# JdeRobot/slam-SDVL

Hardware: AMD Instinct MI355X
Metric: tracked frames/sec (640x480, 5-lvl pyr, ~200 feats) (higher is better)
Workload: dtype u8/f32/f64

## Files before the change

### include/sdvl_hip.h

```cpp
#ifndef SDVL_HIP_H_
#define SDVL_HIP_H_

#include <stdint.h>

#ifdef __cplusplus
extern "C" {
#endif

typedef struct sdvl_ctx sdvl_ctx;
typedef struct sdvl_frame sdvl_frame;

enum sdvl_status {
  SDVL_OK = 0,
  SDVL_ERR_INVALID = -1,
  SDVL_ERR_HIP = -2,
  SDVL_ERR_CAPACITY = -3,
  SDVL_ERR_NO_DEVICE = -4
};

#define SDVL_MAX_LEVELS 8
#define SDVL_MAX_CORNERS 6144
#define SDVL_MAX_ALIGN_FEATURES 2048
#define SDVL_CELL_KP_CAP 176
#define SDVL_MAX_CELL_SIZE 64
// ... 366 lines not shown
  int32_t n_points;
  int32_t n_deleted;
  int32_t lk_iters;
  int32_t n_corners;
  int32_t status;
} sdvl_track_result;

typedef struct sdvl_track_feature_out {
  double px[2];
  int32_t level;
  int32_t point;
} sdvl_track_feature_out;

typedef struct sdvl_track_point_stat {
  int32_t score, n_failed, last_frame;
  int32_t status;
} sdvl_track_point_stat;

int sdvl_track_create(sdvl_ctx *ctx, int n_trackers, int max_points, int max_features, int grid_cells, int max_matches,
                      int max_ransac_its, sdvl_track_set **out);
int sdvl_track_destroy(sdvl_ctx *ctx, sdvl_track_set *set);
int sdvl_frame_register(sdvl_ctx *ctx, const sdvl_frame *frame, const double *pose7);
int sdvl_frames_register(sdvl_ctx *ctx, int n, const sdvl_frame *const *frames, const double *poses7);
int sdvl_track_upload(sdvl_ctx *ctx, sdvl_track_set *set, int n, const int32_t *trackers, const int32_t *feat_buf, const int32_t *n_points,
                      const sdvl_track_point *points, const int32_t *n_features, const sdvl_track_feature *features);
int sdvl_track_append(sdvl_ctx *ctx, sdvl_track_set *set, int n, const int32_t *trackers, const int32_t *feat_buf, const int32_t *n_points,
                      const sdvl_track_point *points, const int32_t *n_features, const sdvl_track_feature *features);
int sdvl_track_align(sdvl_ctx *ctx, sdvl_track_set *set, int n_jobs, const sdvl_track_job *jobs, const uint16_t *cell_rank,
                     const int32_t *rand_raw, const sdvl_camera *cam, const sdvl_track_params *p);
int sdvl_track_search(sdvl_ctx *ctx, sdvl_track_set *set);
int sdvl_track_collect(sdvl_ctx *ctx, sdvl_track_set *set, int n_jobs, sdvl_track_result *results);
const sdvl_track_feature_out *sdvl_track_features(const sdvl_track_set *set, int job);
const sdvl_track_point_stat *sdvl_track_stats(const sdvl_track_set *set, int job);

typedef struct sdvl_klt_job {
  const sdvl_frame *prev, *next;
  int32_t pt_begin, pt_end;
} sdvl_klt_job;

typedef struct sdvl_klt_params {
  int32_t win_size;
  int32_t max_level;
  int32_t max_its;
  int32_t pad_;
  double eps;
  double min_eig_threshold;
} sdvl_klt_params;

int sdvl_klt_track(sdvl_ctx *ctx, int n_jobs, const sdvl_klt_job *jobs, int n_pts, const float *prev_xy, float *next_xy, uint8_t *status,
                   float *err, const sdvl_klt_params *params);

typedef struct sdvl_homography_job {
  int32_t m_begin, m_end;
  int32_t draw_begin, draw_end;
} sdvl_homography_job;

typedef struct sdvl_homography_result {
  double H[9];
  int32_t best_draw;
  int32_t n_its;
  int32_t n_inliers;
  int32_t pad_;
} sdvl_homography_result;

int sdvl_homography_ransac(sdvl_ctx *ctx, int n_jobs, const sdvl_homography_job *jobs, int n_m, const double *src_xy, const double *dst_xy,
                           int n_draws, const int32_t *draws4, double threshold, int max_its, double confidence,
// ... 84 lines not shown
```

### slam-sdvl_amd/__init__.py

```python
import ctypes as C
import os

import numpy as np

try:
    import torch
except ImportError:
    torch = None

_HERE = os.path.dirname(os.path.abspath(__file__))
CSRC = os.path.join(_HERE, "csrc")
LIB_PATH = os.path.join(CSRC, "libsdvl_hip.so")
HOST_LIB_PATH = os.path.join(_HERE, "host", "libsdvl_host.so")

SDVL_GRAY8, SDVL_RGB8, SDVL_BGR8, SDVL_RGBA8, SDVL_BGRA8 = 0, 1, 2, 3, 4
SDVL_BAYER_RGGB8, SDVL_BAYER_GRBG8, SDVL_BAYER_GBRG8, SDVL_BAYER_BGGR8 = 16, 17, 18, 19
SDVL_YUYV8, SDVL_UYVY8 = 20, 21
SDVL_GRAY10_16, SDVL_GRAY12_16, SDVL_GRAY16 = 22, 23, 24


def _raw_bytes(im):
    im = np.asarray(im)
    if im.dtype == np.uint16:
        im = np.ascontiguousarray(im.astype("<u2", copy=False)).view(np.uint8).reshape(im.shape + (2,))
# ... 91 lines not shown
                ("R", C.c_double * 9), ("t", C.c_double * 3), ("plane", C.c_double * 4),
                ("seed", C.c_uint32), ("frame_id", C.c_uint32), ("texture", C.c_uint32), ("reserved_", C.c_uint32),
                ("dist", C.c_double * 5)]


SYNTH_MAX_SURFACES = 8
SYNTH_NO_SURFACE = 255
SYNTH_SCENE_MAX_VIEWS = 4096


class SynthSurface(C.Structure):
    _fields_ = [("plane", C.c_double * 4), ("origin", C.c_double * 3), ("e1", C.c_double * 3), ("e2", C.c_double * 3),
                ("half_u", C.c_double), ("half_v", C.c_double), ("seed_add", C.c_uint32), ("pad_", C.c_uint32)]


class SynthScene(C.Structure):
    _fields_ = [("fx", C.c_double), ("fy", C.c_double), ("u0", C.c_double), ("v0", C.c_double),
                ("R", C.c_double * 9), ("t", C.c_double * 3),
                ("seed", C.c_uint32), ("frame_id", C.c_uint32), ("texture", C.c_uint32), ("n_surfaces", C.c_uint32),
                ("dist", C.c_double * 5), ("surfaces", SynthSurface * SYNTH_MAX_SURFACES)]


ABI_SYMBOLS = [
    "sdvl_ctx_create", "sdvl_ctx_destroy", "sdvl_last_error", "sdvl_ctx_synchronize", "sdvl_ctx_stream",
    "sdvl_ctx_bind_thread", "sdvl_ctx_device", "sdvl_pointer_device", "sdvl_ctx_scratch_device",
    "sdvl_ctx_timing_enable", "sdvl_ctx_timing_only", "sdvl_ctx_timing_get", "sdvl_ctx_timing_reset",
    "sdvl_frame_create", "sdvl_frame_create_many", "sdvl_frame_destroy", "sdvl_frame_upload", "sdvl_frames_upload", "sdvl_ctx_prefetch_images", "sdvl_ctx_prefetch_fence", "sdvl_frame_set_image_device", "sdvl_frame_borrow_image_device",
    "sdvl_pyramid_build", "sdvl_frame_download_level", "sdvl_fast_num_cells", "sdvl_cell_kp_cap", "sdvl_fast_cells",
    "sdvl_detect_corners", "sdvl_frames_corner_counts", "sdvl_frame_download_corners", "sdvl_retain_best",
    "sdvl_frame_set_corners", "sdvl_frames_set_corners", "sdvl_frame_num_corners", "sdvl_shi_tomasi", "sdvl_orb_describe",
    "sdvl_frame_download_descriptors", "sdvl_filter_inputs", "sdvl_filter_inputs_begin", "sdvl_filter_inputs_end", "sdvl_filter_corners_begin", "sdvl_filter_corners_end", "sdvl_orb_describe_points", "sdvl_hamming_argmin", "sdvl_image_align", "sdvl_image_align_begin", "sdvl_image_align_end", "sdvl_align_store_create", "sdvl_align_store_destroy", "sdvl_align_store_write", "sdvl_image_align_begin_stored", "sdvl_search_points", "sdvl_search_begin", "sdvl_search_slot", "sdvl_search_run", "sdvl_align_patches", "sdvl_pose_from_matches", "sdvl_search_points_filter", "sdvl_search_run_filter", "sdvl_depth_filter", "sdvl_search_run_chain", "sdvl_search_chain_end", "sdvl_frame_footprint", "sdvl_undistort", "sdvl_frames_upload_undistorted", "sdvl_convert_gray", "sdvl_frames_upload_color", "sdvl_ctx_set_wait_hook", "sdvl_ctx_wait_done", "sdvl_ctx_wait_block", "sdvl_ctx_health", "sdvl_ctx_counters",
    "sdvl_track_create", "sdvl_track_destroy", "sdvl_frame_register", "sdvl_frames_register", "sdvl_track_upload", "sdvl_track_append", "sdvl_track_align", "sdvl_track_search",
    "sdvl_track_collect", "sdvl_track_features", "sdvl_track_stats",
    "sdvl_synth_render", "sdvl_synth_render_scene", "sdvl_synth_scene_size", "sdvl_synth_scene_preset", "sdvl_synth_scene_preset_names",
    "sdvl_device_malloc", "sdvl_device_free", "sdvl_device_download",
    "sdvl_frames_own_images", "sdvl_feed_create", "sdvl_feed_destroy", "sdvl_feed_last_error", "sdvl_feed_slot_arrived", "sdvl_feed_images", "sdvl_ctx_feed_acquire", "sdvl_ctx_feed_release", "sdvl_frame_footprint_cap", "sdvl_ctx_set_corner_capacity", "sdvl_frame_corner_capacity", "sdvl_detect_scratch_bytes",
    "sdvl_klt_track", "sdvl_homography_ransac", "sdvl_bundle_adjust",
    "sdvl_ctx_set_wait_spin", "sdvl_ctx_fork_mark", "sdvl_ctx_fork_begin", "sdvl_ctx_fork_end", "sdvl_host_alloc_pinned", "sdvl_host_free_pinned", "sdvl_host_register", "sdvl_host_unregister",
]

_lib = None


def load_library():
    global _lib
    if _lib is None:
        if not os.path.exists(LIB_PATH):
            raise SdvlError("libsdvl_hip.so is not built (%s): run `python -c 'import __graft_entry__ as g; g.build()'`"
                            % LIB_PATH)
        lib = C.CDLL(LIB_PATH)
        lib.sdvl_last_error.restype = C.c_char_p
        lib.sdvl_last_error.argtypes = [C.c_void_p]
        lib.sdvl_ctx_stream.restype = C.c_void_p
        lib.sdvl_ctx_stream.argtypes = [C.c_void_p]
        lib.sdvl_bundle_adjust.argtypes = [C.c_void_p, C.c_int, C.c_void_p, C.c_int, C.c_void_p, C.c_void_p, C.c_int, C.c_void_p, C.c_int,
                                           C.c_void_p, C.c_void_p, C.c_void_p, C.c_void_p, C.c_void_p, C.c_void_p]
        lib.sdvl_synth_scene_preset.argtypes = [C.c_char_p, C.c_void_p]
        lib.sdvl_synth_scene_preset_names.restype = C.c_char_p
        lib.sdvl_synth_render_scene.argtypes = [C.c_void_p, C.c_int, C.c_void_p, C.c_int, C.c_int, C.c_void_p, C.c_int64, C.c_void_p, C.c_void_p]
        _lib = lib
    return _lib


def synth_scene_presets():
    return load_library().sdvl_synth_scene_preset_names().decode().split()

# ... 157 lines not shown


class TrackFeature(C.Structure):
    _fields_ = [("px", C.c_double * 2), ("bearing", C.c_double * 3), ("level", C.c_int32), ("point", C.c_int32)]


TRACK_DUPLICATE = 0x40000000


class TrackParams(C.Structure):
    _fields_ = [("align", AlignParams), ("search", SearchParams), ("pose", PoseParams), ("cell_size", C.c_int32), ("patch_size", C.c_int32),
                ("max_failed", C.c_int32), ("pad_", C.c_int32)]


class TrackJob(C.Structure):
    _fields_ = [("tracker", C.c_int32), ("feat_buf", C.c_int32), ("last", C.c_void_p), ("cur", C.c_void_p), ("T", C.c_double * 7),
                ("last_pose", C.c_double * 7), ("frame_id", C.c_int32), ("max_matches", C.c_int32)]


class TrackResult(C.Structure):
    _fields_ = [("pose", C.c_double * 7), ("align_error", C.c_double), ("scene_depth", C.c_double)] + [(n, C.c_int32) for n in (
        "align_meas", "align_iters", "n_features", "n_requests", "matches", "attempts", "n_draws", "n_inliers", "n_outliers", "refined",
        "n_points", "n_deleted", "lk_iters", "n_corners", "status")]


class TrackFeatureOut(C.Structure):
    _fields_ = [("px", C.c_double * 2), ("level", C.c_int32), ("point", C.c_int32)]


class TrackPointStat(C.Structure):
    _fields_ = [("score", C.c_int32), ("n_failed", C.c_int32), ("last_frame", C.c_int32), ("status", C.c_int32)]


class TrackSet:

    def __init__(self, ctx, n_trackers, max_points, max_features, grid_cells, max_matches, max_ransac_its):
        self.ctx = ctx
        self.n, self.cells, self.max_ransac_its = int(n_trackers), int(grid_cells), int(max_ransac_its)
        h = C.c_void_p()
        ctx._check(ctx.lib.sdvl_track_create(ctx.h, self.n, int(max_points), int(max_features), self.cells, int(max_matches),
                                             self.max_ransac_its, C.byref(h)))
        self.h = h
        self.n_points = {}
        ctx.lib.sdvl_track_features.restype = C.POINTER(TrackFeatureOut)
        ctx.lib.sdvl_track_features.argtypes = [C.c_void_p, C.c_int]
        ctx.lib.sdvl_track_stats.restype = C.POINTER(TrackPointStat)
        ctx.lib.sdvl_track_stats.argtypes = [C.c_void_p, C.c_int]

    def _rows(self, fn, trackers, feat_buf, points, features):
        n = len(trackers)
        assert len(feat_buf) == len(points) == len(features) == n
        tr, fb = np.asarray(trackers, np.int32), np.asarray(feat_buf, np.int32)
        npt, nft = np.asarray([len(p) for p in points], np.int32), np.asarray([len(f) for f in features], np.int32)
        pa = (TrackPoint * max(int(npt.sum()), 1))(*[r for p in points for r in p])
        fa = (TrackFeature * max(int(nft.sum()), 1))(*[r for f in features for r in f])
        self.ctx._check(fn(self.ctx.h, self.h, n, _ptr(tr, i32p), _ptr(fb, i32p), _ptr(npt, i32p), pa, _ptr(nft, i32p), fa))
        return tr.tolist(), npt.tolist()

    def upload(self, trackers, feat_buf, points, features):
        for t, k in zip(*self._rows(self.ctx.lib.sdvl_track_upload, trackers, feat_buf, points, features)):
            self.n_points[t] = k

    def append(self, trackers, feat_buf, points, features):
        for t, k in zip(*self._rows(self.ctx.lib.sdvl_track_append, trackers, feat_buf, points, features)):
            self.n_points[t] = self.n_points.get(t, 0) + k

    def step(self, jobs, cell_rank, rand_raw, cam, params, between=None):
        n = len(jobs)
        lib = self.ctx.lib
        rank = np.ascontiguousarray(cell_rank, np.uint16).reshape(n, self.cells)
        raw = np.ascontiguousarray(rand_raw, np.int32).reshape(n, self.max_ransac_its)
        n_points = [self.n_points.get(jobs[j].tracker, 0) for j in range(n)]
        self.ctx._check(lib.sdvl_track_align(self.ctx.h, self.h, n, jobs, _ptr(rank, C.POINTER(C.c_uint16)), _ptr(raw, i32p), C.byref(cam),
                                             C.byref(params)))
        if between is not None:
            between()
        self.ctx._check(lib.sdvl_track_search(self.ctx.h, self.h))
        res = (TrackResult * n)()
        self.ctx._check(lib.sdvl_track_collect(self.ctx.h, self.h, n, res))
        feat_t = np.dtype([("px", "<f8", 2), ("level", "<i4"), ("point", "<i4")])
        stat_t = np.dtype([("score", "<i4"), ("n_failed", "<i4"), ("last_frame", "<i4"), ("status", "<i4")])
        feats, stats = [], []
        for j in range(n):
            fp, sp = lib.sdvl_track_features(self.h, j), lib.sdvl_track_stats(self.h, j)
            feats.append(np.ctypeslib.as_array(C.cast(fp, u8p), (res[j].matches * C.sizeof(TrackFeatureOut),)).view(feat_t).copy()
                         if res[j].matches else np.zeros(0, feat_t))
            stats.append(np.ctypeslib.as_array(C.cast(sp, u8p), (n_points[j] * C.sizeof(TrackPointStat),)).view(stat_t).copy()
                         if n_points[j] else np.zeros(0, stat_t))
        return res, feats, stats

    def close(self):
        if self.h:
            self.ctx._check(self.ctx.lib.sdvl_track_destroy(self.ctx.h, self.h))
            self.h = None


BUNDLE_MAX_FREE = 16
BUNDLE_OK, BUNDLE_EMPTY, BUNDLE_NO_EDGES, BUNDLE_NONFINITE = 0, 1, 2, 3
# ... 321 lines not shown
    def pose_from_matches(self, jobs, fx, max_ransac_points=5, max_ransac_its=100, max_optim_pose_its=10, inlier_error_threshold=2.0):
        n = len(jobs)
        pj = (PoseJob * n)()
        obs_all, rand_all, nits_all = [], [], []
        for k, (obs, pose, draws) in enumerate(jobs):
            obs = np.ascontiguousarray(obs, np.float64).reshape(-1, 6)
            size = len(obs)
            pj[k].obs_begin = len(obs_all); pj[k].obs_end = len(obs_all) + size
            pj[k].rand_begin = len(rand_all); pj[k].nits_begin = len(nits_all)
            for c in range(7):
                pj[k].pose[c] = float(pose[c])
            for o in obs:
                obs_all.append(PoseObs(o[0], o[1], o[2], o[3], o[4], 1.0 / (1 << int(o[5]))))
            assert len(draws) >= max_ransac_its
            rand_all += [int(d) % size if size else 0 for d in draws[:max_ransac_its]]
            nits_all += ransac_budget_table(size, max_ransac_points, max_ransac_its)
        po = (PoseObs * max(len(obs_all), 1))(*obs_all)
        ra = np.asarray(rand_all, np.int32); ni = np.asarray(nits_all, np.int32)
        prm = PoseParams(max_ransac_points, max_ransac_its, max_optim_pose_its, 0, inlier_error_threshold / fx, fx)
        res = (PoseResult * n)()
        lists = np.zeros(max(len(obs_all), 1), np.int32)
        self.lib.sdvl_pose_from_matches.argtypes = [C.c_void_p, C.c_int, C.c_void_p, C.c_int, C.c_void_p, C.c_int, C.c_void_p, C.c_int,
                                                    C.c_void_p, C.c_void_p, C.c_void_p, C.c_void_p]
        self._check(self.lib.sdvl_pose_from_matches(self.h, n, pj, len(obs_all), po, len(ra), _ptr(ra, i32p), len(ni), _ptr(ni, i32p),
                                                    C.byref(prm), res, _ptr(lists, i32p)))
        out = []
        for k in range(n):
            b = pj[k].obs_begin
            out.append(dict(pose=np.array(list(res[k].pose)), n_draws=res[k].n_draws, refined=res[k].refined,
                            inliers=lists[b:b + res[k].n_inliers].copy(),
                            outliers=lists[b + res[k].n_inliers:b + res[k].n_inliers + res[k].n_outliers].copy()))
        return out

    def track_set(self, n_trackers, max_points, max_features, grid_cells, max_matches, max_ransac_its):
        return TrackSet(self, n_trackers, max_points, max_features, grid_cells, max_matches, max_ransac_its)

    def register(self, frames, poses):
        n = len(frames)
        arr = (C.c_void_p * max(n, 1))(*[f.h for f in frames])
        p7 = np.ascontiguousarray(poses, np.float64).reshape(n, 7)
        self._check(self.lib.sdvl_frames_register(self.h, n, arr, _ptr(p7, f64p)))

    def klt_track(self, jobs, win_size=30, max_level=4, max_its=30, eps=0.001, min_eig_threshold=1e-4):
        kj = (KltJob * max(len(jobs), 1))()
        prev_all, next_all = [], []
        at = 0
        for k, (fp, fn, pxy, nxy) in enumerate(jobs):
            pxy = np.asarray(pxy, np.float32).reshape(-1, 2)
            nxy = np.asarray(nxy, np.float32).reshape(-1, 2)
            assert len(pxy) == len(nxy)
            kj[k].prev, kj[k].next = fp.h.value, fn.h.value
            kj[k].pt_begin, kj[k].pt_end = at, at + len(pxy)
            at += len(pxy)
            prev_all.append(pxy)
            next_all.append(nxy)
        prev = np.ascontiguousarray(np.concatenate(prev_all) if jobs else np.zeros((0, 2)), np.float32)
        nxt = np.ascontiguousarray(np.concatenate(next_all) if jobs else np.zeros((0, 2)), np.float32).copy()
        status = np.zeros(max(at, 1), np.uint8)
        err = np.zeros(max(at, 1), np.float32)
        prm = KltParams(win_size, max_level, max_its, 0, eps, min_eig_threshold)
        self.lib.sdvl_klt_track.argtypes = [C.c_void_p, C.c_int, C.c_void_p, C.c_int, C.c_void_p, C.c_void_p, C.c_void_p, C.c_void_p, C.c_void_p]
        self._check(self.lib.sdvl_klt_track(self.h, len(jobs), kj, at, prev.ctypes.data, nxt.ctypes.data, status.ctypes.data, err.ctypes.data,
                                            C.byref(prm)))
        return [dict(xy=nxt[kj[k].pt_begin:kj[k].pt_end].copy(), status=status[kj[k].pt_begin:kj[k].pt_end].astype(bool),
                     err=err[kj[k].pt_begin:kj[k].pt_end].copy()) for k in range(len(jobs))]

# ... 188 lines not shown
```

### slam-sdvl_amd/csrc/sdvl_orb.hip

```cpp
#include <algorithm>
#include <vector>

#include "sdvl_internal.h"
#include "sdvl_orb_device.h"

namespace {

struct OrbJob {
  const uint8_t *level[SDVL_MAX_LEVELS];
  int lw[SDVL_MAX_LEVELS], lh[SDVL_MAX_LEVELS];
  const int32_t *corners;
  uint8_t *desc;
  uint8_t *out;
  float *out_angle;
  double *out_score;
  const int32_t *n_ptr;
  int n;
  int levels;
};

__device__ __forceinline__ bool xcd_frame_block(int n_frames, int chunks, int *frame, int *chunk) {
  const int b = static_cast<int>(blockIdx.x), q = b >> 3;
  *frame = (q / chunks) * 8 + (b & 7);
  *chunk = q % chunks;
  return *frame < n_frames;
}
inline dim3 xcd_frame_grid(int n_frames, int chunks) { return dim3(static_cast<unsigned>((n_frames + 7) / 8 * 8 * chunks)); }

__global__ __launch_bounds__(256) void orb_describe_kernel(const OrbJob *__restrict__ jobs, int n_jobs, int chunks) {
  int fj, bx;
  if (!xcd_frame_block(n_jobs, chunks, &fj, &bx)) return;
  const OrbJob &job = jobs[fj];
  const int lane = threadIdx.x & 63;
  const int n = job.n_ptr ? min(job.n_ptr[0], SDVL_MAX_CORNERS) : job.n;
  const int wpb = static_cast<int>(blockDim.x >> 6);
  for (int ci = bx * wpb + (threadIdx.x >> 6); ci < n; ci += chunks * wpb) {
  const int cx = job.corners[4 * ci], cy = job.corners[4 * ci + 1], cl = job.corners[4 * ci + 2];
  if (cl < 0 || cl >= job.levels) continue;
  const int W = job.lw[cl], H = job.lh[cl];
  uint8_t *dst = job.desc + static_cast<size_t>(ci) * 32;
  if (!(cx >= 19 && cx < W - 19 && cy >= 19 && cy < H - 19)) {
    if (lane < 32) {
      dst[lane] = 0;
      if (job.out) job.out[static_cast<size_t>(ci) * 32 + lane] = 0;
    }
    if (lane == 0 && job.out_angle) job.out_angle[ci] = -1.f;
    continue;
  }
  float angle_deg;
  const uint32_t nib = orb_wave_nibble(job.level[cl], static_cast<uint32_t>(cy * W + cx), W, lane, &angle_deg);
  const uint32_t hi = __shfl_down(nib, 1, 64);
  if ((lane & 1) == 0) {
    const uint8_t byte = static_cast<uint8_t>(nib | (hi << 4));
    dst[lane >> 1] = byte;
    if (job.out) job.out[static_cast<size_t>(ci) * 32 + (lane >> 1)] = byte;
  }
  if (lane == 0 && job.out_angle) job.out_angle[ci] = angle_deg;
  }
}

constexpr int kShiPerWave = 4;
__global__ __launch_bounds__(256) void shi_tomasi_kernel(const OrbJob *__restrict__ jobs, int n_jobs, int chunks) {
  int fj, bx;
  if (!xcd_frame_block(n_jobs, chunks, &fj, &bx)) return;
  const OrbJob &job = jobs[fj];
  const int lane = threadIdx.x & 63, grp = lane >> 4, q = lane & 15;
  const int n = job.n_ptr ? min(job.n_ptr[0], SDVL_MAX_CORNERS) : job.n;
  const int wpb = static_cast<int>(blockDim.x >> 6);
  for (int c0 = (bx * wpb + (threadIdx.x >> 6)) * kShiPerWave; c0 < n; c0 += chunks * wpb * kShiPerWave) {
    const int ci = c0 + grp;
    int sxx = 0, syy = 0, sxy = 0;
    bool inside = false;
    if (ci < n) {
      const int px = job.corners[4 * ci], py = job.corners[4 * ci + 1], cl = job.corners[4 * ci + 2];
      if (cl >= 0 && cl < job.levels) {
        const int W = job.lw[cl], H = job.lh[cl];
        const int x_min = px - 4, x_max = px + 4, y_min = py - 4, y_max = py + 4;
        inside = !(x_min < 1 || x_max >= W - 1 || y_min < 1 || y_max >= H - 1);
        if (inside) {
          const uint8_t *p = job.level[cl] + static_cast<size_t>(y_min + (q >> 1)) * W + (x_min + 4 * (q & 1));
          uint32_t lf, rt, up, dn;
          __builtin_memcpy(&lf, p - 1, 4);
          __builtin_memcpy(&rt, p + 1, 4);
          __builtin_memcpy(&up, p - W, 4);
          __builtin_memcpy(&dn, p + W, 4);
#pragma unroll
          for (int k = 0; k < 4; k++) {
            const int dx = static_cast<int>((rt >> (8 * k)) & 0xFFu) - static_cast<int>((lf >> (8 * k)) & 0xFFu);
            const int dy = static_cast<int>((dn >> (8 * k)) & 0xFFu) - static_cast<int>((up >> (8 * k)) & 0xFFu);
            sxx += dx * dx;
            syy += dy * dy;
            sxy += dx * dy;
          }
        }
      }
    }
#define SDVL_ROW_SUM(v)                                                   \
    v += __builtin_amdgcn_update_dpp(0, v, 0x111, 0xf, 0xf, false);       \
    v += __builtin_amdgcn_update_dpp(0, v, 0x112, 0xf, 0xf, false);       \
    v += __builtin_amdgcn_update_dpp(0, v, 0x114, 0xf, 0xe, false);       \
    v += __builtin_amdgcn_update_dpp(0, v, 0x118, 0xf, 0xc, false);
    SDVL_ROW_SUM(sxx)
    SDVL_ROW_SUM(syy)
    SDVL_ROW_SUM(sxy)
#undef SDVL_ROW_SUM
    if (q == 15 && ci < n) {
      const int cl = job.corners[4 * ci + 2];
      if (cl >= 0 && cl < job.levels) {
        double score = 0.0;
        if (inside) {
          float dXX = static_cast<float>(sxx), dYY = static_cast<float>(syy), dXY = static_cast<float>(sxy);
          dXX = static_cast<float>(dXX / (2.0 * 64));
          dYY = static_cast<float>(dYY / (2.0 * 64));
          dXY = static_cast<float>(dXY / (2.0 * 64));
          const float disc = (dXX + dYY) * (dXX + dYY) - 4 * (dXX * dYY - dXY * dXY);
          score = 0.5 * (dXX + dYY - sqrt(static_cast<double>(disc)));
        }
        job.out_score[ci] = score;
      }
    }
  }
}
inline int shi_chunks(int max_n) { return (max_n + kShiPerWave - 1) / kShiPerWave; }


struct FilterJob {
  const uint8_t *level[SDVL_MAX_LEVELS];
  int lw[SDVL_MAX_LEVELS], lh[SDVL_MAX_LEVELS];
  const int32_t *corners;
  const int32_t *n_ptr;
  const double *scores;
  const uint32_t *locked;
  sdvl_filtered_corner *out;
  int32_t *out_count;
  int levels, ccap;
};

constexpr int kFilterMaxCorners = SDVL_MAX_CORNERS;

__global__ __launch_bounds__(256) void filter_select_kernel(const FilterJob *__restrict__ jobs, int cell_size, int grid_w, int n_cells, int margin,
                                                            int min_score, int max_out) {
  __shared__ uint16_t s_cell[kFilterMaxCorners];
  __shared__ int s_sel[4096];
  __shared__ int s_wave[4];
  const FilterJob &job = jobs[blockIdx.x];
  const int tid = threadIdx.x, lane = tid & 63, wave = tid >> 6;
  const int n = min(min(job.n_ptr[0], job.ccap), kFilterMaxCorners);
  for (int i = tid; i < n; i += 256) {
    const int px = job.corners[4 * i], py = job.corners[4 * i + 1], level = job.corners[4 * i + 2];
    uint16_t c = 0xFFFFu;
    if (level >= 0 && level < job.levels && !(px < margin || py < margin || px >= job.lw[level] - margin || py >= job.lh[level] - margin)) {
      const int scale = 1 << level;
      const int pos = ((py * scale) / cell_size) * grid_w + (px * scale) / cell_size;
      if (pos >= 0 && pos < n_cells && !((job.locked[pos >> 5] >> (pos & 31)) & 1u)) c = static_cast<uint16_t>(pos);
// ... 14 lines not shown
    s_sel[c] = best > min_score ? best_idx : -1;
  }
  __syncthreads();
  int running = 0;
  for (int c0 = 0; c0 < n_cells; c0 += 256) {
    const int c = c0 + tid;
    const bool ok = c < n_cells && s_sel[c] >= 0;
    const unsigned long long m = __ballot(ok);
    const int below = __builtin_amdgcn_mbcnt_hi(static_cast<uint32_t>(m >> 32), __builtin_amdgcn_mbcnt_lo(static_cast<uint32_t>(m), 0));
    __syncthreads();
    if (lane == 0) s_wave[wave] = __popcll(m);
    __syncthreads();
    int pos = running + below;
    for (int w = 0; w < wave; w++) pos += s_wave[w];
    if (ok && pos < max_out) {
      const int i = s_sel[c];
      sdvl_filtered_corner r;
      r.index = i;
      r.x = job.corners[4 * i]; r.y = job.corners[4 * i + 1]; r.level = job.corners[4 * i + 2];
      r.score = static_cast<int>(job.scores[i]);
      r.pad_ = 0;
      sdvl_filtered_corner *dst = job.out + pos;
      dst->index = r.index; dst->x = r.x; dst->y = r.y; dst->level = r.level; dst->score = r.score; dst->pad_ = 0;
    }
    running += s_wave[0] + s_wave[1] + s_wave[2] + s_wave[3];
  }
  if (tid == 0) job.out_count[0] = running;
}

constexpr int kBinCells = 2048, kBinSlots = 10;
constexpr int kBinCellsSmall = 512, kBinCornersSmall = 2048;
constexpr int kBinCellsLarge = SDVL_MAX_LEVEL_CELLS, kBinSlotsLarge = 4;

template <int kCells, int kCorners, int kSlots = kBinSlots>
__global__ __launch_bounds__(256) void filter_select_binned_kernel(const FilterJob *__restrict__ jobs, int cell_size, int grid_w, int n_cells,
                                                                   int margin, int min_score, int max_out) {
  __shared__ uint16_t s_cell[kCorners];
  __shared__ uint16_t s_list[kCells * kSlots];
  __shared__ int s_cnt[kCells];
  __shared__ int s_wave[4];
  const FilterJob &job = jobs[blockIdx.x];
  const int tid = threadIdx.x, lane = tid & 63, wave = tid >> 6;
  const int n = min(min(job.n_ptr[0], job.ccap), kCorners);
  for (int c = tid; c < n_cells; c += 256) s_cnt[c] = 0;
  __syncthreads();
  for (int i = tid; i < n; i += 256) {
    const int px = job.corners[4 * i], py = job.corners[4 * i + 1], level = job.corners[4 * i + 2];
    uint16_t c = 0xFFFFu;
    if (level >= 0 && level < job.levels && !(px < margin || py < margin || px >= job.lw[level] - margin || py >= job.lh[level] - margin)) {
      const int scale = 1 << level;
      const int pos = ((py * scale) / cell_size) * grid_w + (px * scale) / cell_size;
      if (pos >= 0 && pos < n_cells && !((job.locked[pos >> 5] >> (pos & 31)) & 1u)) {
        c = static_cast<uint16_t>(pos);
        const int slot = atomicAdd(&s_cnt[pos], 1);
        if (slot < kSlots) s_list[pos * kSlots + slot] = static_cast<uint16_t>(i);
      }
    }
    s_cell[i] = c;
  }
  __syncthreads();
  for (int c = tid; c < n_cells; c += 256) {
    const int cnt = s_cnt[c];
    int best_idx = 0, best = min_score;
    if (cnt <= kSlots) {
      int idx[kSlots];
#pragma unroll
      for (int q = 0; q < kSlots; q++) idx[q] = q < cnt ? s_list[c * kSlots + q] : 0x7FFFFFFF;
#pragma unroll
      for (int a = 0; a < kSlots; a++)
#pragma unroll
        for (int b = 0; b + 1 < kSlots - a; b++) {
          const int lo = min(idx[b], idx[b + 1]), hi = max(idx[b], idx[b + 1]);
          idx[b] = lo;
          idx[b + 1] = hi;
        }
#pragma unroll
      for (int q = 0; q < kSlots; q++) {
        if (q >= cnt) break;
        const double score = job.scores[idx[q]];
        if (score > best) {
          best_idx = idx[q];
          best = static_cast<int>(score);
        }
      }
    } else {
      for (int i = 0; i < n; i++) {
        if (s_cell[i] != c) continue;
        const double score = job.scores[i];
        if (score > best) {
          best_idx = i;
          best = static_cast<int>(score);
        }
      }
    }
    s_cnt[c] = best > min_score ? best_idx : -1;
  }
  __syncthreads();
  int running = 0;
  for (int c0 = 0; c0 < n_cells; c0 += 256) {
    const int c = c0 + tid;
    const bool ok = c < n_cells && s_cnt[c] >= 0;
    const unsigned long long m = __ballot(ok);
    const int below = __builtin_amdgcn_mbcnt_hi(static_cast<uint32_t>(m >> 32), __builtin_amdgcn_mbcnt_lo(static_cast<uint32_t>(m), 0));
    __syncthreads();
    if (lane == 0) s_wave[wave] = __popcll(m);
    __syncthreads();
    int pos = running + below;
    for (int w = 0; w < wave; w++) pos += s_wave[w];
    if (ok && pos < max_out) {
      const int i = s_cnt[c];
      sdvl_filtered_corner *dst = job.out + pos;
      dst->index = i;
      dst->x = job.corners[4 * i]; dst->y = job.corners[4 * i + 1]; dst->level = job.corners[4 * i + 2];
      dst->score = static_cast<int>(job.scores[i]);
      dst->pad_ = 0;
    }
    running += s_wave[0] + s_wave[1] + s_wave[2] + s_wave[3];
  }
  if (tid == 0) job.out_count[0] = running;
}

__global__ __launch_bounds__(256) void filter_describe_kernel(const FilterJob *__restrict__ jobs, int max_out, int n_jobs, int chunks) {
  int fj, bx;
  if (!xcd_frame_block(n_jobs, chunks, &fj, &bx)) return;
  const FilterJob &job = jobs[fj];
  const int lane = threadIdx.x & 63;
  const int total = min(job.out_count[0], max_out);
  const int wpb = static_cast<int>(blockDim.x >> 6);
  for (int k = bx * wpb + (threadIdx.x >> 6); k < total; k += chunks * wpb) {
    sdvl_filtered_corner *dst = job.out + k;
    const int cx = dst->x, cy = dst->y, cl = dst->level;
    const int W = job.lw[cl], H = job.lh[cl];
    uint8_t byte = 0;
    if (cx >= 19 && cx < W - 19 && cy >= 19 && cy < H - 19) {
      float angle_deg;
      const uint32_t nib = orb_wave_nibble(job.level[cl], static_cast<uint32_t>(cy * W + cx), W, lane, &angle_deg);
      const uint32_t hi = __shfl_down(nib, 1, 64);
      byte = static_cast<uint8_t>(nib | (hi << 4));
    }
    if ((lane & 1) == 0) dst->desc[lane >> 1] = byte;
  }
}

__global__ __launch_bounds__(256) void filter_gather_kernel(const OrbJob *__restrict__ jobs, uint4 *__restrict__ dst, int row_units, int ccap,
                                                            int with_desc) {
  const OrbJob &job = jobs[blockIdx.y];
  const int u = blockIdx.x * 256 + threadIdx.x;
  if (u >= row_units) return;
  uint4 v;
  if (u <= ccap) {
    v = reinterpret_cast<const uint4 *>(job.n_ptr)[u];
  } else if (with_desc) {
    v = reinterpret_cast<const uint4 *>(job.desc)[u - (ccap + 1)];
  } else {
    return;
  }
  dst[static_cast<size_t>(blockIdx.y) * row_units + u] = v;
}

int fill_jobs(sdvl_ctx *ctx, int n, sdvl_frame *const *frames, int cap, uint8_t *d_out_desc, double *d_out_score,
              OrbJob **d_jobs, int *max_n) {
  const size_t bytes = sizeof(OrbJob) * n;
  void *hs = nullptr, *dsx = nullptr;
  int rc = sdvl_stage_alloc(ctx, bytes, &hs, &dsx);
  if (rc) return rc;
  OrbJob *hj = static_cast<OrbJob *>(hs);
  *max_n = 0;
  for (int i = 0; i < n; i++) {
    int rcf = sdvl_frame_fix_header(ctx, frames[i]);
    if (rcf) return rcf;
    const FrameView &v = frames[i]->v;
    memset(&hj[i], 0, sizeof(OrbJob));
    for (int l = 0; l < v.levels; l++) { hj[i].level[l] = v.level[l]; hj[i].lw[l] = v.lw[l]; hj[i].lh[l] = v.lh[l]; }
    hj[i].corners = v.corners;
// ... 18 lines not shown
  const uint8_t *queries;
  const int32_t *offsets;
  const uint8_t *cands;
  int32_t *best;
  int n, threshold;
};

__global__ __launch_bounds__(64) void hamming_argmin_kernel(const HammingJob *jobp) {
  const HammingJob &job = *jobp;
  const int q = blockIdx.x, lane = threadIdx.x;
  if (q >= job.n) return;
  const uint4 *qp = reinterpret_cast<const uint4 *>(job.queries + 32 * static_cast<size_t>(q));
  const uint4 q0 = qp[0], q1 = qp[1];
  const int begin = job.offsets[q], end = job.offsets[q + 1];
  unsigned long long key = (static_cast<unsigned long long>(job.threshold + 1) << 32) | 0xffffffffull;
  for (int c = begin + lane; c < end; c += 64) {
    const uint4 *cp = reinterpret_cast<const uint4 *>(job.cands + 32 * static_cast<size_t>(c));
    const uint4 a = cp[0], b = cp[1];
    const int d = __popc(a.x ^ q0.x) + __popc(a.y ^ q0.y) + __popc(a.z ^ q0.z) + __popc(a.w ^ q0.w) + __popc(b.x ^ q1.x) +
                  __popc(b.y ^ q1.y) + __popc(b.z ^ q1.z) + __popc(b.w ^ q1.w);
    const unsigned long long k = (static_cast<unsigned long long>(d) << 32) | static_cast<unsigned>(c - begin);
    key = k < key ? k : key;
  }
  for (int off = 32; off > 0; off >>= 1) {
    const unsigned long long o = __shfl_xor(key, off, 64);
    key = o < key ? o : key;
  }
  if (lane == 0) {
    const int d = static_cast<int>(key >> 32);
    const bool found = d < job.threshold;
    job.best[2 * q] = found ? static_cast<int>(key & 0xffffffffull) : -1;
    job.best[2 * q + 1] = d;
  }
}

extern "C" {

int sdvl_orb_describe(sdvl_ctx *ctx, int n, sdvl_frame *const *frames, int cap, uint8_t *out_desc) {
  if (!ctx || n < 0 || (n > 0 && !frames)) return SDVL_ERR_INVALID;
  if (n == 0) return SDVL_OK;
  for (int i = 0; i < n; i++) {
    SDVL_REQUIRE(ctx, frames[i] != nullptr, "null frame");
    if (out_desc) {
      int cnt = 0;
      int rc0 = sdvl_frame_count_host(ctx, frames[i], &cnt);
      if (rc0) return rc0;
    }
    if (out_desc && frames[i]->v.n_corners > cap) {
      ctx->err = "descriptor output capacity smaller than the corner count";
      return SDVL_ERR_CAPACITY;
    }
  }
  uint8_t *d_desc = nullptr;
  const size_t out_bytes = out_desc ? static_cast<size_t>(n) * cap * 32 : 0;
  if (out_desc) {
    int rc = sdvl_ensure(ctx, &ctx->d_out, &ctx->d_out_bytes, out_bytes, false);
    if (!rc) rc = sdvl_ensure(ctx, &ctx->h_out, &ctx->h_out_bytes, out_bytes, true);
    if (rc) return rc;
    d_desc = static_cast<uint8_t *>(ctx->d_out);
  }
  OrbJob *d_jobs = nullptr;
  int max_n = 0;
  int rc = fill_jobs(ctx, n, frames, cap, d_desc, nullptr, &d_jobs, &max_n);
  if (rc) return rc;
  if (max_n > 0) SDVL_LAUNCH(ctx, "orb_describe", orb_describe_kernel, xcd_frame_grid(n, max_n), dim3(64), d_jobs, n, max_n);
    SDVL_HIP_CHECK(ctx, hipGetLastError());
// ... 339 lines not shown
```

### slam-sdvl_amd/csrc/sdvl_search_types.h

```cpp
#ifndef SDVL_SEARCH_TYPES_H_
#define SDVL_SEARCH_TYPES_H_

#include "sdvl_internal.h"
#include "sdvl_math.h"

constexpr int kWavesPerBlock = 4;
constexpr int kLdsCorners = 4096;

struct SearchBlock {
  int first, count;
};

struct SearchFrame {
  const uint8_t *level[SDVL_MAX_LEVELS];
  int lw[SDVL_MAX_LEVELS], lh[SDVL_MAX_LEVELS];
  const int32_t *corners;
  const uint8_t *desc;
  const int32_t *n_ptr;
  int levels;
  int bin_gw;
  const int32_t *bin_start;
  const uint2 *bin_entries;
  int bin_cells, pad_;
  int pad2_[2];
// ... 123 lines not shown
};
static_assert(sizeof(TrackPoint) == sizeof(sdvl_track_point), "upload converts in place");
static_assert(sizeof(sdvl_track_point) == 144, "layout");
struct TrackFeat {
  double px[2];
  double bearing[3];
  int32_t level;
  int32_t point;
};
static_assert(sizeof(TrackFeat) == sizeof(sdvl_track_feature) && sizeof(TrackFeat) == 48, "layout");

struct TrackJobDev {
  SearchFrame cur;
  int tracker, feat_buf;
  int cur_id, last_id;
  int frame_id, max_matches;
  int n_feat, n_points;
  double last_pose[7];
  double pad_;
  const uint8_t *last_level[SDVL_MAX_LEVELS];
  double T0[7];
  double pad2_;
};

extern "C" TrackPoint *sdvl_track_points_device(sdvl_track_set *set, int *max_points, int *n_trackers);

int sdvl_search_launch_device(sdvl_ctx *ctx, int n_slots, const SearchReqDev *d_reqs, const SearchFramePose *d_table,
                              const SearchBlock *d_blocks, int n_blocks, const sdvl_camera *cam, const sdvl_search_params *p,
                              SearchPrep *d_prep, sdvl_search_res *d_res, sdvl_search_res *h_res, bool prepared = false, bool binned = true);
int sdvl_select_matches_launch(sdvl_ctx *ctx, int n_frames, const PoseChainIn &in, PoseJobDev *d_jobs, sdvl_pose_obs *d_obs);
int sdvl_image_align_track_enqueue(sdvl_ctx *ctx, int n_jobs, const TrackJobDev *d_jobs, const TrackPoint *d_points, const TrackFeat *d_feats0,
                                   const TrackFeat *d_feats1, int np, int nfeat_cap, int max_nf, int levels, const sdvl_camera *cam,
                                   const sdvl_align_params *p, sdvl_align_result *d_results, int batch_size);
extern "C" int sdvl_ensure_nits_table(sdvl_ctx *ctx, int npoints_cfg, int max_its, int max_size);

#endif
```

### slam-sdvl_amd/csrc/sdvl_track.hip

```cpp
#include <atomic>
#include <chrono>
#include <vector>

#include "sdvl_internal.h"
#include "sdvl_math.h"
#include "sdvl_search_types.h"
#include "sdvl_search_prepare.h"

namespace {

using namespace sdvl;


struct UploadRec {
  int tracker, feat_buf;
  int n_points, n_feat;
  long long point_off, feat_off;
  int point_dst, feat_dst;
  long long pad_;
};

struct RegisterRec {
  SearchFramePose e;
  int id, pad_;
};

__global__ __launch_bounds__(64) void track_clear_bins_kernel(TrackJobDev *__restrict__ jobs, const uint8_t *__restrict__ no_bins, int n) {
  const int j = blockIdx.x * 64 + threadIdx.x;
  if (j < n && no_bins[j]) {
    jobs[j].cur.bin_start = nullptr;
    jobs[j].cur.bin_entries = nullptr;
    jobs[j].cur.bin_gw = 0;
    jobs[j].cur.bin_cells = 0;
  }
}

__global__ __launch_bounds__(64) void registry_write_kernel(const RegisterRec *__restrict__ recs, int n, SearchFramePose *__restrict__ registry) {
  const int i = blockIdx.x * 64 + threadIdx.x;
  if (i < n) registry[recs[i].id] = recs[i].e;
}

__global__ __launch_bounds__(256) void track_upload_kernel(const UploadRec *__restrict__ recs, const TrackPoint *__restrict__ src_points,
                                                           const TrackFeat *__restrict__ src_feats, TrackPoint *__restrict__ points,
                                                           TrackFeat *__restrict__ feats0, TrackFeat *__restrict__ feats1, int np, int nf) {
  const UploadRec r = recs[blockIdx.x];
  const uint4 *sp = reinterpret_cast<const uint4 *>(src_points + r.point_off);
  uint4 *dp = reinterpret_cast<uint4 *>(points + static_cast<size_t>(r.tracker) * np + r.point_dst);
  const int pw = r.n_points * static_cast<int>(sizeof(TrackPoint) / 16);
  for (int i = threadIdx.x; i < pw; i += 256) dp[i] = sp[i];
  const uint4 *sf = reinterpret_cast<const uint4 *>(src_feats + r.feat_off);
  uint4 *df = reinterpret_cast<uint4 *>((r.feat_buf ? feats1 : feats0) + static_cast<size_t>(r.tracker) * nf + r.feat_dst);
  const int fw = r.n_feat * static_cast<int>(sizeof(TrackFeat) / 16);
  for (int i = threadIdx.x; i < fw; i += 256) df[i] = sf[i];
}

constexpr int kProjThreads = 512;

struct ProjLds {
  size_t px, cell, bytes;
  __host__ __device__ constexpr explicit ProjLds(size_t stride) : px(8 * stride), cell(px + 16 * stride), bytes(cell + 2 * stride + 64) {}
};
constexpr size_t kProjLdsDefault = 60 * 1024, kProjLdsMax = ProjLds(4096).bytes;
static_assert(kProjLdsMax == 106560, "track_project at stride 4096");

__global__ __launch_bounds__(kProjThreads) void track_project_kernel(const TrackJobDev *__restrict__ jobs, TrackPoint *__restrict__ points,
                                                                     const TrackFeat *__restrict__ feats0, const TrackFeat *__restrict__ feats1,
                                                                     int np, int nf, int stride, int mm, int max_its,
                                                                     const sdvl_align_result *__restrict__ ares,
                                                                     const uint16_t *__restrict__ cell_rank, int cells, Cam cam, int cell_size,
                                                                     int patch, SearchFramePose *__restrict__ registry,
                                                                     SearchReqDev *__restrict__ reqs, double *__restrict__ req_point,
                                                                     int32_t *__restrict__ cand_first, int32_t *__restrict__ cand_feat,
                                                                     SearchBlock *__restrict__ blocks, ChainFrameDev *__restrict__ chain,
                                                                     sdvl_search_params sprm, SearchPrep *__restrict__ prep) {
  extern __shared__ __attribute__((aligned(16))) uint8_t s_dyn[];
  const ProjLds lds(stride);
  unsigned long long *s_key = reinterpret_cast<unsigned long long *>(s_dyn);
  double *s_px = reinterpret_cast<double *>(s_dyn + lds.px);
  uint16_t *s_cell = reinterpret_cast<uint16_t *>(s_dyn + lds.cell);
  __shared__ double s_pose[7];
  __shared__ int s_ncand;
  const int j = blockIdx.x, tid = threadIdx.x;
  const TrackJobDev &jb = jobs[j];
  const TrackFeat *F = (jb.feat_buf ? feats1 : feats0) + static_cast<size_t>(jb.tracker) * nf;
  TrackPoint *P = points + static_cast<size_t>(jb.tracker) * np;
  const int n_feat = jb.n_feat;
// ... 88 lines not shown
  for (int b = tid; b < nblk; b += static_cast<int>(blockDim.x)) {
    int cnt = n_cand - b * kWavesPerBlock;
    cnt = cnt < 0 ? 0 : (cnt > kWavesPerBlock ? kWavesPerBlock : cnt);
    blocks[j * nblk + b] = SearchBlock{base + b * kWavesPerBlock, cnt};
  }
  if (tid == 0) {
    ChainFrameDev c;
    c.cand_begin = base;
    c.cand_end = base + n_cand;
    c.max_matches = jb.max_matches;
    c.rand_begin = j * max_its;
    c.obs_begin = j * mm;
    c.pad_ = 0;
#pragma unroll
    for (int q = 0; q < 7; q++) c.pose[q] = s_pose[q];
    c.pad2_ = 0.0;
    chain[j] = c;
  }
}

struct CommitLds {
  size_t found, depth, bytes;
  __host__ __device__ CommitLds(size_t stride, size_t mm) : found(2 * (stride + 1)), depth((found + stride + 64 + 7) / 8 * 8), bytes(depth + 8 * mm) {}
};

__global__ __launch_bounds__(256) void track_commit_kernel(const TrackJobDev *__restrict__ jobs, TrackPoint *__restrict__ points,
                                                           const TrackFeat *__restrict__ feats0_c, const TrackFeat *__restrict__ feats1_c,
                                                           TrackFeat *__restrict__ feats0, TrackFeat *__restrict__ feats1, int np, int nf, int stride,
                                                           int mm, const ChainFrameDev *__restrict__ chain, const int32_t *__restrict__ cand_first,
                                                           const int32_t *__restrict__ cand_feat, const sdvl_search_res *__restrict__ res,
                                                           const sdvl_pose_result *__restrict__ pres, const int32_t *__restrict__ lists,
                                                           const sdvl_align_result *__restrict__ ares, Cam cam, int max_failed,
                                                           SearchFramePose *__restrict__ registry, sdvl_track_result *__restrict__ h_results,
                                                           sdvl_track_feature_out *__restrict__ h_feats, sdvl_track_point_stat *__restrict__ h_stats) {
  extern __shared__ __attribute__((aligned(16))) uint8_t s_dyn[];
  const CommitLds lds(stride, mm);
  uint16_t *s_before = reinterpret_cast<uint16_t *>(s_dyn);
  uint8_t *s_found = s_dyn + lds.found;
  double *s_depth = reinterpret_cast<double *>(s_dyn + lds.depth);
  __shared__ int s_wave[4];
  __shared__ int s_attempts, s_deleted, s_lk, s_npoints;
  __shared__ double s_median;
  const int j = blockIdx.x, tid = threadIdx.x, lane = tid & 63, wave = tid >> 6;
  const TrackJobDev &jb = jobs[j];
  const ChainFrameDev &fr = chain[j];
  const int base = fr.cand_begin, n = fr.cand_end - fr.cand_begin;
  const TrackFeat *F = (jb.feat_buf ? feats1_c : feats0_c) + static_cast<size_t>(jb.tracker) * nf;
  TrackFeat *N = (jb.feat_buf ? feats0 : feats1) + static_cast<size_t>(jb.tracker) * nf;
  TrackPoint *P = points + static_cast<size_t>(jb.tracker) * np;
  if (tid == 0) { s_attempts = 0; s_deleted = 0; s_lk = 0; s_npoints = 0; }
  int lk = 0;
  for (int k = tid; k < n; k += 256) {
    const sdvl_search_res &r = res[base + k];
    s_found[k] = r.found != 0 ? 1 : 0;
    lk += r.lk_its;
  }
  __syncthreads();
  if (lk) atomicAdd(&s_lk, lk);
  int running = 0;
  for (int c0 = 0; c0 < n; c0 += 256) {
    const int k = c0 + tid;
    bool sel = false;
    if (k < n && s_found[k]) {
      sel = true;
      for (int q = cand_first[base + k] - base; q < k; q++)
        if (s_found[q]) { sel = false; break; }
    }
    const unsigned long long m = __ballot(sel);
    const int below = __builtin_amdgcn_mbcnt_hi(static_cast<uint32_t>(m >> 32), __builtin_amdgcn_mbcnt_lo(static_cast<uint32_t>(m), 0));
    __syncthreads();
    if (lane == 0) s_wave[wave] = __popcll(m);
    __syncthreads();
    int b = running;
    for (int w = 0; w < wave; w++) b += s_wave[w];
// ... 81 lines not shown
  for (int q = tid; q < jb.n_points; q += 256) {
    TrackPoint &p = P[q];
    if (p.status & kTrash) p.status = (p.status & ~kTrash) | kDeleted;
    sdvl_track_point_stat s;
    s.score = p.score; s.n_failed = p.n_failed; s.last_frame = p.last_frame; s.status = p.status;
    h_stats[static_cast<size_t>(j) * np + q] = s;
  }
  __syncthreads();
  if (tid == 0) {
    sdvl_track_result out;
#pragma unroll
    for (int q = 0; q < 7; q++) out.pose[q] = pr.pose[q];
    out.align_error = ares[j].error;
    out.scene_depth = s_median;
    out.align_meas = ares[j].n_meas;
    out.align_iters = ares[j].iters_run;
    out.n_features = jb.n_feat;
    out.n_requests = n;
    out.matches = matches;
    out.attempts = s_attempts;
    out.n_draws = pr.n_draws;
    out.n_inliers = pr.n_inliers;
    out.n_outliers = pr.n_outliers;
    out.refined = pr.refined;
    out.n_points = s_npoints;
    out.n_deleted = s_deleted;
    out.lk_iters = s_lk;
    out.n_corners = jb.cur.n_ptr[0];
    out.status = 0;
    h_results[j] = out;
#pragma unroll
    for (int q = 0; q < 7; q++) registry[jb.cur_id].pose[q] = pr.pose[q];
  }
}

}

struct sdvl_track_set {
  sdvl_ctx *ctx;
  int n, np, nf, cells, mm, max_its;
  TrackPoint *d_points = nullptr;
  TrackFeat *d_feats[2] = {nullptr, nullptr};
  uint8_t *d_scratch = nullptr;
  sdvl_part<TrackJobDev> djobs;
  sdvl_part<uint16_t> cell_rank;
  sdvl_part<sdvl_align_result> ares;
  sdvl_part<SearchReqDev> reqs;
  sdvl_part<SearchPrep> prep;
  sdvl_part<sdvl_search_res> res;
  sdvl_part<double> reqpt;
  sdvl_part<int32_t> rand, cfirst, cfeat, lists, nobs;
  sdvl_part<SearchBlock> blocks;
  sdvl_part<ChainFrameDev> chain;
  sdvl_part<PoseJobDev> pjobs;
  sdvl_part<sdvl_pose_obs> obs;
  sdvl_part<uint8_t> hyp;
  sdvl_part<sdvl_pose_result> pres;
  uint8_t *h_pinned = nullptr;
  sdvl_track_result *h_results;
  sdvl_track_feature_out *h_feats;
  sdvl_track_point_stat *h_stats;
  std::vector<int> n_points;
  std::vector<int> n_feat[2];
  std::vector<sdvl_track_job> jobs;
  int stride = 0;
  int phase = 0;
  uint32_t ticket = 0;
  sdvl_camera cam;
  sdvl_track_params prm;
};

extern "C" {

int sdvl_track_create(sdvl_ctx *ctx, int n, int max_points, int max_features, int grid_cells, int max_matches, int max_ransac_its,
                      sdvl_track_set **out) {
  if (!ctx || !out) return SDVL_ERR_INVALID;
  *out = nullptr;
  SDVL_REQUIRE(ctx, n >= 1 && n <= 65536, "tracker count out of range");
  SDVL_REQUIRE(ctx, max_points >= 1 && max_points < SDVL_TRACK_DUPLICATE && max_features >= 4 && max_features <= 4096, "table capacities out of range (features <= 4096)");
  SDVL_REQUIRE(ctx, grid_cells >= 1 && grid_cells <= 65535, "grid too large");
  SDVL_REQUIRE(ctx, max_matches >= 1 && max_matches <= 1024 && max_matches <= max_features, "max_matches outside the device pose stage's range (1024)");
  SDVL_REQUIRE(ctx, max_ransac_its >= 1 && max_ransac_its <= 4096, "bad max_ransac_its");
  SDVL_HIP_CHECK(ctx, sdvl_bind_device(ctx));
  sdvl_track_set *s = new sdvl_track_set();
  s->ctx = ctx;
  s->n = n;
  s->np = max_points;
  s->nf = (max_features + 3) / 4 * 4;
  s->cells = grid_cells;
  s->mm = max_matches;
  s->max_its = max_ransac_its;
  const size_t N = static_cast<size_t>(n), NF = N * s->nf;
  hipError_t e = hipMalloc(reinterpret_cast<void **>(&s->d_points), sizeof(TrackPoint) * N * s->np);
  if (e == hipSuccess) e = hipMalloc(reinterpret_cast<void **>(&s->d_feats[0]), sizeof(TrackFeat) * NF);
  if (e == hipSuccess) e = hipMalloc(reinterpret_cast<void **>(&s->d_feats[1]), sizeof(TrackFeat) * NF);
  sdvl_layout L;
  s->djobs = L.take<TrackJobDev>(N);
  s->cell_rank = L.take<uint16_t>(N * s->cells);
  s->rand = L.take<int32_t>(N * s->max_its);
  s->ares = L.take<sdvl_align_result>(N);
  s->reqs = L.take<SearchReqDev>(NF);
  s->prep = L.take<SearchPrep>(NF);
  s->res = L.take<sdvl_search_res>(NF);
  s->reqpt = L.take<double>(NF * 3);
  s->cfirst = L.take<int32_t>(NF);
  s->cfeat = L.take<int32_t>(NF);
  s->blocks = L.take<SearchBlock>(NF / kWavesPerBlock);
  s->chain = L.take<ChainFrameDev>(N);
  const bool separate = sdvl_pose_separate_launches(n);
  s->pjobs = L.take<PoseJobDev>(separate ? N : 0);
  s->obs = L.take<sdvl_pose_obs>(N * s->mm);
  s->hyp = L.take<uint8_t>(separate ? sdvl_pose_hyp_bytes() * N * s->max_its : 0);
  s->pres = L.take<sdvl_pose_result>(N);
  s->lists = L.take<int32_t>(N * s->mm);
  s->nobs = L.take<int32_t>(N);
  if (e == hipSuccess) e = hipMalloc(reinterpret_cast<void **>(&s->d_scratch), L.bytes());
  if (e == hipSuccess) {
    sdvl_layout H;
    const sdvl_part<sdvl_track_result> results = H.take<sdvl_track_result>(N);
    const sdvl_part<sdvl_track_feature_out> feats = H.take<sdvl_track_feature_out>(NF);
    const sdvl_part<sdvl_track_point_stat> stats = H.take<sdvl_track_point_stat>(N * s->np);
    e = hipHostMalloc(reinterpret_cast<void **>(&s->h_pinned), H.bytes(), hipHostMallocDefault);
    if (e == hipSuccess) {
      memset(s->h_pinned, 0, H.bytes());
      s->h_results = results.in(s->h_pinned);
      s->h_feats = feats.in(s->h_pinned);
      s->h_stats = stats.in(s->h_pinned);
    }
  }
  if (e != hipSuccess) {
    ctx->err = std::string("sdvl_track_create: ") + hipGetErrorString(e);
    sdvl_track_destroy(ctx, s);
    return SDVL_ERR_HIP;
  }
  s->n_points.assign(n, 0);
  s->n_feat[0].assign(n, 0);
  s->n_feat[1].assign(n, 0);
  *out = s;
  return SDVL_OK;
}

TrackPoint *sdvl_track_points_device(sdvl_track_set *set, int *max_points, int *n_trackers) {
  if (max_points) *max_points = set->np;
  if (n_trackers) *n_trackers = set->n;
  return set->d_points;
}

int sdvl_track_destroy(sdvl_ctx *ctx, sdvl_track_set *s) {
  if (!ctx || !s) return SDVL_ERR_INVALID;
  (void)sdvl_bind_device(ctx);
  (void)sdvl_stream_wait(ctx);
  if (s->d_points) (void)hipFree(s->d_points);
  if (s->d_feats[0]) (void)hipFree(s->d_feats[0]);
  if (s->d_feats[1]) (void)hipFree(s->d_feats[1]);
  if (s->d_scratch) (void)hipFree(s->d_scratch);
  if (s->h_pinned) (void)hipHostFree(s->h_pinned);
  delete s;
  return SDVL_OK;
}

int sdvl_frame_register(sdvl_ctx *ctx, const sdvl_frame *f, const double *pose7) { return sdvl_frames_register(ctx, 1, &f, pose7); }

int sdvl_frames_register(sdvl_ctx *ctx, int n, const sdvl_frame *const *frames, const double *poses7) {
  if (!ctx || n < 0 || (n > 0 && (!frames || !poses7))) return SDVL_ERR_INVALID;
  if (n == 0) return SDVL_OK;
  for (int i = 0; i < n; i++)
    SDVL_REQUIRE(ctx, frames[i] && frames[i]->home == ctx && frames[i]->reg_id >= 0 && frames[i]->reg_id < ctx->registry_cap,
                 "frame was not created on this context");
  void *hs = nullptr, *dsx = nullptr;
  int rc = sdvl_stage_alloc(ctx, sizeof(RegisterRec) * static_cast<size_t>(n), &hs, &dsx);
  if (rc) return rc;
  RegisterRec *r = static_cast<RegisterRec *>(hs);
  for (int i = 0; i < n; i++) {
    fill_view(&r[i].e.f, frames[i]);
    memcpy(r[i].e.pose, poses7 + 7 * i, sizeof(double) * 7);
    r[i].e.pad_ = 0.0;
    r[i].id = frames[i]->reg_id;
    r[i].pad_ = 0;
  }
  SDVL_HIP_CHECK(ctx, sdvl_push(ctx, dsx, hs, sizeof(RegisterRec) * static_cast<size_t>(n)));
  SDVL_LAUNCH(ctx, "registry_write", registry_write_kernel, dim3((n + 63) / 64), dim3(64), static_cast<const RegisterRec *>(dsx), n,
              static_cast<SearchFramePose *>(ctx->d_registry));
  SDVL_HIP_CHECK(ctx, hipGetLastError());
  return SDVL_OK;
}

static int track_upload_rows(sdvl_ctx *ctx, sdvl_track_set *s, int n, const int32_t *trackers, const int32_t *feat_buf, const int32_t *n_points,
                             const sdvl_track_point *points, const int32_t *n_features, const sdvl_track_feature *features, bool append) {
// ... 92 lines not shown
  rc = sdvl_ensure_nits_table(ctx, p->pose.max_ransac_points, p->pose.max_ransac_its, s->mm);
  if (rc) return rc;
  s->stride = (max_nf + kWavesPerBlock - 1) / kWavesPerBlock * kWavesPerBlock;
  if (s->stride < kWavesPerBlock) s->stride = kWavesPerBlock;
  s->cam = *cam;
  s->prm = *p;
  s->jobs.assign(jobs, jobs + n_jobs);
  const size_t rand_bytes = sizeof(int32_t) * static_cast<size_t>(n_jobs) * s->max_its;
  const size_t head_bytes = s->rand.off + rand_bytes;
  void *hs = nullptr, *dsx = nullptr;
  rc = sdvl_stage_alloc(ctx, head_bytes, &hs, &dsx);
  if (rc) return rc;
  TrackJobDev *hj = s->djobs.in(hs);
  for (int j = 0; j < n_jobs; j++) {
    const sdvl_track_job &a = jobs[j];
    TrackJobDev &d = hj[j];
    fill_view(&d.cur, a.cur,  true);
    d.tracker = a.tracker;
    d.feat_buf = a.feat_buf;
    d.cur_id = a.cur->reg_id;
    d.last_id = a.last->reg_id;
    d.frame_id = a.frame_id;
    d.max_matches = a.max_matches;
    d.n_feat = s->n_feat[a.feat_buf][a.tracker];
    d.n_points = s->n_points[a.tracker];
    memcpy(d.last_pose, a.last_pose, sizeof(double) * 7);
    d.pad_ = 0.0;
    SDVL_REQUIRE(ctx, a.last->width == a.cur->width && a.last->height == a.cur->height && a.last->v.levels == a.cur->v.levels,
                 "frame pair with different geometry");
    for (int l = 0; l < SDVL_MAX_LEVELS; l++) d.last_level[l] = l < a.last->v.levels ? a.last->v.level[l] : nullptr;
    memcpy(d.T0, a.T, sizeof(double) * 7);
    d.pad2_ = 0.0;
  }
  memcpy(s->cell_rank.in(hs), cell_rank, sizeof(uint16_t) * static_cast<size_t>(n_jobs) * s->cells);
  memcpy(s->rand.in(hs), rand_raw, rand_bytes);
  SDVL_HIP_CHECK(ctx, sdvl_push(ctx, s->d_scratch, hs, head_bytes));
  rc = sdvl_image_align_track_enqueue(ctx, n_jobs, s->djobs.cin(s->d_scratch), static_cast<const TrackPoint *>(s->d_points),
                                      static_cast<const TrackFeat *>(s->d_feats[0]), static_cast<const TrackFeat *>(s->d_feats[1]), s->np, s->nf, max_nf,
                                      jobs[0].cur->v.levels, cam, &p->align, s->ares.in(s->d_scratch), s->n);
  if (rc) return rc;
  s->phase = 1;
  return SDVL_OK;
}

int sdvl_track_search(sdvl_ctx *ctx, sdvl_track_set *s) {
  if (!ctx || !s || s->ctx != ctx) return SDVL_ERR_INVALID;
  SDVL_REQUIRE(ctx, s->phase == 1, "sdvl_track_search without sdvl_track_align");
  const int n_jobs = static_cast<int>(s->jobs.size());
  for (const sdvl_track_job &a : s->jobs) {
    SDVL_REQUIRE(ctx, !a.cur->hdr_stale, "current frame has a new image but no corners (detect or set corners first)");
    SDVL_REQUIRE(ctx, s->prm.search.max_fast_levels <= a.cur->v.levels, "max_fast_levels exceeds the pyramid depth");
  }
  const Cam c = cam_of(s->cam);
  const int stride = s->stride;
  uint8_t *const D = s->d_scratch;
  SearchFramePose *registry = static_cast<SearchFramePose *>(ctx->d_registry);
  {
    static const bool never = getenv("SDVL_TRACK_NO_BINS") != nullptr;
    bool any = false;
    for (const sdvl_track_job &a : s->jobs) any = any || (a.cur->bin_cells > 0 && (never || !a.cur->bins_valid));
    for (const sdvl_track_job &a : s->jobs) ctx->counters[(a.cur->bin_cells > 0 && !never && a.cur->bins_valid) ? 0 : 1]++;
    if (any) {
      void *hs = nullptr, *dsx = nullptr;
      const int rc_m = sdvl_stage_alloc(ctx, static_cast<size_t>(n_jobs), &hs, &dsx);
      if (rc_m) return rc_m;
      uint8_t *hm = static_cast<uint8_t *>(hs);
      for (int j = 0; j < n_jobs; j++) hm[j] = (s->jobs[j].cur->bin_cells > 0 && (never || !s->jobs[j].cur->bins_valid)) ? 1 : 0;
      SDVL_HIP_CHECK(ctx, sdvl_push(ctx, dsx, hs, static_cast<size_t>(n_jobs)));
      hipLaunchKernelGGL(track_clear_bins_kernel, dim3((n_jobs + 63) / 64), dim3(64), 0, ctx->stream, s->djobs.in(D), static_cast<const uint8_t *>(dsx), n_jobs);
      SDVL_HIP_CHECK(ctx, hipGetLastError());
    }
  }
  const size_t proj_lds = ProjLds(stride).bytes;
  if (proj_lds > kProjLdsDefault) {
    static std::atomic<unsigned long long> attr_devices{0};
    const int rc_a = sdvl_allow_dynamic_lds(ctx, reinterpret_cast<const void *>(track_project_kernel), kProjLdsMax, &attr_devices);
    if (rc_a) return rc_a;
  }
  {
    const int proj_threads = stride <= 256 ? (s->n > 32 ? 128 : 256) : kProjThreads;
    SDVL_LAUNCH_LDS(ctx, "track_project", track_project_kernel, dim3(n_jobs), dim3(proj_threads), proj_lds, s->djobs.cin(D), s->d_points,
                    static_cast<const TrackFeat *>(s->d_feats[0]), static_cast<const TrackFeat *>(s->d_feats[1]), s->np, s->nf, stride, s->mm,
                    s->max_its, s->ares.cin(D), s->cell_rank.cin(D), s->cells, c, s->prm.cell_size, s->prm.patch_size, registry, s->reqs.in(D),
                    s->reqpt.in(D), s->cfirst.in(D), s->cfeat.in(D), s->blocks.in(D), s->chain.in(D), s->prm.search, s->prep.in(D));
    SDVL_HIP_CHECK(ctx, hipGetLastError());
  }
  int rc = sdvl_search_launch_device(ctx, n_jobs * stride, s->reqs.in(D), registry, s->blocks.in(D), n_jobs * (stride / kWavesPerBlock), &s->cam,
                                     &s->prm.search, s->prep.in(D), s->res.in(D), nullptr,  true);
  if (rc) return rc;
  const PoseChainIn chain = {s->chain.cin(D), nullptr, s->cfirst.cin(D), s->res.cin(D), s->reqpt.cin(D), c, s->nobs.in(D), nullptr};
  const bool separate = sdvl_pose_separate_launches(s->n);
  sdvl_pose_params pp = s->prm.pose;
  pp.pad_ = 1;
  rc = sdvl_pose_enqueue_device(ctx, n_jobs, &chain, separate ? s->pjobs.in(D) : nullptr, s->obs.in(D), s->rand.in(D), static_cast<const int32_t *>(ctx->d_nits),
                                &pp, separate ? s->hyp.in(D) : nullptr, s->pres.in(D), s->lists.in(D), s->mm, s->n);
  if (rc) return rc;
  SDVL_LAUNCH_LDS(ctx, "track_commit", track_commit_kernel, dim3(n_jobs), dim3(256), CommitLds(stride, s->mm).bytes, s->djobs.cin(D), s->d_points,
                  static_cast<const TrackFeat *>(s->d_feats[0]), static_cast<const TrackFeat *>(s->d_feats[1]), s->d_feats[0], s->d_feats[1], s->np,
                  s->nf, stride, s->mm, s->chain.cin(D), s->cfirst.cin(D), s->cfeat.cin(D), s->res.cin(D), s->pres.cin(D), s->lists.cin(D),
                  s->ares.cin(D), c, s->prm.max_failed, registry, s->h_results, s->h_feats, s->h_stats);
  SDVL_HIP_CHECK(ctx, hipGetLastError());
  SDVL_HIP_CHECK(ctx, sdvl_mark_record(ctx, SDVL_MARK_CHAIN, &s->ticket));
  s->phase = 2;
  return SDVL_OK;
}

int sdvl_track_collect(sdvl_ctx *ctx, sdvl_track_set *s, int n_jobs, sdvl_track_result *results) {
  if (!ctx || !s || s->ctx != ctx || !results) return SDVL_ERR_INVALID;
  SDVL_REQUIRE(ctx, s->phase == 2 && n_jobs == static_cast<int>(s->jobs.size()), "sdvl_track_collect without a matching sdvl_track_search");
  SDVL_HIP_CHECK(ctx, sdvl_mark_wait(ctx, SDVL_MARK_CHAIN, s->ticket));
  s->phase = 0;
  memcpy(results, s->h_results, sizeof(sdvl_track_result) * n_jobs);
  for (int j = 0; j < n_jobs; j++) {
    const sdvl_track_job &a = s->jobs[j];
    s->n_feat[1 - a.feat_buf][a.tracker] = results[j].matches;
    if (results[j].n_corners >= 0) a.cur->v.n_corners = results[j].n_corners;
  }
  ctx->wait_gen++;
  return SDVL_OK;
}

const sdvl_track_feature_out *sdvl_track_features(const sdvl_track_set *s, int job) {
  return (s && job >= 0 && job < s->n) ? s->h_feats + static_cast<size_t>(job) * s->nf : nullptr;
}

const sdvl_track_point_stat *sdvl_track_stats(const sdvl_track_set *s, int job) {
  return (s && job >= 0 && job < s->n) ? s->h_stats + static_cast<size_t>(job) * s->np : nullptr;
}

}
```

### slam-sdvl_amd/host/capi.cc

```cpp
#include <algorithm>
#include <cstddef>
#include <cstring>
#include <set>
#include <string>

#include "farm.h"
#include "homography_init.h"

using namespace sdvl;

namespace {
thread_local std::string g_err;
bool g_use_mapper = false;

template <typename F>
int Guarded(F body) {
  try {
    body();
    return 0;
  } catch (const std::exception &e) {
    g_err = e.what();
    return -1;
  }
}
// ... 130 lines not shown
  for (int k = 0; k < 6; k++) out6[k] = 0.0;
  for (auto &kf : b->map(i).GetKeyframes())
    for (auto &ft : kf->GetFeatures()) {
      Point *p = ft ? ft->GetPointRaw() : nullptr;
      if (!p || !seen.insert(p).second) continue;
      out6[0] += 1.0;
      out6[1] += p->Score();
      out6[2] += p->GetFailed();
      out6[3] += p->ToDelete() ? 1.0 : 0.0;
      out6[4] += p->GetInverseDepth();
      out6[5] += p->GetStd();
    }
  return 0;
}

int sdvlh_batch_map_points(void *bp, int i, int cap, double *out4) {
  TrackerGroup *b = AsGroup(bp);
  if (!b || i < 0 || i >= b->size()) return -1;
  MapperMap *m = dynamic_cast<MapperMap *>(&b->map(i));
  if (!m) return -1;
  int n = -1;
  const int rc = Guarded([&] {
    Device::SetCurrent(b->device());
    b->batch().SyncHostState();
    const std::vector<MapperMap::MapPoint> pts = m->GetMapPoints();
    n = static_cast<int>(pts.size());
    for (int k = 0; k < n && k < cap && out4; k++) {
      out4[4 * k] = pts[k].x; out4[4 * k + 1] = pts[k].y; out4[4 * k + 2] = pts[k].z; out4[4 * k + 3] = pts[k].fixed ? 1.0 : 0.0;
    }
  });
  return rc ? -2 : n;
}

void sdvlh_set_device_pose(int on) { SDVLBatch::SetDevicePose(on != 0); }
int sdvlh_device_pose() { return SDVLBatch::DevicePose() ? 1 : 0; }

long sdvlh_batch_stage_times(void *bp, double *out, int cap, int reset) {
  StageTimes &st = AsGroup(bp)->batch().stage_times;
  for (int i = 0; i < cap && i < ST_COUNT; i++) out[i] = st.t[i];
  const long n = st.steps;
  if (reset) st = StageTimes();
  return n;
}

int sdvlh_batch_step_host(void *bp, const uint8_t *const *imgs, int stride, sdvlh_frame_stats *out) {
  return Guarded([&] { AsGroup(bp)->Step(TrackerGroup::Frames::kHost, reinterpret_cast<const void *const *>(imgs), stride, out); });
}
int sdvlh_batch_step_device(void *bp, const void *const *dev_imgs, int stride, sdvlh_frame_stats *out) {
  return Guarded([&] { AsGroup(bp)->Step(TrackerGroup::Frames::kResident, dev_imgs, stride, out); });
}
int sdvlh_batch_step_device_transient(void *bp, const void *const *dev_imgs, int stride, sdvlh_frame_stats *out) {
  return Guarded([&] { AsGroup(bp)->Step(TrackerGroup::Frames::kTransient, dev_imgs, stride, out); });
}
int sdvlh_batch_set_next_device(void *bp, const void *const *dev_imgs, int stride) {
  return Guarded([&] { AsGroup(bp)->SetNextImages(dev_imgs, stride); });
}

void *sdvlh_farm_create(int gpu, int G, int Bg, int w, int h, const double *cam4, const double *plane4, const double *first_poses7,
                        int host_threads_per_group) {
  try {
    return new TrackerFarm(gpu, G, Bg, w, h, cam4, plane4, first_poses7, host_threads_per_group, g_use_mapper);
  } catch (const std::exception &e) {
    g_err = e.what();
    return nullptr;
  }
}
// ... 60 lines not shown
```

### slam-sdvl_amd/host/frontend.cc

```cpp
#include "host_internal.h"

#include <algorithm>
#include <atomic>
#include <cmath>
#include <condition_variable>
#include <cstdlib>
#include <cstring>
#include <iostream>
#include <mutex>
#include <new>
#include <stdexcept>
#include <chrono>
#include <thread>

#include <sys/mman.h>

namespace sdvl {

using std::shared_ptr;
using std::vector;

static thread_local Device *g_current_device = nullptr;

static thread_local StageTimes *g_stage_times = nullptr;
// ... 565 lines not shown

vector<vector<uchar>> &Frame::GetDescriptors() {
  if (!descriptors_on_host_ && Config::UseORB() && !GetCorners().empty()) {
    Device *dev = Device::Current();
    vector<uint8_t> buf(corners_.size() * 32);
    dev->Check(sdvl_frame_download_descriptors(dev->ctx(), dev_, static_cast<int>(corners_.size()), buf.data()), "sdvl_frame_download_descriptors");
    descriptors_.resize(corners_.size());
    for (size_t i = 0; i < corners_.size(); i++) descriptors_[i].assign(buf.begin() + 32 * i, buf.begin() + 32 * (i + 1));
    descriptors_on_host_ = true;
  }
  return descriptors_;
}

void Frame::FilterCorners() { FilterCornersBatch({shared_from_this()}); }

void Frame::FilterCornersBatch(const vector<shared_ptr<Frame>> &frames) {
  FilterCornersBegin(frames);
  FilterCornersEnd(frames);
}

void Frame::FilterCornersBegin(const vector<shared_ptr<Frame>> &frames) {
  const int n = static_cast<int>(frames.size());
  if (n == 0) return;
  Device *dev = Device::Current();
  const int cell = Config::CellSize();
  const int gw = static_cast<int>(std::ceil(static_cast<double>(frames[0]->width_) / cell));
  const int gh = static_cast<int>(std::ceil(static_cast<double>(frames[0]->height_) / cell));
  const int words = (gw * gh + 31) / 32;
  vector<sdvl_frame *> devs(n);
  vector<uint32_t> locked(static_cast<size_t>(n) * words, 0u);
  for (int i = 0; i < n; i++) {
    Frame &f = *frames[i];
    devs[i] = f.dev_;
    f.ForEachFeaturePosition([&](double px, double py) {
      const int index = static_cast<int>(py / cell) * gw + static_cast<int>(px / cell);
      if (index >= 0 && index < gw * gh) locked[static_cast<size_t>(i) * words + (index >> 5)] |= 1u << (index & 31);
    });
  }
  dev->Check(sdvl_filter_corners_begin(dev->ctx(), n, devs.data(), locked.data(), words, cell, DetectMargin(), Config::MinFeatureScore(),
                                       Config::UseORB() ? 1 : 0), "sdvl_filter_corners_begin");
}

void Frame::FilterCornersEnd(const vector<shared_ptr<Frame>> &frames, const std::function<void(int, const std::function<void(int)> &)> *pfor) {
  const int n = static_cast<int>(frames.size());
  if (n == 0) return;
  Device *dev = Device::Current();
  const int cell = Config::CellSize();
  const int gw = static_cast<int>(std::ceil(static_cast<double>(frames[0]->width_) / cell));
  const int gh = static_cast<int>(std::ceil(static_cast<double>(frames[0]->height_) / cell));
  const int cap = gw * gh;
  vector<int32_t> counts(n);
  vector<sdvl_filtered_corner> &recs = dev->scratch_filtered;
  if (recs.size() < static_cast<size_t>(n) * cap) recs.resize(static_cast<size_t>(n) * cap);
  dev->Check(sdvl_filter_corners_end(dev->ctx(), n, cap, counts.data(), recs.data()), "sdvl_filter_corners_end");
  (void)pfor;
  for (int i = 0; i < n; i++) {
    Frame &f = *frames[i];
    f.filt_.assign(recs.begin() + static_cast<size_t>(i) * cap, recs.begin() + static_cast<size_t>(i) * cap + counts[i]);
    f.filtered_corners_.resize(counts[i]);
    for (int k = 0; k < counts[i]; k++) f.filtered_corners_[k] = f.filt_[k].index;
  }
}

int Frame::GetNumPoints() const {
  int count = 0;
  if (flat_)
    for (const sdvl_track_feature_out &f : flat_->feats) count += f.point >= 0 ? 1 : 0;
  for (auto it = features_.begin(); it != features_.end(); it++) {
    if (!(*it)) continue;
    if (!(*it)->GetPointRaw()) continue;
    count++;
  }
  return count;
}

bool Frame::Project(const Vector3d &p3D, Vector2d *p2D) {
  const Vector3d rel_p = GetRelativePos(p3D);
  if (rel_p(2) < 0.0) return false;
  camera_->Project(rel_p, p2D);
  return true;
}

void Frame::SetFlatFeatures(const sdvl_track_feature_out *feats, int n, const shared_ptr<PointTable> &points) {
  features_.clear();
  DropFlat();
  if (!arena_) arena_ = NewArena();
  sdvl_track_feature_out *dst = nullptr;
  if (n > 0) {
    dst = static_cast<sdvl_track_feature_out *>(arena_->Allocate(sizeof(sdvl_track_feature_out) * static_cast<size_t>(n), alignof(sdvl_track_feature_out)));
    std::memcpy(dst, feats, sizeof(sdvl_track_feature_out) * static_cast<size_t>(n));
  }
  flat_store_.feats.data = dst;
  flat_store_.feats.n = n;
// ... 711 lines not shown
```

### slam-sdvl_amd/host/frontend.h

```cpp
#ifndef SDVL_FRONTEND_H_
#define SDVL_FRONTEND_H_

#include "frontend_deps.h"

namespace sdvl {

class ChunkPool {
 public:
  static constexpr size_t kChunk = 32 * 1024;
  ~ChunkPool();
  char *Get();
  void Put(char *c);

 private:
  void Map(size_t bytes);
  std::mutex m_;
  std::vector<char *> free_;
  std::vector<std::pair<void *, size_t>> regions_;
};

class Device {
 public:
  explicit Device(int gpu = 0);
  ~Device();
// ... 153 lines not shown
template <typename T>
struct ArenaAllocator {
  typedef T value_type;
  FrameArena *arena;
  explicit ArenaAllocator(FrameArena *a) : arena(a) {}
  template <typename U>
  ArenaAllocator(const ArenaAllocator<U> &o) : arena(o.arena) {}
  T *allocate(size_t n) { return static_cast<T *>(arena->Allocate(n * sizeof(T), alignof(T))); }
  void deallocate(T *, size_t) { arena->Release(); }
  template <typename U>
  bool operator==(const ArenaAllocator<U> &o) const { return arena == o.arena; }
  template <typename U>
  bool operator!=(const ArenaAllocator<U> &o) const { return arena != o.arena; }
};


class Frame : public std::enable_shared_from_this<Frame> {
 public:
  Frame(Camera *camera, ORBDetector *detector, const Image &img, bool corners);
  ~Frame();
  static void CreateBatch(Camera *camera, ORBDetector *detector, const std::vector<Image> &imgs, bool corners, int nfeatures,
                          std::vector<std::shared_ptr<Frame>> *out, const std::function<void(int, std::function<void(int)>)> *pfor = nullptr);

  bool IsKeyframe() { return is_keyframe_; }
  void SetKeyframe() { is_keyframe_ = true; }
  bool ImageTransient() const { return image_transient_; }
  void SetImageTransient(bool on) { image_transient_ = on; }
  static void OwnImages(const std::vector<std::shared_ptr<Frame>> &frames);
  void FilterCorners();
  static void FilterCornersBatch(const std::vector<std::shared_ptr<Frame>> &frames);
  static void FilterCornersBegin(const std::vector<std::shared_ptr<Frame>> &frames);
  static void FilterCornersEnd(const std::vector<std::shared_ptr<Frame>> &frames,
                               const std::function<void(int, const std::function<void(int)> &)> *pfor = nullptr);
  static void DetectBatch(const std::vector<std::shared_ptr<Frame>> &frames, int nfeatures);
  SE3 &GetPose() { return pose_; }
  const SE3 &GetPose() const { return pose_; }
  void SetPose(const SE3 &se3) { pose_ = se3; }
  std::vector<Image> &GetPyramid();
  typedef std::vector<std::shared_ptr<Point>> PointTable;
  std::vector<std::shared_ptr<Feature>> &GetFeatures() {
    if (flat_) MaterializeFeatures();
    return features_;
  }
  void SetFlatFeatures(const sdvl_track_feature_out *feats, int n, const std::shared_ptr<PointTable> &points);
  bool HasFlatFeatures() const { return flat_ != nullptr; }
  bool IsRegistered() const { return registered_; }
  void SetRegistered() { registered_ = true; }
  void ClearRegistered() { registered_ = false; }
  int GetLastBA() const { return last_ba_; }
  void SetLastBA(int id) { last_ba_ = id; }
  std::vector<Vector3i> &GetCorners();
  int GetNumCorners();
  std::vector<int> &GetFilteredCorners() { return filtered_corners_; }
  std::vector<Vector2d> &GetOutliers() { return outliers_; }
  std::vector<std::vector<uchar>> &GetDescriptors();
  int NumFiltered() const { return static_cast<int>(filt_.size()); }
  Vector3i FilteredCorner(int k) const { return Vector3i(filt_[k].x, filt_[k].y, filt_[k].level); }
  const uchar *FilteredDescriptor(int k) const { return filt_[k].desc; }
  const uchar *HostDescriptor(int index) const {
    for (const sdvl_filtered_corner &c : filt_)
      if (c.index == index) return c.desc;
    return nullptr;
  }
  Camera *GetCamera() const { return camera_; }
  int GetWidth() const { return width_; }
  int GetHeight() const { return height_; }
// ... 246 lines not shown
```

### slam-sdvl_amd/host/frontend_deps.h

```cpp
#ifndef SDVL_FRONTEND_DEPS_H_
#define SDVL_FRONTEND_DEPS_H_

#include <array>
#include <atomic>
#include <cstring>
#include <functional>
#include <deque>
#include <list>
#include <memory>
#include <mutex>
#include <string>
#include <thread>
#include <utility>
#include <vector>

#include "../../include/sdvl_hip.h"
#include "config.h"
#include "se3.h"
#include "types.h"

namespace sdvl {

class Frame;
class Feature;
// ... 78 lines not shown
  int GetLastBA() const { return last_ba_; }
  void SetLastBA(int id) { last_ba_ = id; }
  static void ConsumeId();
  static double ComputeTau(const SE3 &pose, const Vector3d &v, double depth, double px_error_angle);
  static double PDFNormal(double mean, double sd, double x);

 private:
  PointStatus status_;
  bool delete_;
  bool fixed_;
  int last_frame_, n_successful_, n_failed_;
  int id_;
  Vector3d p3d_;
  double rho_;
  std::shared_ptr<Feature> feature_;
  double sigma2_, a_, b_, z_range_;
  double cos_alpha_ = 1.0, last_distance_ = 1.0;
  int track_row_ = -1;
  int seen_stamp_ = -1;
  int last_ba_ = -1;
  bool dev_trashed_ = false;
  std::list<std::shared_ptr<Feature>> features_;
};

class Map {
 public:
  virtual ~Map() {}
  std::mutex &GetMutex() { return mutex_map_; }
  virtual void UpdateMap() {}
  virtual void Start() {}
  virtual void Stop() {}
  void DeletePoint(const std::shared_ptr<Point> &p) { points_trash_.push_back(p); version_++; }
  bool NeedKeyframe(const std::shared_ptr<Frame> &frame, int matches);
  virtual void AddKeyframe(const std::shared_ptr<Frame> &frame, bool search = true);
  virtual void AddFrame(const std::shared_ptr<Frame> &) {}
  virtual void LimitKeyframes(const std::shared_ptr<Frame> &) {}
  virtual void SetRelocalizing(bool) {}
  virtual void EmptyTrash();
  bool TakeTablesDirty() { const bool d = tables_dirty_; tables_dirty_ = false; return d; }
  std::vector<std::shared_ptr<Frame>> &GetKeyframes() { return keyframes_; }
  unsigned long long Version() const { return version_; }
  void Touch() { version_++; }
  virtual void InitCandidates(const std::shared_ptr<Frame> &) {}

 protected:
  std::vector<std::shared_ptr<Frame>> keyframes_;
  std::vector<std::shared_ptr<Point>> points_trash_;
  bool tables_dirty_ = false;
  unsigned long long version_ = 0;
  std::shared_ptr<Frame> last_kf_;
  int last_matches_ = 0;
  std::mutex mutex_map_;
};

}

#endif
```

### slam-sdvl_amd/host/sdvl_host.h

```cpp
#ifndef SDVL_HOST_H_
#define SDVL_HOST_H_

#include "frontend.h"
#include "bundle.h"

namespace sdvl {

class PlaneMap : public Map {
 public:
  PlaneMap(const Vector3d &n, double d) : n_(n), d_(d) {}
  void InitCandidates(const std::shared_ptr<Frame> &kf) override;
  void SeedFromFiltered(const std::shared_ptr<Frame> &kf);
  void SetPlane(const Vector3d &n, double d) { n_ = n; d_ = d; }
  void LimitKeyframes(const std::shared_ptr<Frame> &frame) override;
  void EmptyTrash() override;

 private:
  Vector3d n_;
  double d_;
  std::vector<std::shared_ptr<Frame>> culled_;
};

class MapperMap : public PlaneMap {
 public:
// ... 71 lines not shown
  std::thread thread_;
  std::atomic<bool> running_{false};
  std::atomic<long> updates_{0};
  Device *tracker_device_ = nullptr;
};

typedef std::pair<std::shared_ptr<Point>, Vector2d> PointInfo;
typedef std::list<PointInfo> GridCell;

class SDVLBatch;
class HomographyInit;

class SDVL {
 public:
  enum State { STATE_FIRST_FRAME, STATE_SECOND_FRAME, STATE_RUNNING };
  enum TrackingQuality { TRACKING_GOOD, TRACKING_INSUFFICIENT, TRACKING_BAD };
  explicit SDVL(Camera *camera);
  SDVL(Camera *camera, Map *map, const SE3 &first_pose = SE3());
  ~SDVL();
  void SetBootstrapPlane(const Vector3d &n, double d);
  void SetTwoFrameInit(bool on);
  bool TwoFrameInit() const { return two_frame_init_; }
  void SetBundleAdjustment(bool on);
  void GetCameraTrail(std::vector<std::pair<SE3, bool>> *positions);
  void GetPoints(std::vector<Vector3d> *positions);
  void GetLastFeatures(std::vector<Vector3i> *positions);
  void Start() { map_->Start(); }
  void Stop() { map_->Stop(); }
  void Mapping();
  bool HandleFrame(const Image &img);
  void SetNextImage(const Image &next);
  SE3 GetPose() const;
  TrackingQuality GetTrackingQuality() const { return tracking_quality_; }
  bool HasMap() { return state_ == STATE_RUNNING; }
  const FrameStats &LastStats() const { return stats_; }
  Map *GetMap() { return map_; }
  const StageTimes *HandleFrameStageTimes() const;

 private:
  friend class SDVLBatch;
  void CalcTrackingQuality(int matches, int attempts);
  void SetMotionModel();
  void GetMotionModel();
  void ResetMotionModel();
  void SaveFirstFrame(FrameStats &st);
  bool InitFirstFrame(FrameStats &st);
  void SecondFrameDone(bool initialised, FrameStats &st);
  bool two_frame_init_ = false, init_failed_ = false;
  std::unique_ptr<HomographyInit> h_init_;
  int TrackingDecision();
  void StartRelocalizing();
  void Relocalized(const std::shared_ptr<Frame> &kf, FrameStats &st);
  void LinkFeatures();
  void SaveKeyframe(FrameStats &st);
  std::unique_ptr<Device> own_device_;
  std::unique_ptr<Map> own_map_;
  Camera *camera_;
  Map *map_;
  ORBDetector orb_detector_;
  RandStream rng_;
  State state_ = STATE_FIRST_FRAME;
  std::shared_ptr<Frame> current_frame_, last_frame_, last_kf_, pending_kf_;
  TrackingQuality tracking_quality_ = TRACKING_GOOD;
  Vector6d vel_;
  FeatureAlign feature_align_;
  int lost_frames_ = 0, matches_ = 0, attempts_ = 0;
  int frame_counter_ = 0;
  SE3 first_pose_;
  FrameStats stats_;
  bool relocalize_pending_ = false;
  std::unique_ptr<SDVLBatch> self_batch_;
  std::vector<Image> next_image_;
  void SyncSelfBatch();
  struct TrackState {
    bool valid = false;
    int feat_buf = 0;
    int slot = 0;
    const void *owner = nullptr;
    std::shared_ptr<Frame::PointTable> points;
    std::vector<sdvl_track_point_stat> stats;
    bool stats_dirty = false;
    std::vector<sdvl_track_point> up_points;
    std::vector<sdvl_track_feature> up_feats;
    std::vector<Frame *> up_register;
    bool append_pending = false;
    size_t first_seed = 0;
  } track_;
  struct RelocCache {
    const void *owner = nullptr;
    unsigned long long version = ~0ull;
    unsigned long long epoch = 0;
    std::vector<std::shared_ptr<Frame>> kfs;
    std::vector<int32_t> begin;
    std::vector<double> T;
  } reloc_;
};

class SDVLBatch {
 public:
  SDVLBatch(Device *dev, const std::vector<SDVL *> &trackers, int host_threads);
  ~SDVLBatch();
  void HandleFrames(const std::vector<Image> &imgs, FrameStats *stats);
  void SetNextImages(const std::vector<Image> &next);
  static void SetDevicePose(bool on);
  static bool DevicePose();
  static void SetTrackTables(bool on);
  static bool TrackTables();
  void SyncHostState();

 private:
  void ParallelFor(int n, const std::function<void(int)> &fn);
 public:
  StageTimes stage_times;
 private:
  friend class SDVL;
  Device *dev_;
  std::vector<SDVL *> trk_;
  int threads_;
  std::function<void(int, std::function<void(int)>)> pfor_;
  std::function<void(int, const std::function<void(int)> &)> pfor_ref_;
  std::vector<sdvl_search_req> scratch_reqs_;
  FeatureAlign::PoseBatch scratch_pose_;
  std::vector<double> scratch_points_;
  std::vector<int32_t> chain_cand_req_, chain_cand_first_, chain_rand_;
  struct Step;
  struct HostStep;
  enum FrameStart { kFirstFrame, kLost, kRunning };
  FrameStart BeginFrame(int i, const std::shared_ptr<Frame> &frame, FrameStats &st);
  void InitializeTrackers(Step &s);
  void DetectOnSideStream(const std::vector<std::shared_ptr<Frame>> &frames, bool fork);
  void FetchCornerCounts(const std::vector<std::shared_ptr<Frame>> &frames, FrameStats *stats);
  void CollectKeyframes(Step &s, bool fetch_counts);
  void GatherRows(const std::vector<int> &up, bool own_buf);
  void SyncStats(SDVL &t);
  void EpilogueAndMapper(Step &s);
  void FinishKeyframes(Step &s);
  void RunMappers();
  bool HandleFramesTracked(const std::vector<Image> &imgs, FrameStats *stats);
  bool TrackedStepApplies();
  bool EnsureTrackSet();
  void TakeLookAhead(Step &s);
  void QueueLookAhead(const Step &s);
  void RelocalizeIntoStep(Step &s);
  sdvl_track_params AssembleTrackJobs(const Step &s);
  void SubmitTracked(Step &s);
  void ReplayTracked(Step &s);
  void SaveTrackedFrames(Step &s);
  void InvalidateStaleTables();
  int TrackOnHost(SDVL &t, FrameStats *st);
  bool BuildTable(SDVL &t);
  bool UploadTables(const std::vector<int> &need, std::vector<char> *built);
  bool AppendSeeds(SDVL &t, const std::shared_ptr<Frame> &kf);
  std::vector<Image> next_imgs_;
  std::vector<std::shared_ptr<Frame>> ahead_frames_;
  std::vector<const void *> ahead_src_;
  sdvl_track_set *track_ = nullptr;
  int track_cells_ = 0, track_cap_ = 0;
  std::vector<sdvl_track_job> tr_jobs_;
  std::vector<uint16_t> tr_rank_;
  std::vector<int32_t> tr_rand_;
  std::vector<sdvl_track_result> tr_res_;
  std::vector<sdvl_track_point> tr_up_points_;
  std::vector<sdvl_track_feature> tr_up_feats_;
  std::vector<int32_t> tr_up_trk_, tr_up_buf_, tr_up_np_, tr_up_nf_;
  void RelocalizeLost(const std::vector<int> &lost, FrameStats *stats, std::vector<char> *found);
  void PackRelocCache(SDVL &t, std::vector<sdvl_align_feature> *packed);
  void RefreshRelocStore(const std::vector<int> &lost);
  void RelocAlignKeyframes(const std::vector<int> &lost, std::vector<int> *first, std::vector<sdvl_align_result> *res);
  void RelocAlign(const std::vector<sdvl_align_job> &jobs, const sdvl_align_params &ap, std::vector<sdvl_align_result> *res);
  sdvl_align_store *reloc_store_ = nullptr;
  int reloc_cap_ = 0, reloc_used_ = 0;
  unsigned long long reloc_epoch_ = 0;
  void HandleFramesGeneric(const std::vector<Image> &imgs, FrameStats *stats);
  bool RelocalizeOnHost(SDVL &t, FrameStats &st);
  void AlignImages(HostStep &s);
  void PackRequests(HostStep &s);
  void PackChain(HostStep &s);
  void CollectRequests(HostStep &s);
  void LaunchSearch(HostStep &s);
  void ReplaySelect(HostStep &s);
  void LaunchPose(HostStep &s);
  void CommitAndSave(HostStep &s);
};

}

#endif
```

### slam-sdvl_amd/host/standalone.cc

```cpp
#include "sdvl_host.h"
#include "homography_init.h"
#include "host_internal.h"

#include <algorithm>
#include <atomic>
#include <cmath>
#include <condition_variable>
#include <cstdlib>
#include <cstring>
#include <iostream>
#include <mutex>
#include <new>
#include <stdexcept>
#include <chrono>
#include <thread>

#include <sys/mman.h>

namespace sdvl {

using std::shared_ptr;
using std::vector;

Camera::Camera() {
// ... 113 lines not shown
  }
}

Vector3d Point::GetPosition() const {
  if (fixed_) return p3d_;
  Frame *fr = feature_->GetFrameRaw();
  const SE3 se3 = fr->GetWorldPose();
  const Vector3d &v = feature_->GetVector();
  const double s = 1.0 / rho_;
  return se3 * Vector3d(s * v(0), s * v(1), s * v(2));
}

void Point::SetPosition(const Vector3d &pos) {
  if (fixed_) {
    p3d_ = pos;
    return;
  }
  shared_ptr<Frame> frame = feature_->GetFrame();
  Vector2d p2d;
  frame->Project(pos, &p2d);
  Vector3d v3d = frame->GetCamera()->Unproject(p2d);
  feature_->SetVector(v3d);
  rho_ = 1.0 / frame->DistanceTo(pos);
}

bool Point::Promote() { n_successful_++; n_failed_ = 0; return true; }
bool Point::Unpromote() {
  n_failed_++;
  b_++;
  return n_failed_ > Config::MaxFailed();
}

bool Map::NeedKeyframe(const shared_ptr<Frame> &frame, int) {
  const int npoints = frame->GetNumPoints();
  const bool enough_its = (frame->GetID() - last_kf_->GetID()) >= Config::MinKeyframeIts();
  const bool lost_many = npoints < last_matches_ * Config::LostRatio();
  const bool lost_some = npoints < last_matches_ * 0.9;
  last_matches_ = std::max(last_matches_, npoints);
  if ((enough_its && lost_some) || lost_many) {
    last_matches_ = npoints;
    return true;
  }
  return false;
}

void Map::AddKeyframe(const shared_ptr<Frame> &frame, bool) {
  version_++;
  keyframes_.push_back(frame);
  last_kf_ = frame;
}

void Map::EmptyTrash() {
  if (!points_trash_.empty()) version_++;
  for (auto &p : points_trash_) {
    if (!p->ToDelete() && p->TrackRow() >= 0 && !p->DeviceTrashed()) tables_dirty_ = true;
    std::list<shared_ptr<Feature>> &features = p->GetFeatures();
    for (auto it = features.begin(); it != features.end(); it++) (*it)->SetPoint(nullptr);
    features.clear();
    p->SetDelete();
  }
  points_trash_.clear();
}

void PlaneMap::LimitKeyframes(const shared_ptr<Frame> &frame) {
  if (static_cast<int>(keyframes_.size()) < Config::MaxKeyframes()) return;
  const Vector3d pos = frame->GetWorldPosition();
  shared_ptr<Frame> kf;
  double maxdist = 0.0;
  for (auto it = keyframes_.begin(); it != keyframes_.end(); it++) {
    const Vector3d q = (*it)->GetWorldPosition();
    const double dist = vnorm({q(0) - pos(0), q(1) - pos(1), q(2) - pos(2)});
    if (dist > maxdist) {
      maxdist = dist;
// ... 116 lines not shown
        const double zmin = 1.0 / (p->GetInverseDepth() + 2.0 * p->GetStd());
        const double zmax = 1.0 / (std::max(p->GetInverseDepth() - 2.0 * p->GetStd(), 0.00000001));
        const Vector3d &v = p->GetInitFeature()->GetVector();
        const SE3 pose = p->GetInitFeature()->GetFrame()->GetWorldPose();
        positions->push_back(pose * Vector3d(v(0) * zmin, v(1) * zmin, v(2) * zmin));
        positions->push_back(pose * Vector3d(v(0) * zmax, v(1) * zmax, v(2) * zmax));
      }
    }
  }
}

void SDVL::GetLastFeatures(vector<Vector3i> *positions) {
  std::unique_lock<std::mutex> lock(map_->GetMutex());
  SyncSelfBatch();
  positions->clear();
  if (!last_frame_) return;
  vector<shared_ptr<Feature>> &features = last_frame_->GetFeatures();
  for (auto feature = features.begin(); feature != features.end(); feature++) {
    shared_ptr<Point> point = (*feature)->GetPoint();
    if (!point || point->ToDelete()) continue;
    const Vector2d &pos = (*feature)->GetPosition();
    positions->push_back(Vector3i(static_cast<int>(pos(0)), static_cast<int>(pos(1)), static_cast<int>(point->GetStatus())));
  }
  vector<Vector2d> &outliers = last_frame_->GetOutliers();
  for (auto it = outliers.begin(); it != outliers.end(); it++)
    positions->push_back(Vector3i(static_cast<int>((*it)(0)), static_cast<int>((*it)(1)), static_cast<int>(Point::P_OUTLIER)));
}

SE3 SDVL::GetPose() const {
  if (last_frame_) return last_frame_->GetWorldPose();
  return SE3();
}

void SDVL::CalcTrackingQuality(int matches, int attempts) {
  const double ratio = (attempts == 0) ? 0.0 : static_cast<double>(matches) / static_cast<double>(attempts);
  if (ratio > 0.2) {
    tracking_quality_ = TRACKING_GOOD;
    lost_frames_ = 0;
    return;
  }
  if (matches < Config::MinMatches()) {
    tracking_quality_ = TRACKING_BAD;
    lost_frames_++;
    return;
  }
  lost_frames_ = 0;
  tracking_quality_ = TRACKING_INSUFFICIENT;
}

void SDVL::SetMotionModel() { current_frame_->SetPose(SE3::Exp(vel_) * last_frame_->GetPose()); }

void SDVL::GetMotionModel() {
  const SE3 mov = current_frame_->GetPose() * last_frame_->GetPose().Inverse();
  const Vector6d vel = SE3::Log(mov);
  for (int c = 0; c < 6; c++) vel_[c] = 0.9 * (0.5 * vel[c] + 0.5 * vel_[c]);
}

void SDVL::ResetMotionModel() {
  for (int k = 0; k < 6; k++) vel_[k] = 0.0;
}

void SDVL::SaveFirstFrame(FrameStats &st) {
  current_frame_->SetPose(first_pose_);
  current_frame_->SetKeyframe();
  map_->AddKeyframe(current_frame_, false);
  pending_kf_ = current_frame_;
  last_frame_ = current_frame_;
  last_kf_ = current_frame_;
  state_ = STATE_RUNNING;
  track_.valid = false;
  st.state = 0;
  st.keyframe = 1;
}

void SDVL::SetBundleAdjustment(bool on) {
  MapperMap *m = dynamic_cast<MapperMap *>(map_);
  if (!m) throw std::runtime_error("SDVL::SetBundleAdjustment needs the reference's mapper (MapperMap)");
  m->SetBundleAdjustment(on);
}

void SDVL::SetTwoFrameInit(bool on) {
  if (on && !dynamic_cast<MapperMap *>(map_)) throw std::runtime_error("SDVL::SetTwoFrameInit needs the reference's mapper (MapperMap)");
  two_frame_init_ = on;
  if (on && !h_init_) h_init_.reset(new HomographyInit(map_, Config::MinAvgShift()));
}

bool SDVL::InitFirstFrame(FrameStats &st) {
  st.state = 0;
  current_frame_->CreateCorners(Config::MaxFastLevels(), 2 * Config::NumFeatures());
  current_frame_->SetPose(SE3());
  last_frame_ = current_frame_;
  last_kf_ = current_frame_;
  track_.valid = false;
  if (!h_init_->InitFirstFrame(current_frame_)) return false;
  current_frame_->SetKeyframe();
  map_->AddKeyframe(current_frame_, false);
  state_ = STATE_SECOND_FRAME;
  st.keyframe = 1;
  return true;
}

void SDVL::SecondFrameDone(bool initialised, FrameStats &st) {
  st.state = 1;
  track_.valid = false;
  if (!initialised) {
// ... 35 lines not shown
  map_->SetRelocalizing(false);
  last_kf_ = kf;
  last_frame_ = kf;
  track_.valid = false;
  st.relocalized = 1;
}

void SDVL::LinkFeatures() {
  vector<shared_ptr<Feature>> &features = current_frame_->GetFeatures();
  for (auto it = features.begin(); it != features.end(); it++)
    if (Point *p = (*it)->GetPointRaw()) p->AddFeature(*it);
}

void SDVL::SaveKeyframe(FrameStats &st) {
  current_frame_->SetKeyframe();
  map_->AddKeyframe(current_frame_);
  last_kf_ = current_frame_;
  map_->LimitKeyframes(current_frame_);
  if (!dynamic_cast<MapperMap *>(map_)) pending_kf_ = current_frame_;
  st.keyframe = 1;
}

void SDVL::SetNextImage(const Image &next) {
  next_image_.assign(1, next);
}

bool SDVL::HandleFrame(const Image &img) {
  std::unique_lock<std::mutex> lock(map_->GetMutex());
  FrameStats st;
  Device *dev = Device::Current();
  if (!self_batch_ || self_batch_->dev_ != dev) {
    if (self_batch_) self_batch_->SyncHostState();
    self_batch_.reset(new SDVLBatch(dev, {this}, 1));
    track_.valid = false;
  }
  if (!next_image_.empty()) {
    self_batch_->SetNextImages(next_image_);
    next_image_.clear();
  }
  try {
    self_batch_->HandleFrames({img}, &st);
  } catch (...) {
    self_batch_.reset();
    track_.valid = false;
    throw;
  }
  return !init_failed_;
}

void SDVL::Mapping() {
  std::unique_lock<std::mutex> lock(map_->GetMutex());
  if (pending_kf_) {
    PlaneMap *pm = dynamic_cast<PlaneMap *>(map_);
    if (pm) {
      pending_kf_->FilterCorners();
      pm->SeedFromFiltered(pending_kf_);
    } else {
      map_->InitCandidates(pending_kf_);
    }
    pending_kf_ = nullptr;
  }
  if (MapperMap *m = dynamic_cast<MapperMap *>(map_)) m->UpdateMap();
}

namespace {
class Pool {
// ... 302 lines not shown
      if (!ref->IsRegistered()) {
        double pose[7];
        ref->GetPose().ToArray(pose);
        reg_frames.push_back(ref->device());
        reg_poses.insert(reg_poses.end(), pose, pose + 7);
        ref->SetRegistered();
      }
    up.push_back(need[q]);
  }
  GatherRows(up, false);
  if (!reg_frames.empty())
    dev_->Check(sdvl_frames_register(dev_->ctx(), static_cast<int>(reg_frames.size()), reg_frames.data(), reg_poses.data()), "sdvl_frames_register");
  if (!up.empty())
    dev_->Check(sdvl_track_upload(dev_->ctx(), track_, static_cast<int>(up.size()), tr_up_trk_.data(), tr_up_buf_.data(), tr_up_np_.data(), tr_up_points_.data(),
                                  tr_up_nf_.data(), tr_up_feats_.data()), "sdvl_track_upload");
  for (int i : up) {
    trk_[i]->track_.feat_buf = 0;
    trk_[i]->track_.valid = true;
  }
  if (built) *built = ok;
  return true;
}

struct SDVLBatch::Step {
  Step(const vector<Image> &i, FrameStats *st, int B) : imgs(i), stats(st), decision(B, 0) {}
  const vector<Image> &imgs;
  FrameStats *stats;
  vector<shared_ptr<Frame>> frames;
  vector<int> run, lost, host_run;
  vector<int> init;
  vector<char> decision;
  vector<shared_ptr<Frame>> kfs;
  vector<int> kf_owner;
  bool filter_begun = false;
  bool detected = false;
  std::unique_ptr<StageClock> clk;
  void Stage(int id) { clk.reset(new StageClock(id)); }
  int R() const { return static_cast<int>(run.size()); }
};

static void Concatenate(const vector<vector<sdvl_search_req>> &per, vector<sdvl_search_req> *all, vector<size_t> *begin) {
  begin->resize(per.size() + 1);
  size_t total = 0;
  for (size_t k = 0; k < per.size(); k++) {
    (*begin)[k] = total;
    total += per[k].size();
    if (all) all->insert(all->end(), per[k].begin(), per[k].end());
  }
  (*begin)[per.size()] = total;
}

SDVLBatch::FrameStart SDVLBatch::BeginFrame(int i, const shared_ptr<Frame> &frame, FrameStats &st) {
  SDVL &t = *trk_[i];
  st = FrameStats();
  t.current_frame_ = frame;
  t.current_frame_->SetID(t.frame_counter_++);
  if (t.state_ != SDVL::STATE_RUNNING) {
    if (!t.two_frame_init_) t.SaveFirstFrame(st);
    return kFirstFrame;
  }
  st.state = 2;
  return t.lost_frames_ >= 3 ? kLost : kRunning;
}

void SDVLBatch::InitializeTrackers(Step &s) {
  vector<int> second;
// ... 55 lines not shown
                                       res.data(), inl.data()),
                "sdvl_homography_ransac");
    for (size_t f = 0; f < fit.size(); f++) {
      SDVL &t = *trk_[second[fit[f]]];
      done[fit[f]] = t.h_init_->FinishSecondFrame(res[f], inl.data() + hjobs[f].m_begin, &t.rng_) ? 1 : 0;
    }
  }
  for (size_t k = 0; k < second.size(); k++) trk_[second[k]]->SecondFrameDone(done[k] != 0, s.stats[second[k]]);
}

void SDVLBatch::DetectOnSideStream(const vector<shared_ptr<Frame>> &frames, bool fork) {
  if (fork) dev_->Check(sdvl_ctx_fork_begin(dev_->ctx()), "sdvl_ctx_fork_begin");
  try {
    Frame::DetectBatch(frames, Config::NumFeatures());
  } catch (...) {
    if (fork) (void)sdvl_ctx_fork_end(dev_->ctx());
    throw;
  }
  if (fork) dev_->Check(sdvl_ctx_fork_end(dev_->ctx()), "sdvl_ctx_fork_end");
}

void SDVLBatch::FetchCornerCounts(const vector<shared_ptr<Frame>> &frames, FrameStats *stats) {
  const int B = static_cast<int>(frames.size());
  vector<sdvl_frame *> devs(B);
  vector<int32_t> counts(B);
  for (int i = 0; i < B; i++) devs[i] = frames[i]->device();
  dev_->Check(sdvl_frames_corner_counts(dev_->ctx(), B, devs.data(), counts.data()), "sdvl_frames_corner_counts");
  for (int i = 0; i < B; i++) stats[i].n_corners = counts[i];
}

void SDVLBatch::CollectKeyframes(Step &s, bool fetch_counts) {
  s.kfs.clear();
  s.kf_owner.clear();
  for (size_t i = 0; i < trk_.size(); i++) {
    const bool fresh = s.decision[i] == 2 && !dynamic_cast<MapperMap *>(trk_[i]->map_);
    if (trk_[i]->pending_kf_) { s.kfs.push_back(trk_[i]->pending_kf_); s.kf_owner.push_back(static_cast<int>(i)); }
    else if (fresh) { s.kfs.push_back(trk_[i]->current_frame_); s.kf_owner.push_back(static_cast<int>(i)); }
  }
  if (s.kfs.empty()) return;
  std::unique_ptr<StageClock> nested(s.clk->id != ST_MAPPING ? new StageClock(ST_MAPPING) : nullptr);
  if (fetch_counts) FetchCornerCounts(s.frames, s.stats);
  Frame::FilterCornersBegin(s.kfs);
  s.filter_begun = true;
}

static std::atomic<unsigned long long> g_reloc_epoch{1};

void SDVLBatch::RelocAlign(const vector<sdvl_align_job> &jobs, const sdvl_align_params &ap, vector<sdvl_align_result> *res) {
  res->resize(jobs.size());
  const sdvl_camera cam = trk_[0]->camera_->abi();
  const size_t kChunk = 4096;
  for (size_t b = 0; b < jobs.size(); b += kChunk) {
    const int n = static_cast<int>(std::min(jobs.size(), b + kChunk) - b);
    dev_->Check(sdvl_image_align_begin_stored(dev_->ctx(), n, jobs.data() + b, reloc_store_, &cam, &ap), "sdvl_image_align_begin_stored");
    dev_->Check(sdvl_image_align_end(dev_->ctx(), n, res->data() + b), "sdvl_image_align_end");
  }
}

void SDVLBatch::PackRelocCache(SDVL &t, vector<sdvl_align_feature> *packed) {
  SDVL::RelocCache &rc = t.reloc_;
  rc.kfs.clear();
  rc.begin.assign(1, 0);
  rc.T.clear();
  vector<shared_ptr<Frame>> &kfs = t.map_->GetKeyframes();
  for (auto it = kfs.rbegin(); it != kfs.rend(); it++) {
    rc.kfs.push_back(*it);
    ImageAlign::PackFeatures(**it, packed);
    rc.begin.push_back(static_cast<int32_t>(packed->size()));
    double T7[7];
    ((*it)->GetPose() * (*it)->GetPose().Inverse()).ToArray(T7);
    rc.T.insert(rc.T.end(), T7, T7 + 7);
  }
}

void SDVLBatch::RefreshRelocStore(const vector<int> &lost) {
  const int L = static_cast<int>(lost.size());
// ... 249 lines not shown
  ParallelFor(R, [&](int k) {
    SDVL &t = *trk_[s.run[k]];
    sdvl_track_job &jb = tr_jobs_[k];
    jb.tracker = s.run[k];
    jb.feat_buf = t.track_.feat_buf;
    jb.last = t.last_frame_->device();
    jb.cur = t.current_frame_->device();
    const SE3 T = t.current_frame_->GetPose() * t.last_frame_->GetPose().Inverse();
    T.ToArray(jb.T);
    t.last_frame_->GetPose().ToArray(jb.last_pose);
    jb.frame_id = t.current_frame_->GetID();
    jb.max_matches = t.feature_align_.MaxMatches();
    t.feature_align_.ShuffleCellRanks(tr_rank_.data() + static_cast<size_t>(k) * cells);
    t.feature_align_.PeekRand(max_its, tr_rand_.data() + static_cast<size_t>(k) * max_its);
  });
  sdvl_track_params prm;
  prm.align = AlignParams(false);
  prm.search = SearchParams();
  prm.pose = FeatureAlign::PoseParams(*trk_[0]->camera_);
  prm.cell_size = Config::CellSize();
  prm.patch_size = Config::PatchSize();
  prm.max_failed = Config::MaxFailed();
  prm.pad_ = 0;
  return prm;
}

void SDVLBatch::SubmitTracked(Step &s) {
  const int R = s.R();
  s.Stage(ST_IMAGE_ALIGN);
  const sdvl_track_params prm = AssembleTrackJobs(s);
  const sdvl_camera cam = trk_[0]->camera_->abi();
  const bool fork = !s.detected && trk_.size() <= 4;
  if (fork) dev_->Check(sdvl_ctx_fork_mark(dev_->ctx()), "sdvl_ctx_fork_mark");
  dev_->Check(sdvl_track_align(dev_->ctx(), track_, R, tr_jobs_.data(), tr_rank_.data(), tr_rand_.data(), &cam, &prm), "sdvl_track_align");
  if (!s.detected) {
    DetectOnSideStream(s.frames, fork);
    s.detected = true;
  }
  s.Stage(ST_SEARCH);
  dev_->Check(sdvl_track_search(dev_->ctx(), track_), "sdvl_track_search");
  QueueLookAhead(s);
  tr_res_.resize(R);
  dev_->Check(sdvl_track_collect(dev_->ctx(), track_, R, tr_res_.data()), "sdvl_track_collect");
}

void SDVLBatch::ReplayTracked(Step &s) {
  const int R = s.R();
  s.Stage(ST_FINISH);
  for (int k = 0; k < R; k++)
    if (tr_res_[k].status != 0) throw std::runtime_error("sdvl_track: a table capacity was exceeded on the device");
  ParallelFor(R, [&](int k) {
    const int i = s.run[k];
    SDVL &t = *trk_[i];
    FrameStats &st = s.stats[i];
    const sdvl_track_result &r = tr_res_[k];
    SDVL::TrackState &ts = t.track_;
    st.align_meas = r.align_meas;
    st.align_iters = r.align_iters;
    st.align_features = r.n_features;
    st.search_requests = r.n_requests;
    st.lk_iters = r.lk_iters;
    st.n_corners = r.n_corners;
    t.current_frame_->SetPose(SE3::FromArray(r.pose));
    t.current_frame_->SetRegistered();
    t.current_frame_->SetFlatFeatures(sdvl_track_features(track_, k), r.matches, ts.points);
    t.current_frame_->SetSceneDepthHint(r.scene_depth);
// ... 384 lines not shown
      Frame::DetectBatch(s.frames, Config::NumFeatures());
      s.detected = true;
    }
  s.Stage(ST_PRELUDE);
  for (int i = 0; i < B; i++) {
    const FrameStart start = BeginFrame(i, s.frames[i], stats[i]);
    stats[i].host_path = 1;
    if (start == kFirstFrame && trk_[i]->two_frame_init_) s.init.push_back(i);
    if (start == kFirstFrame || (start == kLost && !RelocalizeOnHost(*trk_[i], stats[i]))) continue;
    trk_[i]->SetMotionModel();
    s.run.push_back(i);
  }
  if (!s.init.empty()) InitializeTrackers(s);
  AlignImages(s);
  s.Stage(ST_PREPARE);
  scratch_reqs_.clear();
  s.chain_obs_begin.assign(s.run.size() + 1, 0);
  if (threads_ <= 1 && !s.run.empty()) {
    PackRequests(s);
    if (s.chain) PackChain(s);
  } else {
    CollectRequests(s);
  }
  LaunchSearch(s);
  ReplaySelect(s);
  LaunchPose(s);
  CommitAndSave(s);
  s.clk.reset();
  EpilogueAndMapper(s);
}

void SDVLBatch::FinishKeyframes(Step &s) {
  if (s.kfs.empty()) return;
  Frame::FilterCornersEnd(s.kfs, &pfor_ref_);
  vector<char> appended(s.kfs.size(), 0);
  ParallelFor(static_cast<int>(s.kfs.size()), [&](int k) {
    SDVL &t = *trk_[s.kf_owner[k]];
    PlaneMap *pm = dynamic_cast<PlaneMap *>(t.map_);
    if (pm) pm->SeedFromFiltered(s.kfs[k]);
    t.pending_kf_ = nullptr;
    if (t.track_.append_pending) {
      t.track_.append_pending = false;
      if (t.track_.valid && AppendSeeds(t, s.kfs[k])) appended[k] = 1;
      else t.track_.valid = false;
    }
  });
  vector<int> up;
  for (size_t k = 0; k < s.kfs.size(); k++)
    if (appended[k]) up.push_back(s.kf_owner[k]);
  GatherRows(up, true);
  if (!up.empty())
    dev_->Check(sdvl_track_append(dev_->ctx(), track_, static_cast<int>(up.size()), tr_up_trk_.data(), tr_up_buf_.data(), tr_up_np_.data(), tr_up_points_.data(),
                                  tr_up_nf_.data(), tr_up_feats_.data()), "sdvl_track_append");
}

void SDVLBatch::EpilogueAndMapper(Step &s) {
  s.Stage(ST_MAPPING);
  if (!s.filter_begun) {
    FetchCornerCounts(s.frames, s.stats);
    CollectKeyframes(s, false);
  }
  FinishKeyframes(s);
  s.Stage(ST_EPILOGUE);
  ParallelFor(static_cast<int>(trk_.size()), [&](int i) {
    SDVL &t = *trk_[i];
    FrameStats &st = s.stats[i];
    st.quality = static_cast<int>(t.tracking_quality_);
// ... 140 lines not shown
```

### slam-sdvl_amd/host/track_sequence.cc

```cpp
#include <algorithm>
#include <atomic>
#include <chrono>
#include <cstdio>
#include <cstdlib>
#include <cstring>
#include <fstream>
#include <iostream>
#include <memory>
#include <string>
#include <thread>
#include <vector>

#include "sdvl_host.h"
#undef SDVL_HD
#include "../csrc/sdvl_synth_scene.h"

extern "C" int sdvl_synth_render_host(const sdvl_synth_view *view, int width, int height, uint8_t *out, int stride);
extern "C" int sdvl_synth_render_scene_host(const sdvl_synth_scene *scene, int width, int height, uint8_t *out, int stride, float *depth, uint8_t *surface);

using namespace sdvl;

namespace {

bool ReadPNM(const std::string &path, int *w, int *h, std::vector<uint8_t> *px, int *format) {
// ... 4 lines not shown
  *format = magic == "P6" ? PIX_RGB8 : PIX_GRAY8;
  int vals[3], n = 0;
  while (n < 3) {
    f >> std::ws;
    if (f.peek() == '#') { std::string skip; std::getline(f, skip); continue; }
    if (!(f >> vals[n])) return false;
    n++;
  }
  if (vals[2] != 255) return false;
  f.get();
  *w = vals[0];
  *h = vals[1];
  px->resize(static_cast<size_t>(vals[0]) * vals[1] * channels);
  f.read(reinterpret_cast<char *>(px->data()), static_cast<std::streamsize>(px->size()));
  return static_cast<size_t>(f.gcount()) == px->size();
}

int RawFormatByName(const std::string &name) {
  static const char *const names[] = {"bayer_rggb", "bayer_grbg", "bayer_gbrg", "bayer_bggr", "yuyv", "uyvy", "gray10", "gray12", "gray16"};
  for (int i = 0; i < 9; i++)
    if (name == names[i]) return PIX_BAYER_RGGB8 + i;
  return 0;
}

const char kUsage[] =
    "track_sequence --synthetic N [--seed S] [--scene NAME] | --list frames.txt [--raw-format NAME]\n"
    "  --list: one binary PGM (P5, 8 bit) or PPM (P6, 8 bit RGB) path per line\n"
    "  --raw-format NAME: the P5 files are raw camera frames, converted to gray on the device:\n"
    "      bayer_rggb | bayer_grbg | bayer_gbrg | bayer_bggr   a Bayer mosaic, named by the 2x2 tile at its top-left corner\n"
    "      yuyv | uyvy                                         YUV 4:2:2; the P5 is 2 W bytes wide for a W-pixel frame\n"
    "      gray10 | gray12 | gray16                            little-endian 16-bit gray; the P5 is 2 W bytes wide\n"
    "    16-bit PGM (maxval above 255) is big-endian and is not supported\n"
    "  common: [--config file.cfg] [--size W H] [--cam fx fy u0 v0] [--dist d0 d1 d2 d3 d4] [--plane nx ny nz d] [--mapper] [--bundle]\n"
    "          [--init plane|two-frame] [--trackers N] [--batch] [--lookahead] [--prerender] [--pageable] [--set SDVL.key value]\n"
    "          [--quiet] [--json] [--profile]\n";

bool WrapListFrame(const uint8_t *data, int file_w, int W, int H, int format, int raw_format, Image *img) {
  if (format == PIX_GRAY8 && raw_format) format = raw_format;
  const int row = W * PixelFormatBytes(format);
  if (file_w != (format == PIX_RGB8 ? W : row)) return false;
  *img = Image::Wrap(data, W, H, row, format);
  return true;
}

}

int main(int argc, char **argv) {
  int W = 640, H = 480, n_synth = 0;
  unsigned seed = 20260001;
  double cam4[4] = {517.3, 516.5, 318.6, 255.3}, dist[5] = {0, 0, 0, 0, 0}, plane[4] = {0, 0, 1, 2.0};
  std::string list, cfg, scene_name;
  bool mapper = false, bundle = false, two_frame = false, size_given = false, cam_given = false, dist_given = false;
  bool prerender = false, pageable = false, quiet = false, json = false, profile = false, batch = false, lookahead = false;
  int n_trackers = 1, raw_format = 0;
  std::vector<std::pair<std::string, double>> sets;
  unsigned texture = SDVL_TEXTURE_PLANE_NOISE;
  for (int i = 1; i < argc; i++) {
    const std::string a = argv[i];
    auto need = [&](int k) { if (i + k >= argc) { std::cerr << "missing value after " << a << std::endl; std::exit(2); } };
    if (a == "--synthetic") { need(1); n_synth = std::atoi(argv[++i]); }
    else if (a == "--seed") { need(1); seed = static_cast<unsigned>(std::strtoul(argv[++i], nullptr, 10)); }
    else if (a == "--list") { need(1); list = argv[++i]; }
    else if (a == "--raw-format") { need(1); raw_format = RawFormatByName(argv[++i]); if (!raw_format) { std::cerr << "unknown --raw-format " << argv[i] << "\n" << kUsage; return 2; } }
    else if (a == "--help" || a == "-h") { std::cout << kUsage; return 0; }
    else if (a == "--config") { need(1); cfg = argv[++i]; }
    else if (a == "--size") { need(2); W = std::atoi(argv[++i]); H = std::atoi(argv[++i]); size_given = true; }
    else if (a == "--cam") { need(4); for (int k = 0; k < 4; k++) cam4[k] = std::atof(argv[++i]); cam_given = true; }
    else if (a == "--dist") { need(5); for (int k = 0; k < 5; k++) dist[k] = std::atof(argv[++i]); dist_given = true; }
    else if (a == "--plane") { need(4); for (int k = 0; k < 4; k++) plane[k] = std::atof(argv[++i]); }
    else if (a == "--mapper") mapper = true;
    else if (a == "--bundle") { bundle = true; mapper = true; }
    else if (a == "--init") { need(1); const std::string t = argv[++i]; if (t == "two-frame") { two_frame = true; mapper = true; } else if (t != "plane") { std::cerr << "unknown --init " << t << std::endl; return 2; } }
    else if (a == "--texture") { need(1); const std::string t = argv[++i]; if (t == "camera") texture = SDVL_TEXTURE_CAMERA; else if (t != "plane") { std::cerr << "unknown texture " << t << std::endl; return 2; } }
    else if (a == "--scene") { need(1); scene_name = argv[++i]; }
    else if (a == "--trackers") { need(1); n_trackers = std::max(1, std::atoi(argv[++i])); }
    else if (a == "--batch") batch = true;
    else if (a == "--lookahead") lookahead = true;
    else if (a == "--prerender") prerender = true;
    else if (a == "--pageable") pageable = true;
    else if (a == "--quiet") quiet = true;
    else if (a == "--json") json = true;
    else if (a == "--profile") profile = true;
    else if (a == "--set") { need(2); sets.emplace_back(argv[i + 1], std::atof(argv[i + 2])); i += 2; }
    else { std::cerr << "unknown argument " << a << std::endl; return 2; }
  }
  if ((n_synth > 0) == !list.empty()) { std::cerr << "give either --synthetic N or --list file" << std::endl; return 2; }
  if (raw_format && list.empty()) { std::cerr << "--raw-format says what the P5 files of a --list hold: give --list file" << std::endl; return 2; }
  sdvl_synth_scene scene_surfaces = {};
  if (!scene_name.empty()) {
    if (n_synth <= 0) { std::cerr << "--scene renders the synthetic sequence: give --synthetic N" << std::endl; return 2; }
    if (sdvl_synth_scene_preset(scene_name.c_str(), &scene_surfaces) != 0) {
      std::cerr << "unknown --scene " << scene_name << " (one of: " << sdvl_synth_scene_preset_names() << ")" << std::endl;
      return 2;
    }
  }
  const bool use_scene = !scene_name.empty();

  Config &c = Config::GetInstance();
  c.SetParameter("SDVL.cell_size", 32); c.SetParameter("SDVL.max_matches", 200); c.SetParameter("SDVL.use_orb", 1);
  c.SetParameter("SDVL.fast_threshold", 10); c.SetParameter("SDVL.num_features", 1000); c.SetParameter("SDVL.min_avg_shift", 5);
  c.SetParameter("SDVL.max_keyframes", 1000); c.SetParameter("SDVL.lost_ratio", 0.7);
  if (!cfg.empty()) {
    if (!c.ReadParameters(cfg)) { std::cerr << "cannot read " << cfg << std::endl; return 2; }
    const CameraParameters &cp = Config::GetCameraParameters();
    if (!size_given) { W = cp.width; H = cp.height; }
    if (!cam_given) { cam4[0] = cp.fx; cam4[1] = cp.fy; cam4[2] = cp.u0; cam4[3] = cp.v0; }
    if (!dist_given) { dist[0] = cp.d1; dist[1] = cp.d2; dist[2] = cp.d3; dist[3] = cp.d4; dist[4] = cp.d5; }
  }

  for (const auto &kv : sets)
// ... 63 lines not shown
      render_dev->Check(sdvl_device_malloc(rc, static_cast<int64_t>(frame_bytes * chunk), &dbuf), "sdvl_device_malloc");
      for (int k0 = 0; k0 < n_frames; k0 += chunk) {
        const int n = std::min(chunk, n_frames - k0);
        if (use_scene) {
          std::vector<sdvl_synth_scene> scenes;
          for (int k = k0; k < k0 + n; k++) scenes.push_back(scene_of(k));
          render_dev->Check(sdvl_synth_render_scene(rc, n, scenes.data(), W, H, dbuf, static_cast<int64_t>(frame_bytes), nullptr, nullptr), "sdvl_synth_render_scene");
        } else {
          std::vector<sdvl_synth_view> views;
          for (int k = k0; k < k0 + n; k++) views.push_back(view_of(k));
          render_dev->Check(sdvl_synth_render(rc, n, views.data(), W, H, dbuf, static_cast<int64_t>(frame_bytes)), "sdvl_synth_render");
        }
        render_dev->Check(sdvl_device_download(rc, dbuf, static_cast<int64_t>(frame_bytes * n), pool + frame_bytes * k0), "sdvl_device_download");
      }
      render_dev->Check(sdvl_device_free(rc, dbuf), "sdvl_device_free");
    }

    struct PerTracker { double busy = 0.0; int tracked = 0; std::vector<float> ms; std::string err; };
    std::vector<PerTracker> per(n_trackers);
    std::atomic<int> ready{0};
    std::atomic<bool> go{false};
    std::chrono::steady_clock::time_point t_go;
    auto run_tracker = [&](int id) {
      PerTracker &me = per[id];
      try {
        Device dev(0);
        Device::SetCurrent(&dev);
        Camera camera(W, H, cam4[0], cam4[1], cam4[2], cam4[3]);
        camera.SetDistortions(dist[0], dist[1], dist[2], dist[3], dist[4]);
        std::unique_ptr<Map> map;
        if (mapper) map.reset(new MapperMap(Vector3d(plane[0], plane[1], plane[2]), plane[3], &camera));
        else map.reset(new PlaneMap(Vector3d(plane[0], plane[1], plane[2]), plane[3]));
        SDVL sdvl(&camera, map.get());
        if (two_frame) sdvl.SetTwoFrameInit(true);
        if (bundle) sdvl.SetBundleAdjustment(true);
        std::vector<uint8_t> px(pool ? 0 : frame_bytes);
        me.ms.reserve(n_frames);
        Image ahead;
        bool ahead_valid = false;
        if (n_trackers > 1) {
          ready.fetch_add(1);
          while (!go.load(std::memory_order_acquire)) std::this_thread::yield();
        }
        for (int k = 0; k < n_frames; k++) {
          uint8_t *data = px.data();
          int format = PIX_GRAY8, file_w = W;
          if (pool) {
            data = pool + frame_bytes * k;
          } else if (n_synth > 0) {
            render_host(k, px.data());
          } else {
            int w = 0, h = 0;
            if (!ReadPNM(files[k], &w, &h, &px, &format) || h != H) {
              me.err = "cannot read " + files[k] + " as a binary PGM / PPM of the configured size";
              return;
            }
            data = px.data();
            file_w = w;
          }
          Image img;
          if (!WrapListFrame(data, file_w, W, H, format, raw_format, &img)) {
            me.err = "cannot read " + files[k] + " as a binary PGM / PPM of the configured size";
            return;
          }
          Image imgu;
          if (lookahead && pool && ahead_valid) {
// ... 160 lines not shown
```

### slam-sdvl_amd/tracker.py

```python
import ctypes as C
import os

import numpy as np

_HERE = os.path.dirname(os.path.abspath(__file__))
HOST_LIB_PATH = os.path.join(_HERE, "host", "libsdvl_host.so")


class FrameStats(C.Structure):
    _fields_ = [(n, C.c_int) for n in ("state", "quality", "matches", "attempts", "inliers", "outliers", "n_corners",
                                       "align_meas", "keyframe", "relocalized")] + [("pose", C.c_double * 7)] + [
        (n, C.c_int) for n in ("align_features", "align_iters", "search_requests", "lk_iters", "host_path")]


_lib = None


def load_host_library():
    global _lib
    if _lib is None:
        if not os.path.exists(HOST_LIB_PATH):
            raise RuntimeError("libsdvl_host.so is not built (%s): run __graft_entry__.build()" % HOST_LIB_PATH)
        lib = C.CDLL(HOST_LIB_PATH)
        lib.sdvlh_last_error.restype = C.c_char_p
# ... 99 lines not shown
class TrackerBatch:
    def __init__(self, dev, B, w, h, cam4, plane4=(0, 0, 1, 2.0), first_poses=None, host_threads=1):
        self.lib = dev.lib
        self.dev = dev
        self.B, self.w, self.h_img = B, w, h
        self.channels = 1
        cam4 = np.ascontiguousarray(cam4, np.float64)
        plane4 = np.ascontiguousarray(plane4, np.float64)
        if first_poses is None:
            first_poses = np.tile(np.array([1, 0, 0, 0, 0, 0, 0], np.float64), (B, 1))
        first_poses = np.ascontiguousarray(first_poses, np.float64).reshape(B, 7)
        self.h = self.lib.sdvlh_batch_create(dev.h, B, w, h, cam4.ctypes.data, plane4.ctypes.data, first_poses.ctypes.data, host_threads)
        if not self.h:
            raise RuntimeError(self.lib.sdvlh_last_error().decode())
        self._stats = (FrameStats * B)()

    def step_host(self, imgs):
        imgs = [np.ascontiguousarray(im, "<u2").view(np.uint8) if np.asarray(im).dtype == np.uint16 else np.ascontiguousarray(im, np.uint8) for im in imgs]
        ptrs = (C.c_void_p * self.B)(*[im.ctypes.data for im in imgs])
        if self.lib.sdvlh_batch_step_host(self.h, ptrs, self.w * self.channels, self._stats) != 0:
            raise RuntimeError(self.lib.sdvlh_last_error().decode())
        return self._stats

    def step_device(self, dev_ptrs):
        ptrs = (C.c_void_p * self.B)(*[int(p) for p in dev_ptrs])
        if self.lib.sdvlh_batch_step_device(self.h, ptrs, self.w * self.channels, self._stats) != 0:
            raise RuntimeError(self.lib.sdvlh_last_error().decode())
        return self._stats

    def set_next_device(self, dev_ptrs):
        ptrs = (C.c_void_p * self.B)(*[int(p) for p in dev_ptrs]) if dev_ptrs is not None else None
        if self.lib.sdvlh_batch_set_next_device(self.h, ptrs, self.w * self.channels) != 0:
            raise RuntimeError(self.lib.sdvlh_last_error().decode())

    def set_distortion(self, dist5):
        d = np.ascontiguousarray(dist5, np.float64)
        self.lib.sdvlh_batch_set_distortion.argtypes = [C.c_void_p, C.c_void_p]
        if self.lib.sdvlh_batch_set_distortion(self.h, d.ctypes.data) != 0:
            raise RuntimeError("sdvlh_batch_set_distortion")

    def set_color(self, fmt):
        code = pixel_format(fmt)
        self.lib.sdvlh_batch_set_color.argtypes = [C.c_void_p, C.c_int]
        if self.lib.sdvlh_batch_set_color(self.h, code) != 0:
            raise RuntimeError(self.lib.sdvlh_last_error().decode())
        self.channels = PIXEL_CHANNELS[code]

    def set_two_frame_init(self, on=True):
        self.lib.sdvlh_batch_set_two_frame_init.argtypes = [C.c_void_p, C.c_int]
        if self.lib.sdvlh_batch_set_two_frame_init(self.h, int(bool(on))) != 0:
            raise RuntimeError(self.lib.sdvlh_last_error().decode())

    def set_bundle_adjustment(self, on=True):
        self.lib.sdvlh_batch_set_bundle_adjustment.argtypes = [C.c_void_p, C.c_int]
        if self.lib.sdvlh_batch_set_bundle_adjustment(self.h, int(bool(on))) != 0:
            raise RuntimeError(self.lib.sdvlh_last_error().decode())

    def bundle_stats(self, i):
        from . import BundleResult
        counts = (C.c_longlong * 6)()
        last = BundleResult()
        self.lib.sdvlh_batch_bundle_stats.argtypes = [C.c_void_p, C.c_int, C.c_void_p, C.c_void_p]
        if self.lib.sdvlh_batch_bundle_stats(self.h, int(i), counts, C.byref(last)) != 0:
            raise RuntimeError("tracker %d has no mapper" % i)
        out = dict(zip(("runs", "skipped", "n_free", "n_fixed", "n_points", "n_edges"), [int(c) for c in counts]))
        out["last"] = last
# ... 148 lines not shown
```

Measured before the change: 460,400.

## Chain speculative keyframe corner filtering into the tracked GPU step

Predicts on the device whether each tracker will take a keyframe and, for predicted keyframes, runs Shi-Tomasi scoring, binned cell selection and descriptor computation inside the tracking chain. The results are pulled to host memory. On the host, a chained result is accepted only if the predicted lock mask matches the real one. Otherwise it falls back to the separate filter pass. This removes the second filter launch-and-wait round trip for keyframes, at the cost of wasted speculative GPU work and extra complexity. It is enabled by default only for batches of more than four trackers.

```diff
diff --git a/include/sdvl_hip.h b/include/sdvl_hip.h
--- a/include/sdvl_hip.h
+++ b/include/sdvl_hip.h
@@ -422,6 +422,30 @@
 int sdvl_track_collect(sdvl_ctx *ctx, sdvl_track_set *set, int n_jobs, sdvl_track_result *results);
 const sdvl_track_feature_out *sdvl_track_features(const sdvl_track_set *set, int job);
 const sdvl_track_point_stat *sdvl_track_stats(const sdvl_track_set *set, int job);
+
+typedef struct sdvl_track_kf_job {
+  int32_t eligible;
+  int32_t last_kf_id;
+  int32_t last_matches;
+  int32_t pad_;
+} sdvl_track_kf_job;
+typedef struct sdvl_track_kf_params {
+  double lost_ratio;
+  int32_t min_matches;
+  int32_t min_keyframe_its;
+  int32_t margin;
+  int32_t min_feature_score;
+} sdvl_track_kf_params;
+typedef struct sdvl_track_kf_result {
+  int32_t decision;
+  int32_t last_matches;
+  int32_t served;
+  int32_t count;
+} sdvl_track_kf_result;
+int sdvl_track_keyframe_filter(sdvl_ctx *ctx, sdvl_track_set *set, int n_jobs, const sdvl_track_kf_job *jobs, const sdvl_track_kf_params *p);
+int sdvl_track_keyframe_result(const sdvl_track_set *set, int job, sdvl_track_kf_result *out, const uint32_t **mask, int32_t *mask_words,
+                               const sdvl_filtered_corner **records);
+int sdvl_keyframe_predict(sdvl_ctx *ctx, int n, const int32_t *in6, const sdvl_track_kf_params *p, int32_t *out2);
 
 typedef struct sdvl_klt_job {
   const sdvl_frame *prev, *next;
diff --git a/slam-sdvl_amd/__init__.py b/slam-sdvl_amd/__init__.py
--- a/slam-sdvl_amd/__init__.py
+++ b/slam-sdvl_amd/__init__.py
@@ -147,6 +147,7 @@
     "sdvl_frame_download_descriptors", "sdvl_filter_inputs", "sdvl_filter_inputs_begin", "sdvl_filter_inputs_end", "sdvl_filter_corners_begin", "sdvl_filter_corners_end", "sdvl_orb_describe_points", "sdvl_hamming_argmin", "sdvl_image_align", "sdvl_image_align_begin", "sdvl_image_align_end", "sdvl_align_store_create", "sdvl_align_store_destroy", "sdvl_align_store_write", "sdvl_image_align_begin_stored", "sdvl_search_points", "sdvl_search_begin", "sdvl_search_slot", "sdvl_search_run", "sdvl_align_patches", "sdvl_pose_from_matches", "sdvl_search_points_filter", "sdvl_search_run_filter", "sdvl_depth_filter", "sdvl_search_run_chain", "sdvl_search_chain_end", "sdvl_frame_footprint", "sdvl_undistort", "sdvl_frames_upload_undistorted", "sdvl_convert_gray", "sdvl_frames_upload_color", "sdvl_ctx_set_wait_hook", "sdvl_ctx_wait_done", "sdvl_ctx_wait_block", "sdvl_ctx_health", "sdvl_ctx_counters",
     "sdvl_track_create", "sdvl_track_destroy", "sdvl_frame_register", "sdvl_frames_register", "sdvl_track_upload", "sdvl_track_append", "sdvl_track_align", "sdvl_track_search",
     "sdvl_track_collect", "sdvl_track_features", "sdvl_track_stats",
+    "sdvl_track_keyframe_filter", "sdvl_track_keyframe_result", "sdvl_keyframe_predict",
     "sdvl_synth_render", "sdvl_synth_render_scene", "sdvl_synth_scene_size", "sdvl_synth_scene_preset", "sdvl_synth_scene_preset_names",
     "sdvl_device_malloc", "sdvl_device_free", "sdvl_device_download",
     "sdvl_frames_own_images", "sdvl_feed_create", "sdvl_feed_destroy", "sdvl_feed_last_error", "sdvl_feed_slot_arrived", "sdvl_feed_images", "sdvl_ctx_feed_acquire", "sdvl_ctx_feed_release", "sdvl_frame_footprint_cap", "sdvl_ctx_set_corner_capacity", "sdvl_frame_corner_capacity", "sdvl_detect_scratch_bytes",
@@ -370,6 +371,19 @@
     _fields_ = [("score", C.c_int32), ("n_failed", C.c_int32), ("last_frame", C.c_int32), ("status", C.c_int32)]
 
 
+class TrackKfJob(C.Structure):
+    _fields_ = [("eligible", C.c_int32), ("last_kf_id", C.c_int32), ("last_matches", C.c_int32), ("pad_", C.c_int32)]
+
+
+class TrackKfParams(C.Structure):
+    _fields_ = [("lost_ratio", C.c_double), ("min_matches", C.c_int32), ("min_keyframe_its", C.c_int32), ("margin", C.c_int32),
+                ("min_feature_score", C.c_int32)]
+
+
+class TrackKfResult(C.Structure):
+    _fields_ = [("decision", C.c_int32), ("last_matches", C.c_int32), ("served", C.c_int32), ("count", C.c_int32)]
+
+
 class TrackSet:
 
     def __init__(self, ctx, n_trackers, max_points, max_features, grid_cells, max_matches, max_ransac_its):
@@ -402,6 +416,19 @@
     def append(self, trackers, feat_buf, points, features):
         for t, k in zip(*self._rows(self.ctx.lib.sdvl_track_append, trackers, feat_buf, points, features)):
             self.n_points[t] = self.n_points.get(t, 0) + k
+
+    def keyframe_filter(self, kf_jobs, kf_params):
+        n = 0 if kf_jobs is None else len(kf_jobs)
+        self.ctx._check(self.ctx.lib.sdvl_track_keyframe_filter(self.ctx.h, self.h, n, kf_jobs, C.byref(kf_params) if n else None))
+
+    def keyframe_result(self, job):
+        lib = self.ctx.lib
+        r, mask, recs, words = TrackKfResult(), C.POINTER(C.c_uint32)(), C.c_void_p(), C.c_int32()
+        lib.sdvl_track_keyframe_result.argtypes = [C.c_void_p, C.c_int, C.c_void_p, C.c_void_p, C.c_void_p, C.c_void_p]
+        self.ctx._check(lib.sdvl_track_keyframe_result(self.h, int(job), C.byref(r), C.byref(mask), C.byref(words), C.byref(recs)))
+        m = np.ctypeslib.as_array(mask, (words.value,)).copy()
+        rec = np.ctypeslib.as_array(C.cast(recs, i32p), (self.cells, 14)).copy()
+        return r, m, rec
 
     def step(self, jobs, cell_rank, rand_raw, cam, params, between=None):
         n = len(jobs)
@@ -789,6 +816,12 @@
                             outliers=lists[b + res[k].n_inliers:b + res[k].n_inliers + res[k].n_outliers].copy()))
         return out
 
+    def keyframe_predict(self, rows, kf_params):
+        rows = np.ascontiguousarray(rows, np.int32).reshape(-1, 6)
+        out = np.zeros((len(rows), 2), np.int32)
+        self._check(self.lib.sdvl_keyframe_predict(self.h, len(rows), _ptr(rows, i32p), C.byref(kf_params), _ptr(out, i32p)))
+        return out
+
     def track_set(self, n_trackers, max_points, max_features, grid_cells, max_matches, max_ransac_its):
         return TrackSet(self, n_trackers, max_points, max_features, grid_cells, max_matches, max_ransac_its)
 
diff --git a/slam-sdvl_amd/csrc/sdvl_orb.hip b/slam-sdvl_amd/csrc/sdvl_orb.hip
--- a/slam-sdvl_amd/csrc/sdvl_orb.hip
+++ b/slam-sdvl_amd/csrc/sdvl_orb.hip
@@ -3,6 +3,7 @@
 
 #include "sdvl_internal.h"
 #include "sdvl_orb_device.h"
+#include "sdvl_search_types.h"
 
 namespace {
 
@@ -60,12 +61,9 @@
 }
 
 constexpr int kShiPerWave = 4;
-__global__ __launch_bounds__(256) void shi_tomasi_kernel(const OrbJob *__restrict__ jobs, int n_jobs, int chunks) {
-  int fj, bx;
-  if (!xcd_frame_block(n_jobs, chunks, &fj, &bx)) return;
-  const OrbJob &job = jobs[fj];
+template <class View>
+__device__ __forceinline__ void shi_tomasi_corners(const View &job, int n, double *__restrict__ out_score, int bx, int chunks) {
   const int lane = threadIdx.x & 63, grp = lane >> 4, q = lane & 15;
-  const int n = job.n_ptr ? min(job.n_ptr[0], SDVL_MAX_CORNERS) : job.n;
   const int wpb = static_cast<int>(blockDim.x >> 6);
   for (int c0 = (bx * wpb + (threadIdx.x >> 6)) * kShiPerWave; c0 < n; c0 += chunks * wpb * kShiPerWave) {
     const int ci = c0 + grp;
@@ -116,10 +114,16 @@
           const float disc = (dXX + dYY) * (dXX + dYY) - 4 * (dXX * dYY - dXY * dXY);
           score = 0.5 * (dXX + dYY - sqrt(static_cast<double>(disc)));
         }
-        job.out_score[ci] = score;
+        out_score[ci] = score;
       }
     }
   }
+}
+__global__ __launch_bounds__(256) void shi_tomasi_kernel(const OrbJob *__restrict__ jobs, int n_jobs, int chunks) {
+  int fj, bx;
+  if (!xcd_frame_block(n_jobs, chunks, &fj, &bx)) return;
+  const OrbJob &job = jobs[fj];
+  shi_tomasi_corners(job, job.n_ptr ? min(job.n_ptr[0], SDVL_MAX_CORNERS) : job.n, job.out_score, bx, chunks);
 }
 inline int shi_chunks(int max_n) { return (max_n + kShiPerWave - 1) / kShiPerWave; }
 
@@ -200,16 +204,16 @@
 constexpr int kBinCellsSmall = 512, kBinCornersSmall = 2048;
 constexpr int kBinCellsLarge = SDVL_MAX_LEVEL_CELLS, kBinSlotsLarge = 4;
 
-template <int kCells, int kCorners, int kSlots = kBinSlots>
-__global__ __launch_bounds__(256) void filter_select_binned_kernel(const FilterJob *__restrict__ jobs, int cell_size, int grid_w, int n_cells,
-                                                                   int margin, int min_score, int max_out) {
+template <int kCells, int kCorners, int kSlots, class View>
+__device__ __forceinline__ void filter_select_binned_cells(const View &job, const double *__restrict__ scores, const uint32_t *__restrict__ locked,
+                                                           sdvl_filtered_corner *__restrict__ out, int32_t *__restrict__ out_count, int ccap,
+                                                           int cell_size, int grid_w, int n_cells, int margin, int min_score, int max_out) {
   __shared__ uint16_t s_cell[kCorners];
   __shared__ uint16_t s_list[kCells * kSlots];
   __shared__ int s_cnt[kCells];
   __shared__ int s_wave[4];
-  const FilterJob &job = jobs[blockIdx.x];
   const int tid = threadIdx.x, lane = tid & 63, wave = tid >> 6;
-  const int n = min(min(job.n_ptr[0], job.ccap), kCorners);
+  const int n = min(min(job.n_ptr[0], ccap), kCorners);
   for (int c = tid; c < n_cells; c += 256) s_cnt[c] = 0;
   __syncthreads();
   for (int i = tid; i < n; i += 256) {
@@ -218,7 +222,7 @@
     if (level >= 0 && level < job.levels && !(px < margin || py < margin || px >= job.lw[level] - margin || py >= job.lh[level] - margin)) {
       const int scale = 1 << level;
       const int pos = ((py * scale) / cell_size) * grid_w + (px * scale) / cell_size;
-      if (pos >= 0 && pos < n_cells && !((job.locked[pos >> 5] >> (pos & 31)) & 1u)) {
+      if (pos >= 0 && pos < n_cells && !((locked[pos >> 5] >> (pos & 31)) & 1u)) {
         c = static_cast<uint16_t>(pos);
         const int slot = atomicAdd(&s_cnt[pos], 1);
         if (slot < kSlots) s_list[pos * kSlots + slot] = static_cast<uint16_t>(i);
@@ -245,7 +249,7 @@
 #pragma unroll
       for (int q = 0; q < kSlots; q++) {
         if (q >= cnt) break;
-        const double score = job.scores[idx[q]];
+        const double score = scores[idx[q]];
         if (score > best) {
           best_idx = idx[q];
           best = static_cast<int>(score);
@@ -254,7 +258,7 @@
     } else {
       for (int i = 0; i < n; i++) {
         if (s_cell[i] != c) continue;
-        const double score = job.scores[i];
+        const double score = scores[i];
         if (score > best) {
           best_idx = i;
           best = static_cast<int>(score);
@@ -277,26 +281,31 @@
     for (int w = 0; w < wave; w++) pos += s_wave[w];
     if (ok && pos < max_out) {
       const int i = s_cnt[c];
-      sdvl_filtered_corner *dst = job.out + pos;
+      sdvl_filtered_corner *dst = out + pos;
       dst->index = i;
       dst->x = job.corners[4 * i]; dst->y = job.corners[4 * i + 1]; dst->level = job.corners[4 * i + 2];
-      dst->score = static_cast<int>(job.scores[i]);
+      dst->score = static_cast<int>(scores[i]);
       dst->pad_ = 0;
     }
     running += s_wave[0] + s_wave[1] + s_wave[2] + s_wave[3];
   }
-  if (tid == 0) job.out_count[0] = running;
-}
-
-__global__ __launch_bounds__(256) void filter_describe_kernel(const FilterJob *__restrict__ jobs, int max_out, int n_jobs, int chunks) {
-  int fj, bx;
-  if (!xcd_frame_block(n_jobs, chunks, &fj, &bx)) return;
-  const FilterJob &job = jobs[fj];
+  if (tid == 0) out_count[0] = running;
+}
+
+template <int kCells, int kCorners, int kSlots = kBinSlots>
+__global__ __launch_bounds__(256) void filter_select_binned_kernel(const FilterJob *__restrict__ jobs, int cell_size, int grid_w, int n_cells,
+                                                                   int margin, int min_score, int max_out) {
+  const FilterJob &job = jobs[blockIdx.x];
+  filter_select_binned_cells<kCells, kCorners, kSlots>(job, job.scores, job.locked, job.out, job.out_count, job.ccap, cell_size, grid_w, n_cells,
+                                                       margin, min_score, max_out);
+}
+
+template <class View>
+__device__ __forceinline__ void filter_describe_corners(const View &job, sdvl_filtered_corner *__restrict__ out, int total, int bx, int chunks) {
   const int lane = threadIdx.x & 63;
-  const int total = min(job.out_count[0], max_out);
   const int wpb = static_cast<int>(blockDim.x >> 6);
   for (int k = bx * wpb + (threadIdx.x >> 6); k < total; k += chunks * wpb) {
-    sdvl_filtered_corner *dst = job.out + k;
+    sdvl_filtered_corner *dst = out + k;
     const int cx = dst->x, cy = dst->y, cl = dst->level;
     const int W = job.lw[cl], H = job.lh[cl];
     uint8_t byte = 0;
@@ -308,6 +317,61 @@
     }
     if ((lane & 1) == 0) dst->desc[lane >> 1] = byte;
   }
+}
+__global__ __launch_bounds__(256) void filter_describe_kernel(const FilterJob *__restrict__ jobs, int max_out, int n_jobs, int chunks) {
+  int fj, bx;
+  if (!xcd_frame_block(n_jobs, chunks, &fj, &bx)) return;
+  const FilterJob &job = jobs[fj];
+  filter_describe_corners(job, job.out, min(job.out_count[0], max_out), bx, chunks);
+}
+
+__global__ __launch_bounds__(256) void shi_tomasi_track_kernel(const TrackJobDev *__restrict__ jobs, const sdvl_track_kf_result *__restrict__ pred,
+                                                               double *__restrict__ scores, int ccap, int n_jobs, int chunks) {
+  int fj, bx;
+  if (!xcd_frame_block(n_jobs, chunks, &fj, &bx)) return;
+  if (pred[fj].decision != 2) return;
+  const SearchFrame &v = jobs[fj].cur;
+  shi_tomasi_corners(v, min(v.n_ptr[0], ccap), scores + static_cast<size_t>(fj) * ccap, bx, chunks);
+}
+
+template <int kCells, int kCorners>
+__global__ __launch_bounds__(256) void filter_select_binned_track_kernel(const TrackJobDev *__restrict__ jobs, sdvl_track_kf_result *__restrict__ pred,
+                                                                         const double *__restrict__ scores, int ccap, const uint32_t *__restrict__ mask,
+                                                                         int mask_words, sdvl_filtered_corner *__restrict__ recs, int cell_size, int grid_w,
+                                                                         int n_cells, int margin, int min_score, int max_out) {
+  const int j = blockIdx.x;
+  if (pred[j].decision != 2) return;
+  const SearchFrame &v = jobs[j].cur;
+  if (v.n_ptr[0] > min(ccap, kCorners)) return;
+  filter_select_binned_cells<kCells, kCorners, kBinSlots>(v, scores + static_cast<size_t>(j) * ccap, mask + static_cast<size_t>(j) * mask_words,
+                                                          recs + static_cast<size_t>(j) * max_out, &pred[j].count, ccap, cell_size, grid_w, n_cells,
+                                                          margin, min_score, max_out);
+  if (threadIdx.x == 0) pred[j].served = 1;
+}
+
+__global__ __launch_bounds__(256) void filter_describe_track_kernel(const TrackJobDev *__restrict__ jobs, const sdvl_track_kf_result *__restrict__ pred,
+                                                                    sdvl_filtered_corner *__restrict__ recs, int max_out, int n_jobs, int chunks) {
+  int fj, bx;
+  if (!xcd_frame_block(n_jobs, chunks, &fj, &bx)) return;
+  const sdvl_track_kf_result p = pred[fj];
+  if (p.decision != 2 || !p.served) return;
+  filter_describe_corners(jobs[fj].cur, recs + static_cast<size_t>(fj) * max_out, min(p.count, max_out), bx, chunks);
+}
+
+static_assert(sizeof(sdvl_filtered_corner) % 8 == 0, "keyframe_pull copies records in 8-byte units");
+__global__ __launch_bounds__(256) void keyframe_pull_kernel(const sdvl_track_kf_result *__restrict__ pred, const uint32_t *__restrict__ mask, int mask_words,
+                                                            const sdvl_filtered_corner *__restrict__ recs, int max_out,
+                                                            sdvl_track_kf_result *__restrict__ h_pred, uint32_t *__restrict__ h_mask,
+                                                            sdvl_filtered_corner *__restrict__ h_recs) {
+  const int j = blockIdx.x, tid = threadIdx.x;
+  const sdvl_track_kf_result p = pred[j];
+  if (tid == 0) h_pred[j] = p;
+  if (p.decision != 2 || !p.served) return;
+  for (int w = tid; w < mask_words; w += 256) h_mask[static_cast<size_t>(j) * mask_words + w] = mask[static_cast<size_t>(j) * mask_words + w];
+  const uint2 *src = reinterpret_cast<const uint2 *>(recs + static_cast<size_t>(j) * max_out);
+  uint2 *dst = reinterpret_cast<uint2 *>(h_recs + static_cast<size_t>(j) * max_out);
+  const int units = min(p.count, max_out) * static_cast<int>(sizeof(sdvl_filtered_corner) / 8);
+  for (int u = tid; u < units; u += 256) dst[u] = src[u];
 }
 
 __global__ __launch_bounds__(256) void filter_gather_kernel(const OrbJob *__restrict__ jobs, uint4 *__restrict__ dst, int row_units, int ccap,
@@ -392,6 +456,29 @@
     job.best[2 * q] = found ? static_cast<int>(key & 0xffffffffull) : -1;
     job.best[2 * q + 1] = d;
   }
+}
+
+int sdvl_keyframe_filter_enqueue(sdvl_ctx *ctx, int n_jobs, const KeyframeChain &k) {
+  SDVL_REQUIRE(ctx, k.n_cells >= 1 && k.n_cells <= kBinCells && k.max_out == k.n_cells && k.mask_words * 32 >= k.n_cells && k.ccap >= 1 &&
+                        k.ccap <= kFilterMaxCorners,
+               "keyframe filter inside the tracked step: grids of up to 2048 cells");
+  const int chunks = 64;
+  SDVL_LAUNCH(ctx, "shi_tomasi_track", shi_tomasi_track_kernel, xcd_frame_grid(n_jobs, chunks), dim3(64), k.jobs, static_cast<const sdvl_track_kf_result *>(k.pred),
+              k.scores, k.ccap, n_jobs, chunks);
+  if (k.n_cells <= kBinCellsSmall)
+    SDVL_LAUNCH(ctx, "filter_select_track", (filter_select_binned_track_kernel<kBinCellsSmall, kBinCornersSmall>), dim3(n_jobs), dim3(256), k.jobs, k.pred,
+                static_cast<const double *>(k.scores), k.ccap, static_cast<const uint32_t *>(k.mask), k.mask_words, k.recs, k.cell_size, k.grid_w, k.n_cells,
+                k.margin, k.min_score, k.max_out);
+  else
+    SDVL_LAUNCH(ctx, "filter_select_track", (filter_select_binned_track_kernel<kBinCells, kFilterMaxCorners>), dim3(n_jobs), dim3(256), k.jobs, k.pred,
+                static_cast<const double *>(k.scores), k.ccap, static_cast<const uint32_t *>(k.mask), k.mask_words, k.recs, k.cell_size, k.grid_w, k.n_cells,
+                k.margin, k.min_score, k.max_out);
+  SDVL_LAUNCH(ctx, "filter_describe_track", filter_describe_track_kernel, xcd_frame_grid(n_jobs, chunks), dim3(64), k.jobs,
+              static_cast<const sdvl_track_kf_result *>(k.pred), k.recs, k.max_out, n_jobs, chunks);
+  SDVL_LAUNCH(ctx, "keyframe_pull", keyframe_pull_kernel, dim3(n_jobs), dim3(256), static_cast<const sdvl_track_kf_result *>(k.pred),
+              static_cast<const uint32_t *>(k.mask), k.mask_words, static_cast<const sdvl_filtered_corner *>(k.recs), k.max_out, k.h_pred, k.h_mask, k.h_recs);
+  SDVL_HIP_CHECK(ctx, hipGetLastError());
+  return SDVL_OK;
 }
 
 extern "C" {
diff --git a/slam-sdvl_amd/csrc/sdvl_search_types.h b/slam-sdvl_amd/csrc/sdvl_search_types.h
--- a/slam-sdvl_amd/csrc/sdvl_search_types.h
+++ b/slam-sdvl_amd/csrc/sdvl_search_types.h
@@ -179,6 +179,19 @@
 int sdvl_image_align_track_enqueue(sdvl_ctx *ctx, int n_jobs, const TrackJobDev *d_jobs, const TrackPoint *d_points, const TrackFeat *d_feats0,
                                    const TrackFeat *d_feats1, int np, int nfeat_cap, int max_nf, int levels, const sdvl_camera *cam,
                                    const sdvl_align_params *p, sdvl_align_result *d_results, int batch_size);
+struct KeyframeChain {
+  const TrackJobDev *jobs;
+  sdvl_track_kf_result *pred;
+  double *scores;
+  uint32_t *mask;
+  sdvl_filtered_corner *recs;
+  int ccap, mask_words, max_out;
+  int cell_size, grid_w, n_cells, margin, min_score;
+  sdvl_track_kf_result *h_pred;
+  uint32_t *h_mask;
+  sdvl_filtered_corner *h_recs;
+};
+int sdvl_keyframe_filter_enqueue(sdvl_ctx *ctx, int n_jobs, const KeyframeChain &k);
 extern "C" int sdvl_ensure_nits_table(sdvl_ctx *ctx, int npoints_cfg, int max_its, int max_size);
 
 #endif
diff --git a/slam-sdvl_amd/csrc/sdvl_track.hip b/slam-sdvl_amd/csrc/sdvl_track.hip
--- a/slam-sdvl_amd/csrc/sdvl_track.hip
+++ b/slam-sdvl_amd/csrc/sdvl_track.hip
@@ -52,6 +52,32 @@
   uint4 *df = reinterpret_cast<uint4 *>((r.feat_buf ? feats1 : feats0) + static_cast<size_t>(r.tracker) * nf + r.feat_dst);
   const int fw = r.n_feat * static_cast<int>(sizeof(TrackFeat) / 16);
   for (int i = threadIdx.x; i < fw; i += 256) df[i] = sf[i];
+}
+
+__device__ __forceinline__ void keyframe_predict(int matches, int attempts, int npoints, int frame_id, int last_kf_id, int last_matches,
+                                                 const sdvl_track_kf_params &kp, int *decision, int *last_matches_out) {
+  *last_matches_out = last_matches;
+  const double ratio = (attempts == 0) ? 0.0 : static_cast<double>(matches) / static_cast<double>(attempts);
+  if (!(ratio > 0.2)) {
+    *decision = matches < kp.min_matches ? 0 : 1;
+    return;
+  }
+  const bool enough_its = (frame_id - last_kf_id) >= kp.min_keyframe_its;
+  const bool lost_many = npoints < last_matches * kp.lost_ratio;
+  const bool lost_some = npoints < last_matches * 0.9;
+  const bool kf = (enough_its && lost_some) || lost_many;
+  *last_matches_out = kf ? npoints : (last_matches > npoints ? last_matches : npoints);
+  *decision = kf ? 2 : 1;
+}
+
+__global__ __launch_bounds__(64) void keyframe_predict_kernel(const int32_t *__restrict__ in6, int n, sdvl_track_kf_params kp, int32_t *__restrict__ out2) {
+  const int i = blockIdx.x * 64 + threadIdx.x;
+  if (i >= n) return;
+  const int32_t *r = in6 + 6 * i;
+  int d, lm;
+  keyframe_predict(r[0], r[1], r[2], r[3], r[4], r[5], kp, &d, &lm);
+  out2[2 * i] = d;
+  out2[2 * i + 1] = lm;
 }
 
 constexpr int kProjThreads = 512;
@@ -206,14 +232,17 @@
                                                            const sdvl_pose_result *__restrict__ pres, const int32_t *__restrict__ lists,
                                                            const sdvl_align_result *__restrict__ ares, Cam cam, int max_failed,
                                                            SearchFramePose *__restrict__ registry, sdvl_track_result *__restrict__ h_results,
-                                                           sdvl_track_feature_out *__restrict__ h_feats, sdvl_track_point_stat *__restrict__ h_stats) {
+                                                           sdvl_track_feature_out *__restrict__ h_feats, sdvl_track_point_stat *__restrict__ h_stats,
+                                                           const sdvl_track_kf_job *__restrict__ kf_in, sdvl_track_kf_params kp,
+                                                           sdvl_track_kf_result *__restrict__ kf_pred, uint32_t *__restrict__ kf_mask,
+                                                           int mask_words, int cell_size, int grid_w, int grid_cells) {
   extern __shared__ __attribute__((aligned(16))) uint8_t s_dyn[];
   const CommitLds lds(stride, mm);
   uint16_t *s_before = reinterpret_cast<uint16_t *>(s_dyn);
   uint8_t *s_found = s_dyn + lds.found;
   double *s_depth = reinterpret_cast<double *>(s_dyn + lds.depth);
   __shared__ int s_wave[4];
-  __shared__ int s_attempts, s_deleted, s_lk, s_npoints;
+  __shared__ int s_attempts, s_deleted, s_lk, s_npoints, s_decision;
   __shared__ double s_median;
   const int j = blockIdx.x, tid = threadIdx.x, lane = tid & 63, wave = tid >> 6;
   const TrackJobDev &jb = jobs[j];
@@ -361,6 +390,27 @@
 #pragma unroll
     for (int q = 0; q < 7; q++) registry[jb.cur_id].pose[q] = pr.pose[q];
   }
+  if (!kf_in) return;
+  if (tid == 0) {
+    const sdvl_track_kf_job in = kf_in[j];
+    sdvl_track_kf_result r;
+    r.decision = -1;
+    r.last_matches = in.last_matches;
+    r.served = 0;
+    r.count = 0;
+    if (in.eligible) keyframe_predict(matches, s_attempts, s_npoints, jb.frame_id, in.last_kf_id, in.last_matches, kp, &r.decision, &r.last_matches);
+    kf_pred[j] = r;
+    s_decision = r.decision;
+  }
+  __syncthreads();
+  if (s_decision != 2) return;
+  uint32_t *mask = kf_mask + static_cast<size_t>(j) * mask_words;
+  for (int w = tid; w < mask_words; w += 256) mask[w] = 0u;
+  __syncthreads();
+  for (int r = tid; r < matches; r += 256) {
+    const int index = static_cast<int>(N[r].px[1] / cell_size) * grid_w + static_cast<int>(N[r].px[0] / cell_size);
+    if (index >= 0 && index < grid_cells) atomicOr(&mask[index >> 5], 1u << (index & 31));
+  }
 }
 
 }
@@ -385,6 +435,20 @@
   sdvl_part<sdvl_pose_obs> obs;
   sdvl_part<uint8_t> hyp;
   sdvl_part<sdvl_pose_result> pres;
+  sdvl_part<sdvl_track_kf_job> kfin;
+  uint8_t *d_kf = nullptr;
+  sdvl_part<sdvl_track_kf_result> kf_pred;
+  sdvl_part<uint32_t> kf_mask;
+  sdvl_part<double> kf_scores;
+  sdvl_part<sdvl_filtered_corner> kf_recs;
+  uint8_t *h_kf = nullptr;
+  sdvl_part<sdvl_track_kf_result> hkf_pred;
+  sdvl_part<uint32_t> hkf_mask;
+  sdvl_part<sdvl_filtered_corner> hkf_recs;
+  int kf_words = 0;
+  std::vector<sdvl_track_kf_job> kf_jobs;
+  sdvl_track_kf_params kf_prm = {};
+  bool kf_step = false;
   uint8_t *h_pinned = nullptr;
   sdvl_track_result *h_results;
   sdvl_track_feature_out *h_feats;
@@ -425,6 +489,7 @@
   if (e == hipSuccess) e = hipMalloc(reinterpret_cast<void **>(&s->d_feats[1]), sizeof(TrackFeat) * NF);
   sdvl_layout L;
   s->djobs = L.take<TrackJobDev>(N);
+  s->kfin = L.take<sdvl_track_kf_job>(N);
   s->cell_rank = L.take<uint16_t>(N * s->cells);
   s->rand = L.take<int32_t>(N * s->max_its);
   s->ares = L.take<sdvl_align_result>(N);
@@ -483,6 +548,8 @@
   if (s->d_feats[0]) (void)hipFree(s->d_feats[0]);
   if (s->d_feats[1]) (void)hipFree(s->d_feats[1]);
   if (s->d_scratch) (void)hipFree(s->d_scratch);
+  if (s->d_kf) (void)hipFree(s->d_kf);
+  if (s->h_kf) (void)hipHostFree(s->h_kf);
   if (s->h_pinned) (void)hipHostFree(s->h_pinned);
   delete s;
   return SDVL_OK;
@@ -641,6 +708,10 @@
     memcpy(d.T0, a.T, sizeof(double) * 7);
     d.pad2_ = 0.0;
   }
+  s->kf_step = static_cast<int>(s->kf_jobs.size()) == n_jobs;
+  memset(s->kfin.in(hs), 0, s->kfin.bytes());
+  if (s->kf_step) memcpy(s->kfin.in(hs), s->kf_jobs.data(), sizeof(sdvl_track_kf_job) * static_cast<size_t>(n_jobs));
+  s->kf_jobs.clear();
   memcpy(s->cell_rank.in(hs), cell_rank, sizeof(uint16_t) * static_cast<size_t>(n_jobs) * s->cells);
   memcpy(s->rand.in(hs), rand_raw, rand_bytes);
   SDVL_HIP_CHECK(ctx, sdvl_push(ctx, s->d_scratch, hs, head_bytes));
@@ -707,8 +778,32 @@
   SDVL_LAUNCH_LDS(ctx, "track_commit", track_commit_kernel, dim3(n_jobs), dim3(256), CommitLds(stride, s->mm).bytes, s->djobs.cin(D), s->d_points,
                   static_cast<const TrackFeat *>(s->d_feats[0]), static_cast<const TrackFeat *>(s->d_feats[1]), s->d_feats[0], s->d_feats[1], s->np,
                   s->nf, stride, s->mm, s->chain.cin(D), s->cfirst.cin(D), s->cfeat.cin(D), s->res.cin(D), s->pres.cin(D), s->lists.cin(D),
-                  s->ares.cin(D), c, s->prm.max_failed, registry, s->h_results, s->h_feats, s->h_stats);
+                  s->ares.cin(D), c, s->prm.max_failed, registry, s->h_results, s->h_feats, s->h_stats,
+                  s->kf_step ? s->kfin.cin(D) : nullptr, s->kf_prm, s->kf_step ? s->kf_pred.in(s->d_kf) : nullptr,
+                  s->kf_step ? s->kf_mask.in(s->d_kf) : nullptr, s->kf_words, s->prm.cell_size,
+                  static_cast<int>(ceil(s->cam.width / s->prm.cell_size)), s->cells);
   SDVL_HIP_CHECK(ctx, hipGetLastError());
+  if (s->kf_step) {
+    KeyframeChain k;
+    k.jobs = s->djobs.cin(D);
+    k.pred = s->kf_pred.in(s->d_kf);
+    k.scores = s->kf_scores.in(s->d_kf);
+    k.mask = s->kf_mask.in(s->d_kf);
+    k.recs = s->kf_recs.in(s->d_kf);
+    k.ccap = SDVL_MAX_CORNERS;
+    k.mask_words = s->kf_words;
+    k.max_out = s->cells;
+    k.cell_size = s->prm.cell_size;
+    k.grid_w = (s->jobs[0].cur->width + s->prm.cell_size - 1) / s->prm.cell_size;
+    k.n_cells = s->cells;
+    k.margin = s->kf_prm.margin;
+    k.min_score = s->kf_prm.min_feature_score;
+    k.h_pred = s->hkf_pred.in(s->h_kf);
+    k.h_mask = s->hkf_mask.in(s->h_kf);
+    k.h_recs = s->hkf_recs.in(s->h_kf);
+    rc = sdvl_keyframe_filter_enqueue(ctx, n_jobs, k);
+    if (rc) return rc;
+  }
   SDVL_HIP_CHECK(ctx, sdvl_mark_record(ctx, SDVL_MARK_CHAIN, &s->ticket));
   s->phase = 2;
   return SDVL_OK;
@@ -737,4 +832,70 @@
   return (s && job >= 0 && job < s->n) ? s->h_stats + static_cast<size_t>(job) * s->np : nullptr;
 }
 
-}
+int sdvl_track_keyframe_filter(sdvl_ctx *ctx, sdvl_track_set *s, int n_jobs, const sdvl_track_kf_job *jobs, const sdvl_track_kf_params *p) {
+  if (!ctx || !s || s->ctx != ctx || n_jobs < 0) return SDVL_ERR_INVALID;
+  SDVL_REQUIRE(ctx, s->phase == 0, "sdvl_track_keyframe_filter while a step is in flight");
+  s->kf_jobs.clear();
+  if (n_jobs == 0 || !jobs) return SDVL_OK;
+  SDVL_REQUIRE(ctx, p != nullptr && n_jobs <= s->n, "keyframe inputs: null parameters or more jobs than trackers");
+  SDVL_REQUIRE(ctx, s->cells <= 2048, "keyframe filter inside the tracked step: grids of up to 2048 cells");
+  SDVL_REQUIRE(ctx, p->margin >= 0 && p->min_keyframe_its >= 0, "bad keyframe parameters");
+  if (!s->d_kf) {
+    SDVL_HIP_CHECK(ctx, sdvl_bind_device(ctx));
+    const size_t N = static_cast<size_t>(s->n);
+    s->kf_words = (s->cells + 31) / 32;
+    sdvl_layout L, H;
+    s->kf_pred = L.take<sdvl_track_kf_result>(N);
+    s->kf_mask = L.take<uint32_t>(N * s->kf_words);
+    s->kf_recs = L.take<sdvl_filtered_corner>(N * s->cells);
+    s->kf_scores = L.take<double>(N * SDVL_MAX_CORNERS);
+    s->hkf_pred = H.take<sdvl_track_kf_result>(N);
+    s->hkf_mask = H.take<uint32_t>(N * s->kf_words);
+    s->hkf_recs = H.take<sdvl_filtered_corner>(N * s->cells);
+    hipError_t e = hipMalloc(reinterpret_cast<void **>(&s->d_kf), L.bytes());
+    if (e == hipSuccess) e = hipHostMalloc(reinterpret_cast<void **>(&s->h_kf), H.bytes(), hipHostMallocDefault);
+    if (e != hipSuccess) {
+      if (s->d_kf) (void)hipFree(s->d_kf);
+      s->d_kf = nullptr;
+      ctx->err = std::string("sdvl_track_keyframe_filter: ") + hipGetErrorString(e);
+      return SDVL_ERR_HIP;
+    }
+    memset(s->h_kf, 0, H.bytes());
+  }
+  s->kf_prm = *p;
+  s->kf_jobs.assign(jobs, jobs + n_jobs);
+  return SDVL_OK;
+}
+
+int sdvl_track_keyframe_result(const sdvl_track_set *s, int job, sdvl_track_kf_result *out, const uint32_t **mask, int32_t *mask_words,
+                               const sdvl_filtered_corner **records) {
+  if (!s || !out || job < 0 || job >= s->n || !s->kf_step || !s->h_kf || s->phase != 0) return SDVL_ERR_INVALID;
+  *out = s->hkf_pred.cin(s->h_kf)[job];
+  if (mask) *mask = s->hkf_mask.cin(s->h_kf) + static_cast<size_t>(job) * s->kf_words;
+  if (mask_words) *mask_words = s->kf_words;
+  if (records) *records = s->hkf_recs.cin(s->h_kf) + static_cast<size_t>(job) * s->cells;
+  return SDVL_OK;
+}
+
+int sdvl_keyframe_predict(sdvl_ctx *ctx, int n, const int32_t *in6, const sdvl_track_kf_params *p, int32_t *out2) {
+  if (!ctx || n < 0 || (n > 0 && (!in6 || !out2)) || !p) return SDVL_ERR_INVALID;
+  if (n == 0) return SDVL_OK;
+  SDVL_HIP_CHECK(ctx, sdvl_bind_device(ctx));
+  const size_t in_bytes = sizeof(int32_t) * 6 * static_cast<size_t>(n), out_bytes = sizeof(int32_t) * 2 * static_cast<size_t>(n);
+  void *hs = nullptr, *dsx = nullptr;
+  int rc = sdvl_ensure(ctx, &ctx->d_out, &ctx->d_out_bytes, out_bytes, false);
+  if (!rc) rc = sdvl_ensure(ctx, &ctx->h_out, &ctx->h_out_bytes, out_bytes, true);
+  if (!rc) rc = sdvl_stage_alloc(ctx, in_bytes, &hs, &dsx);
+  if (rc) return rc;
+  memcpy(hs, in6, in_bytes);
+  SDVL_HIP_CHECK(ctx, sdvl_push(ctx, dsx, hs, in_bytes));
+  SDVL_LAUNCH(ctx, "keyframe_predict", keyframe_predict_kernel, dim3((n + 63) / 64), dim3(64), static_cast<const int32_t *>(dsx), n, *p,
+              static_cast<int32_t *>(ctx->d_out));
+  SDVL_HIP_CHECK(ctx, hipGetLastError());
+  SDVL_HIP_CHECK(ctx, hipMemcpyAsync(ctx->h_out, ctx->d_out, out_bytes, hipMemcpyDeviceToHost, ctx->stream));
+  SDVL_HIP_CHECK(ctx, sdvl_stream_wait(ctx));
+  memcpy(out2, ctx->h_out, out_bytes);
+  return SDVL_OK;
+}
+
+}
diff --git a/slam-sdvl_amd/host/capi.cc b/slam-sdvl_amd/host/capi.cc
--- a/slam-sdvl_amd/host/capi.cc
+++ b/slam-sdvl_amd/host/capi.cc
@@ -186,6 +186,30 @@
   return rc ? -2 : n;
 }
 
+int sdvlh_batch_set_chained_keyframe_filter(void *bp, int on) {
+  if (!bp) return -1;
+  return Guarded([&] { AsGroup(bp)->batch().SetChainedKeyframeFilter(on != 0); });
+}
+int sdvlh_batch_keyframe_filter_counts(void *bp, long long *out3) {
+  if (!bp || !out3) return -1;
+  return Guarded([&] { AsGroup(bp)->batch().KeyframeFilterCounts(out3); });
+}
+int sdvlh_batch_force_keyframe_misprediction(void *bp, int i) {
+  if (!bp || i < 0 || i >= AsGroup(bp)->size()) return -1;
+  return Guarded([&] { AsGroup(bp)->batch().ForceKeyframeMisprediction(i); });
+}
+
+int sdvlh_batch_restart_tracker(void *bp, int i) {
+  if (!bp || i < 0 || i >= AsGroup(bp)->size()) return -1;
+  return Guarded([&] { AsGroup(bp)->tracker(i).Restart(); });
+}
+
+void sdvlh_tracking_decision(int matches, int attempts, int npoints, int frame_id, int last_kf_id, int last_matches, int *out2) {
+  const SDVL::TrackingQuality q = SDVL::QualityOf(matches, attempts);
+  out2[0] = q == SDVL::TRACKING_BAD ? 0 : ((q == SDVL::TRACKING_GOOD && Map::KeyframeRule(npoints, frame_id - last_kf_id, &last_matches)) ? 2 : 1);
+  out2[1] = last_matches;
+}
+
 void sdvlh_set_device_pose(int on) { SDVLBatch::SetDevicePose(on != 0); }
 int sdvlh_device_pose() { return SDVLBatch::DevicePose() ? 1 : 0; }
 
diff --git a/slam-sdvl_amd/host/frontend.cc b/slam-sdvl_amd/host/frontend.cc
--- a/slam-sdvl_amd/host/frontend.cc
+++ b/slam-sdvl_amd/host/frontend.cc
@@ -621,13 +621,26 @@
   for (int i = 0; i < n; i++) {
     Frame &f = *frames[i];
     devs[i] = f.dev_;
-    f.ForEachFeaturePosition([&](double px, double py) {
-      const int index = static_cast<int>(py / cell) * gw + static_cast<int>(px / cell);
-      if (index >= 0 && index < gw * gh) locked[static_cast<size_t>(i) * words + (index >> 5)] |= 1u << (index & 31);
-    });
+    f.LockMask(cell, gw, gh, locked.data() + static_cast<size_t>(i) * words);
   }
   dev->Check(sdvl_filter_corners_begin(dev->ctx(), n, devs.data(), locked.data(), words, cell, DetectMargin(), Config::MinFeatureScore(),
                                        Config::UseORB() ? 1 : 0), "sdvl_filter_corners_begin");
+}
+
+void Frame::LockMask(int cell, int gw, int gh, uint32_t *mask) const {
+  std::fill(mask, mask + (gw * gh + 31) / 32, 0u);
+  ForEachFeaturePosition([&](double px, double py) {
+    const int index = static_cast<int>(py / cell) * gw + static_cast<int>(px / cell);
+    if (index >= 0 && index < gw * gh) mask[index >> 5] |= 1u << (index & 31);
+  });
+}
+
+int Frame::FilterMargin() { return DetectMargin(); }
+
+void Frame::SetFiltered(const sdvl_filtered_corner *recs, int n) {
+  filt_.assign(recs, recs + n);
+  filtered_corners_.resize(n);
+  for (int k = 0; k < n; k++) filtered_corners_[k] = filt_[k].index;
 }
 
 void Frame::FilterCornersEnd(const vector<shared_ptr<Frame>> &frames, const std::function<void(int, const std::function<void(int)> &)> *pfor) {
@@ -644,10 +657,7 @@
   dev->Check(sdvl_filter_corners_end(dev->ctx(), n, cap, counts.data(), recs.data()), "sdvl_filter_corners_end");
   (void)pfor;
   for (int i = 0; i < n; i++) {
-    Frame &f = *frames[i];
-    f.filt_.assign(recs.begin() + static_cast<size_t>(i) * cap, recs.begin() + static_cast<size_t>(i) * cap + counts[i]);
-    f.filtered_corners_.resize(counts[i]);
-    for (int k = 0; k < counts[i]; k++) f.filtered_corners_[k] = f.filt_[k].index;
+    frames[i]->SetFiltered(recs.data() + static_cast<size_t>(i) * cap, counts[i]);
   }
 }
 
diff --git a/slam-sdvl_amd/host/frontend.h b/slam-sdvl_amd/host/frontend.h
--- a/slam-sdvl_amd/host/frontend.h
+++ b/slam-sdvl_amd/host/frontend.h
@@ -209,6 +209,9 @@
   static void FilterCornersBegin(const std::vector<std::shared_ptr<Frame>> &frames);
   static void FilterCornersEnd(const std::vector<std::shared_ptr<Frame>> &frames,
                                const std::function<void(int, const std::function<void(int)> &)> *pfor = nullptr);
+  void LockMask(int cell, int gw, int gh, uint32_t *mask) const;
+  void SetFiltered(const sdvl_filtered_corner *recs, int n);
+  static int FilterMargin();
   static void DetectBatch(const std::vector<std::shared_ptr<Frame>> &frames, int nfeatures);
   SE3 &GetPose() { return pose_; }
   const SE3 &GetPose() const { return pose_; }
diff --git a/slam-sdvl_amd/host/frontend_deps.h b/slam-sdvl_amd/host/frontend_deps.h
--- a/slam-sdvl_amd/host/frontend_deps.h
+++ b/slam-sdvl_amd/host/frontend_deps.h
@@ -134,6 +134,7 @@
   virtual void Stop() {}
   void DeletePoint(const std::shared_ptr<Point> &p) { points_trash_.push_back(p); version_++; }
   bool NeedKeyframe(const std::shared_ptr<Frame> &frame, int matches);
+  static bool KeyframeRule(int npoints, int its_since_kf, int *last_matches);
   virtual void AddKeyframe(const std::shared_ptr<Frame> &frame, bool search = true);
   virtual void AddFrame(const std::shared_ptr<Frame> &) {}
   virtual void LimitKeyframes(const std::shared_ptr<Frame> &) {}
@@ -142,6 +143,8 @@
   bool TakeTablesDirty() { const bool d = tables_dirty_; tables_dirty_ = false; return d; }
   std::vector<std::shared_ptr<Frame>> &GetKeyframes() { return keyframes_; }
   unsigned long long Version() const { return version_; }
+  const std::shared_ptr<Frame> &LastKeyframe() const { return last_kf_; }
+  int LastMatches() const { return last_matches_; }
   void Touch() { version_++; }
   virtual void InitCandidates(const std::shared_ptr<Frame> &) {}
 
diff --git a/slam-sdvl_amd/host/sdvl_host.h b/slam-sdvl_amd/host/sdvl_host.h
--- a/slam-sdvl_amd/host/sdvl_host.h
+++ b/slam-sdvl_amd/host/sdvl_host.h
@@ -127,6 +127,9 @@
   void SetNextImage(const Image &next);
   SE3 GetPose() const;
   TrackingQuality GetTrackingQuality() const { return tracking_quality_; }
+  void Restart();
+  void SetChainedKeyframeFilter(bool on);
+  static TrackingQuality QualityOf(int matches, int attempts);
   bool HasMap() { return state_ == STATE_RUNNING; }
   const FrameStats &LastStats() const { return stats_; }
   Map *GetMap() { return map_; }
@@ -165,6 +168,7 @@
   FrameStats stats_;
   bool relocalize_pending_ = false;
   std::unique_ptr<SDVLBatch> self_batch_;
+  int self_chained_kf_ = -1;
   std::vector<Image> next_image_;
   void SyncSelfBatch();
   struct TrackState {
@@ -202,6 +206,9 @@
   static void SetTrackTables(bool on);
   static bool TrackTables();
   void SyncHostState();
+  void SetChainedKeyframeFilter(bool on) { chained_kf_ = on ? 1 : 0; }
+  void KeyframeFilterCounts(long long out3[3]) const { out3[0] = kf_chained_; out3[1] = kf_fallback_; out3[2] = kf_second_waits_; }
+  void ForceKeyframeMisprediction(int tracker) { kf_force_ = tracker; }
 
  private:
   void ParallelFor(int n, const std::function<void(int)> &fn);
@@ -238,6 +245,8 @@
   void QueueLookAhead(const Step &s);
   void RelocalizeIntoStep(Step &s);
   sdvl_track_params AssembleTrackJobs(const Step &s);
+  void ArmKeyframeFilter(Step &s);
+  bool TakeChainedKeyframe(Frame &frame, int job);
   void SubmitTracked(Step &s);
   void ReplayTracked(Step &s);
   void SaveTrackedFrames(Step &s);
@@ -255,6 +264,11 @@
   std::vector<uint16_t> tr_rank_;
   std::vector<int32_t> tr_rand_;
   std::vector<sdvl_track_result> tr_res_;
+  std::vector<sdvl_track_kf_job> tr_kf_;
+  std::vector<uint32_t> kf_mask_;
+  int chained_kf_ = -1;
+  int kf_force_ = -1;
+  long long kf_chained_ = 0, kf_fallback_ = 0, kf_second_waits_ = 0;
   std::vector<sdvl_track_point> tr_up_points_;
   std::vector<sdvl_track_feature> tr_up_feats_;
   std::vector<int32_t> tr_up_trk_, tr_up_buf_, tr_up_np_, tr_up_nf_;
diff --git a/slam-sdvl_amd/host/standalone.cc b/slam-sdvl_amd/host/standalone.cc
--- a/slam-sdvl_amd/host/standalone.cc
+++ b/slam-sdvl_amd/host/standalone.cc
@@ -169,13 +169,16 @@
 }
 
 bool Map::NeedKeyframe(const shared_ptr<Frame> &frame, int) {
-  const int npoints = frame->GetNumPoints();
-  const bool enough_its = (frame->GetID() - last_kf_->GetID()) >= Config::MinKeyframeIts();
-  const bool lost_many = npoints < last_matches_ * Config::LostRatio();
-  const bool lost_some = npoints < last_matches_ * 0.9;
-  last_matches_ = std::max(last_matches_, npoints);
+  return KeyframeRule(frame->GetNumPoints(), frame->GetID() - last_kf_->GetID(), &last_matches_);
+}
+
+bool Map::KeyframeRule(int npoints, int its_since_kf, int *last_matches) {
+  const bool enough_its = its_since_kf >= Config::MinKeyframeIts();
+  const bool lost_many = npoints < *last_matches * Config::LostRatio();
+  const bool lost_some = npoints < *last_matches * 0.9;
+  *last_matches = std::max(*last_matches, npoints);
   if ((enough_its && lost_some) || lost_many) {
-    last_matches_ = npoints;
+    *last_matches = npoints;
     return true;
   }
   return false;
@@ -358,20 +361,17 @@
   return SE3();
 }
 
+SDVL::TrackingQuality SDVL::QualityOf(int matches, int attempts) {
+  const double ratio = (attempts == 0) ? 0.0 : static_cast<double>(matches) / static_cast<double>(attempts);
+  if (ratio > 0.2) return TRACKING_GOOD;
+  if (matches < Config::MinMatches()) return TRACKING_BAD;
+  return TRACKING_INSUFFICIENT;
+}
+
 void SDVL::CalcTrackingQuality(int matches, int attempts) {
-  const double ratio = (attempts == 0) ? 0.0 : static_cast<double>(matches) / static_cast<double>(attempts);
-  if (ratio > 0.2) {
-    tracking_quality_ = TRACKING_GOOD;
-    lost_frames_ = 0;
-    return;
-  }
-  if (matches < Config::MinMatches()) {
-    tracking_quality_ = TRACKING_BAD;
-    lost_frames_++;
-    return;
-  }
-  lost_frames_ = 0;
-  tracking_quality_ = TRACKING_INSUFFICIENT;
+  tracking_quality_ = QualityOf(matches, attempts);
+  if (tracking_quality_ == TRACKING_BAD) lost_frames_++;
+  else lost_frames_ = 0;
 }
 
 void SDVL::SetMotionModel() { current_frame_->SetPose(SE3::Exp(vel_) * last_frame_->GetPose()); }
@@ -397,6 +397,18 @@
   track_.valid = false;
   st.state = 0;
   st.keyframe = 1;
+}
+
+void SDVL::SetChainedKeyframeFilter(bool on) {
+  self_chained_kf_ = on ? 1 : 0;
+  if (self_batch_) self_batch_->SetChainedKeyframeFilter(on);
+}
+
+void SDVL::Restart() {
+  state_ = STATE_FIRST_FRAME;
+  lost_frames_ = 0;
+  ResetMotionModel();
+  track_.valid = false;
 }
 
 void SDVL::SetBundleAdjustment(bool on) {
@@ -498,6 +510,7 @@
   if (!self_batch_ || self_batch_->dev_ != dev) {
     if (self_batch_) self_batch_->SyncHostState();
     self_batch_.reset(new SDVLBatch(dev, {this}, 1));
+    if (self_chained_kf_ >= 0) self_batch_->SetChainedKeyframeFilter(self_chained_kf_ != 0);
     track_.valid = false;
   }
   if (!next_image_.empty()) {
@@ -866,6 +879,8 @@
   vector<char> decision;
   vector<shared_ptr<Frame>> kfs;
   vector<int> kf_owner;
+  vector<shared_ptr<Frame>> kf_rest;
+  bool kf_armed = false;
   bool filter_begun = false;
   bool detected = false;
   std::unique_ptr<StageClock> clk;
@@ -987,16 +1002,79 @@
 void SDVLBatch::CollectKeyframes(Step &s, bool fetch_counts) {
   s.kfs.clear();
   s.kf_owner.clear();
+  s.kf_rest.clear();
+  vector<int> job_of(trk_.size(), -1);
+  if (s.kf_armed)
+    for (size_t k = 0; k < s.run.size(); k++)
+      if (tr_kf_[k].eligible) job_of[s.run[k]] = static_cast<int>(k);
   for (size_t i = 0; i < trk_.size(); i++) {
     const bool fresh = s.decision[i] == 2 && !dynamic_cast<MapperMap *>(trk_[i]->map_);
-    if (trk_[i]->pending_kf_) { s.kfs.push_back(trk_[i]->pending_kf_); s.kf_owner.push_back(static_cast<int>(i)); }
-    else if (fresh) { s.kfs.push_back(trk_[i]->current_frame_); s.kf_owner.push_back(static_cast<int>(i)); }
+    if (trk_[i]->pending_kf_) {
+      s.kfs.push_back(trk_[i]->pending_kf_);
+      s.kf_owner.push_back(static_cast<int>(i));
+      s.kf_rest.push_back(trk_[i]->pending_kf_);
+    } else if (fresh) {
+      s.kfs.push_back(trk_[i]->current_frame_);
+      s.kf_owner.push_back(static_cast<int>(i));
+      if (job_of[i] >= 0 && TakeChainedKeyframe(*trk_[i]->current_frame_, job_of[i])) {
+        kf_chained_++;
+      } else {
+        if (job_of[i] >= 0) kf_fallback_++;
+        s.kf_rest.push_back(trk_[i]->current_frame_);
+      }
+    }
   }
   if (s.kfs.empty()) return;
   std::unique_ptr<StageClock> nested(s.clk->id != ST_MAPPING ? new StageClock(ST_MAPPING) : nullptr);
   if (fetch_counts) FetchCornerCounts(s.frames, s.stats);
-  Frame::FilterCornersBegin(s.kfs);
+  if (!s.kf_rest.empty()) {
+    Frame::FilterCornersBegin(s.kf_rest);
+    kf_second_waits_++;
+  }
   s.filter_begun = true;
+}
+
+bool SDVLBatch::TakeChainedKeyframe(Frame &frame, int job) {
+  sdvl_track_kf_result r;
+  const uint32_t *mask = nullptr;
+  const sdvl_filtered_corner *recs = nullptr;
+  int32_t words = 0;
+  if (sdvl_track_keyframe_result(track_, job, &r, &mask, &words, &recs) != SDVL_OK) return false;
+  if (r.decision != 2 || !r.served) return false;
+  const int cell = Config::CellSize();
+  const int gw = static_cast<int>(std::ceil(static_cast<double>(frame.GetWidth()) / cell));
+  const int gh = static_cast<int>(std::ceil(static_cast<double>(frame.GetHeight()) / cell));
+  if (words != (gw * gh + 31) / 32 || r.count < 0 || r.count > gw * gh) return false;
+  kf_mask_.resize(words);
+  frame.LockMask(cell, gw, gh, kf_mask_.data());
+  if (std::memcmp(kf_mask_.data(), mask, sizeof(uint32_t) * static_cast<size_t>(words)) != 0) return false;
+  frame.SetFiltered(recs, r.count);
+  return true;
+}
+
+void SDVLBatch::ArmKeyframeFilter(Step &s) {
+  s.kf_armed = false;
+  const int forced = kf_force_;
+  kf_force_ = -1;
+  if (chained_kf_ == 0 || (chained_kf_ < 0 && trk_.size() <= 4) || track_cells_ > 2048) return;
+  const int cell = Config::CellSize();
+  const Frame &f0 = *s.frames[s.run[0]];
+  const int gw = static_cast<int>(std::ceil(static_cast<double>(f0.GetWidth()) / cell));
+  const int gh = static_cast<int>(std::ceil(static_cast<double>(f0.GetHeight()) / cell));
+  if (gw * gh != track_cells_) return;
+  const int R = s.R();
+  tr_kf_.assign(R, sdvl_track_kf_job{0, 0, 0, 0});
+  bool any = false;
+  for (int k = 0; k < R; k++) {
+    const SDVL &t = *trk_[s.run[k]];
+    if (dynamic_cast<MapperMap *>(t.map_) || !t.map_->LastKeyframe()) continue;
+    tr_kf_[k] = sdvl_track_kf_job{1, t.map_->LastKeyframe()->GetID(), s.run[k] == forced ? 0 : t.map_->LastMatches(), 0};
+    any = true;
+  }
+  if (!any) return;
+  const sdvl_track_kf_params kp = {Config::LostRatio(), Config::MinMatches(), Config::MinKeyframeIts(), Frame::FilterMargin(), Config::MinFeatureScore()};
+  dev_->Check(sdvl_track_keyframe_filter(dev_->ctx(), track_, R, tr_kf_.data(), &kp), "sdvl_track_keyframe_filter");
+  s.kf_armed = true;
 }
 
 static std::atomic<unsigned long long> g_reloc_epoch{1};
@@ -1312,6 +1390,7 @@
   const sdvl_camera cam = trk_[0]->camera_->abi();
   const bool fork = !s.detected && trk_.size() <= 4;
   if (fork) dev_->Check(sdvl_ctx_fork_mark(dev_->ctx()), "sdvl_ctx_fork_mark");
+  ArmKeyframeFilter(s);
   dev_->Check(sdvl_track_align(dev_->ctx(), track_, R, tr_jobs_.data(), tr_rank_.data(), tr_rand_.data(), &cam, &prm), "sdvl_track_align");
   if (!s.detected) {
     DetectOnSideStream(s.frames, fork);
@@ -1762,7 +1841,7 @@
 
 void SDVLBatch::FinishKeyframes(Step &s) {
   if (s.kfs.empty()) return;
-  Frame::FilterCornersEnd(s.kfs, &pfor_ref_);
+  Frame::FilterCornersEnd(s.kf_rest, &pfor_ref_);
   vector<char> appended(s.kfs.size(), 0);
   ParallelFor(static_cast<int>(s.kfs.size()), [&](int k) {
     SDVL &t = *trk_[s.kf_owner[k]];
diff --git a/slam-sdvl_amd/host/track_sequence.cc b/slam-sdvl_amd/host/track_sequence.cc
--- a/slam-sdvl_amd/host/track_sequence.cc
+++ b/slam-sdvl_amd/host/track_sequence.cc
@@ -60,7 +60,7 @@
     "      gray10 | gray12 | gray16                            little-endian 16-bit gray; the P5 is 2 W bytes wide\n"
     "    16-bit PGM (maxval above 255) is big-endian and is not supported\n"
     "  common: [--config file.cfg] [--size W H] [--cam fx fy u0 v0] [--dist d0 d1 d2 d3 d4] [--plane nx ny nz d] [--mapper] [--bundle]\n"
-    "          [--init plane|two-frame] [--trackers N] [--batch] [--lookahead] [--prerender] [--pageable] [--set SDVL.key value]\n"
+    "          [--init plane|two-frame] [--trackers N] [--batch] [--lookahead] [--chained-keyframes on|off] [--prerender] [--pageable] [--set SDVL.key value]\n"
     "          [--quiet] [--json] [--profile]\n";
 
 bool WrapListFrame(const uint8_t *data, int file_w, int W, int H, int format, int raw_format, Image *img) {
@@ -80,6 +80,7 @@
   std::string list, cfg, scene_name;
   bool mapper = false, bundle = false, two_frame = false, size_given = false, cam_given = false, dist_given = false;
   bool prerender = false, pageable = false, quiet = false, json = false, profile = false, batch = false, lookahead = false;
+  int chained_kf = -1;
   int n_trackers = 1, raw_format = 0;
   std::vector<std::pair<std::string, double>> sets;
   unsigned texture = SDVL_TEXTURE_PLANE_NOISE;
@@ -104,6 +105,7 @@
     else if (a == "--trackers") { need(1); n_trackers = std::max(1, std::atoi(argv[++i])); }
     else if (a == "--batch") batch = true;
     else if (a == "--lookahead") lookahead = true;
+    else if (a == "--chained-keyframes") { need(1); chained_kf = std::string(argv[++i]) == "on" ? 1 : 0; }
     else if (a == "--prerender") prerender = true;
     else if (a == "--pageable") pageable = true;
     else if (a == "--quiet") quiet = true;
@@ -233,6 +235,7 @@
         if (mapper) map.reset(new MapperMap(Vector3d(plane[0], plane[1], plane[2]), plane[3], &camera));
         else map.reset(new PlaneMap(Vector3d(plane[0], plane[1], plane[2]), plane[3]));
         SDVL sdvl(&camera, map.get());
+        if (chained_kf >= 0) sdvl.SetChainedKeyframeFilter(chained_kf != 0);
         if (two_frame) sdvl.SetTwoFrameInit(true);
         if (bundle) sdvl.SetBundleAdjustment(true);
         std::vector<uint8_t> px(pool ? 0 : frame_bytes);
diff --git a/slam-sdvl_amd/tracker.py b/slam-sdvl_amd/tracker.py
--- a/slam-sdvl_amd/tracker.py
+++ b/slam-sdvl_amd/tracker.py
@@ -155,6 +155,28 @@
         ptrs = (C.c_void_p * self.B)(*[int(p) for p in dev_ptrs]) if dev_ptrs is not None else None
         if self.lib.sdvlh_batch_set_next_device(self.h, ptrs, self.w * self.channels) != 0:
             raise RuntimeError(self.lib.sdvlh_last_error().decode())
+
+    def set_chained_keyframe_filter(self, on=True):
+        self.lib.sdvlh_batch_set_chained_keyframe_filter.argtypes = [C.c_void_p, C.c_int]
+        if self.lib.sdvlh_batch_set_chained_keyframe_filter(self.h, int(bool(on))) != 0:
+            raise RuntimeError(self.lib.sdvlh_last_error().decode())
+
+    def keyframe_filter_counts(self):
+        out = (C.c_longlong * 3)()
+        self.lib.sdvlh_batch_keyframe_filter_counts.argtypes = [C.c_void_p, C.c_void_p]
+        if self.lib.sdvlh_batch_keyframe_filter_counts(self.h, out) != 0:
+            raise RuntimeError(self.lib.sdvlh_last_error().decode())
+        return int(out[0]), int(out[1]), int(out[2])
+
+    def force_keyframe_misprediction(self, i):
+        self.lib.sdvlh_batch_force_keyframe_misprediction.argtypes = [C.c_void_p, C.c_int]
+        if self.lib.sdvlh_batch_force_keyframe_misprediction(self.h, int(i)) != 0:
+            raise RuntimeError("sdvlh_batch_force_keyframe_misprediction")
+
+    def restart_tracker(self, i):
+        self.lib.sdvlh_batch_restart_tracker.argtypes = [C.c_void_p, C.c_int]
+        if self.lib.sdvlh_batch_restart_tracker(self.h, int(i)) != 0:
+            raise RuntimeError("sdvlh_batch_restart_tracker")
 
     def set_distortion(self, dist5):
         d = np.ascontiguousarray(dist5, np.float64)
```

Measured after the change: 475,200, median of 5. +3.2%, better.
